# TianyiFranklinWang/MIRROR

Hardware: AMD Instinct MI355X
Metric: SSL samples/sec (slide+RNA pairs) (higher is better)
Workload: dtype bf16; 1 GPU; BASELINE c2: B=16/GPU x [4096 patch tokens x 1024-d] + [2048 genes], D=512, RNA depth 6 / 8 heads, train mode, local-batch InfoNCE; precision_policy=bf16, per_gpu_batch=16, global_batch=16, parallelism=dp1, grad_bucket_dtype=f32, step_launch=hip_graph

## Files before the change

include/mirror_hip.h:

```cpp
#ifndef MIRROR_HIP_H
#define MIRROR_HIP_H
#include <stdint.h>

#ifdef __cplusplus
extern "C" {
#endif

#define MH_OK 0
#define MH_EINVAL (-1)
#define MH_EUNSUP (-2)
#define MH_EHIP (-3)

#define MH_F32 0
#define MH_BF16 1

#define MH_ACT_NONE 0
#define MH_ACT_RELU 1
#define MH_ACT_GELU 2

typedef void* mh_stream;

const char* mh_last_error(void);
int mh_version(void);
int mh_exp_build(void);
// ... 23 lines not shown
    int32_t a_kc, b_kc;
    int32_t dtA, dtB, dtC, mma;
    int32_t batch1, batch2;
    int64_t sA1, sA2, sB1, sB2, sC1, sC2;
    float alpha, diag;
    int32_t act;
    int32_t accumulate;
    int32_t split_k;
    const void* R; float rcoef;
    float* workspace;
    int64_t workspace_floats;
    void* C2;
    int32_t r_bf16;
    int32_t k_segments;
    int64_t sA_seg, sB_seg;
    int32_t row_softmax;
    const mh_gemm_epi* epi;
    int32_t a_rows_per_batch, a_row_skip;
    int32_t shared_chip;
    int32_t c_rows_per_batch, c_row_skip;
    int32_t window_batches;
} mh_gemm_desc;
int mh_gemm(const mh_gemm_desc* d, mh_stream s);
const char* mh_gemm_variant_name(void);
int64_t mh_gemm_workspace_bytes(const mh_gemm_desc* d);

int mh_skinny_fwd(const void* x, int64_t ldx, const void* w, int64_t ldw, const float* bias, const float* addend, int64_t ldadd,
                  void* y, int64_t ldy, int M, int N, int K, int act, int dt_x, int dt_y, mh_stream s);
int mh_skinny_wgrad(const void* dy, int64_t lddy, const void* x, int64_t ldx, float* dw, int64_t lddw, float* db, int M, int N,
                    int K, int accumulate, int dt_dy, int dt_x, mh_stream s);
#define MH_SKINNY_MANY_MAX 32
typedef struct {
    const void* dy; int64_t lddy;
    const void* x; int64_t ldx;
    float* dw; int64_t lddw;
    float* db;
    int32_t M, N, K;
    int32_t dt_dy, dt_x;
} mh_skinny_wgrad_item;
int mh_skinny_wgrad_many(const mh_skinny_wgrad_item* items, int n, mh_stream s);
int mh_transpose_bf16(const void* in, void* out, int R, int C, mh_stream s);
int mh_transpose_bf16_many(const void* src, void* dst, const int64_t* table, int n, int max_r, int max_c, int vec_ok,
                           mh_stream s);

int mh_layernorm_fwd(const void* x, const float* gamma, const float* beta, void* y, float* mean, float* rstd,
                     int batches, int rows_per_batch, int D, int64_t x_bs, int64_t y_bs, float eps,
                     int dt_x, int dt_y, mh_stream s);
int mh_layernorm_fwd_dual(const float* x, const float* gamma, const float* beta, float* y, void* y_bf16, float* mean, float* rstd,
                          int batches, int rows_per_batch, int D, int64_t x_bs, int64_t y_bs, float eps, mh_stream s);
int mh_layernorm_fwd_q8(const float* x, const float* gamma, const float* beta, void* y, float* mean, float* rstd,
                        int batches, int rows_per_batch, int D, int64_t x_bs, int64_t y_bs, float eps, void* q8, unsigned* ring,
                        const float* tick, float margin, float* scale, mh_stream s);
int64_t mh_layernorm_bwd_workspace_bytes(int64_t rows, int D);
typedef struct {
    const void* dy;
    const void* x;
    const float *gamma, *mean, *rstd;
    void* dx;
    float *dgamma, *dbeta;
    int32_t batches, rows_per_batch, D;
    int64_t x_bs, y_bs;
    int32_t dt_x, dt_dy, dt_dx;
    int32_t accumulate_dx;
    float* workspace;
    int64_t ws_floats;
    const void* gadd;
    int32_t pad, l;
    const float* row_mask;
    const float* lm_scale;
    void* relu_out;
    int32_t relu_first, relu_rows;
    float* relu_db;
    const void* fan_bf16;
    float fan_alpha;
    const float* fan_cls;
    void* drop_out;
    float drop_p;
    uint64_t drop_seed, drop_offset;
    const uint64_t* drop_base;
    float* drop_db;
    int32_t drop_rows_per_batch;
} mh_ln_bwd;
int mh_layernorm_bwd(const mh_ln_bwd* d, mh_stream s);

int mh_layernorm_fwd_lm(const float* x, const float* gamma, const float* beta, void* y, float* mean, float* rstd, void* xpm,
                        void* xpm_bf16, int batches, int rows, int D, int64_t x_bs, int pad, int l, float eps, const float* row_mask,
                        const float* lm_scale, mh_stream s);

int mh_quant_fp8(const void* x, int64_t n, void* q, float* scale, unsigned* amax_scratch, int dt, mh_stream s);
int mh_quant_fp8_delayed(const void* x, int64_t n, void* q, float* scale, unsigned* ring, const float* tick, float margin,
                         int dt, mh_stream s);
int mh_gemm_fp8(const void* A, int64_t lda, int64_t a_bs, const void* B, int64_t ldb, void* C, int64_t ldc, int64_t c_bs, int batch,
                const float* scale_a, const float* scale_b, const float* bias, int act, int M, int N, int K, int dt_c, mh_stream s);

int mh_softmax_fwd(const void* x, void* y, int64_t rows, int cols, int64_t ldx, int64_t ldy,
                   int dt_x, int dt_y, mh_stream s);
int mh_softmax_bwd(const void* y, const void* dy, void* dx, int64_t rows, int cols, int64_t ldy, int64_t lddy,
                   int64_t lddx, int dt_y, int dt_dy, int dt_dx, mh_stream s);

int mh_softmax_masked_fwd(const void* x, void* y, const float* rowmask, const float* colmask, int64_t batches, int h, int R,
                          int cols, int dt_x, int dt_y, mh_stream s);
int mh_softmax_masked_bwd(const void* y, const void* dy, void* dx, const float* rowmask, const float* colmask, int64_t batches,
                          int h, int R, int cols, int dt_y, int dt_d, mh_stream s);
int mh_row_scale(const void* x, const float* scale, void* y, int64_t rows, int D, int dt, mh_stream s);
int mh_keymask_plan(const unsigned char* mask, float* mrow, float* mlm, float* lscale, int64_t B, int64_t n_src, int lead, int wrap,
                    int pad, int l, mh_stream s);

int mh_landmark_fwd(const void* qkv, void* lm, int B, int n_p, int D, int l, int dt, mh_stream s);
int mh_landmark_bwd(const void* dlm, void* dqkv, int B, int n_p, int D, int l, int dt, mh_stream s);
int mh_resconv_fwd(const void* v, int64_t ldv, int64_t v_bs, const float* w, void* out, int64_t ldo, int64_t o_bs,
                   int B, int n_p, int heads, int dh, int taps, int transpose, int accumulate,
                   int dt_v, int dt_o, mh_stream s);
int mh_resconv_wgrad(const void* v, int64_t ldv, int64_t v_bs, const void* dout, int64_t ldo, int64_t o_bs,
                     float* dw, int B, int n_p, int heads, int dh, int taps, int dt_v, int dt_o, mh_stream s);
int64_t mh_resconv_bwd_workspace_bytes(int B, int n_p, int heads, int dh, int taps);
int mh_resconv_bwd(const void* dout, int64_t ldo, int64_t o_bs, const void* v, int64_t ldv, int64_t v_bs, const float* w, void* dv,
                   int64_t lddv, int64_t dv_bs, float* dw, float* workspace, int64_t ws_floats, int B, int n_p, int heads, int dh,
                   int taps, int dt_v, int dt_o, mh_stream s);
int mh_pinv_absmax(const float* x, uint64_t* stats64, int BH, int m, mh_stream s);
int mh_pinv_z0(const float* x, const uint64_t* stats64, float* z0, int BH, int m, mh_stream s);
int mh_pinv_z0_bwd(const float* x, const float* z0, const float* dz0, const uint64_t* stats64, float* dx,
                   float* scratch1, int scratch_zeroed, int BH, int m, mh_stream s);
int mh_pinv_s2_bwd(const float* p, const float* dz0, const uint64_t* stats64, float* dx, float* scratch1, int scratch_zeroed, int BH,
                   int m, const float* mlm, int heads, mh_stream s);
int mh_pinv_chain_prep(const float* x, const uint64_t* stats64, float* z0, void* xp, void* z0p, int BH, int m, mh_stream s);
int mh_pinv_chain_pack(const float* dz, void* up, int BH, int m, mh_stream s);
int mh_pinv_chain_fwd(const void* XP, void* saved, void* zfT, int BH, int m, int iters, const float* z0f, const uint64_t* stats64,
                      int z0_rowmajor, mh_stream s);
int mh_nys_sim2(const void* lm, float* a2, void* xp, float* z0f, uint64_t* stats64, int B, int m, int D, int heads, float scale,
                int64_t lm_ld, const float* mlm, mh_stream s);
int mh_nys_dz_dav(const float* dw2, const float* av, const void* zfT, void* up, void* dav, float* delta3, int BH, int m, int dh,
                  mh_stream s);
int mh_pinv_chain_bwd(const void* XP, const void* saved, const void* dzf, void* work, float* dX, float* dz0, int BH, int m,
                      int iters, mh_stream s);
int64_t mh_pinv_chain_workspace_bytes(int BH, int m, int iters, int which);
int mh_nys_attn1_fwd(const void* qkv, const void* lm, const void* w2, void* out, float* lse1, const float* mrow, const float* mlm,
                     int B, int h, int n_p, int m, int dh, float scale, int accumulate, int64_t lm_ld, void* o1, mh_stream s);
int mh_nys_attn1_fwd_q8(const void* qkv, const void* lm, const void* w2, void* out, float* lse1, int B, int h, int n_p, int m, int dh,
                        float scale, int accumulate, void* q8, unsigned* ring, const float* tick, float margin, float* q8_scale, void* o1,
                        mh_stream s);
int64_t mh_nys_attn3_ws_floats(int B, int h, int n_p);
int64_t mh_nys_attn3_workspace_bytes(int B, int h, int n_p);
int mh_nys_attn3_fwd(const void* qkv, const void* lm, float* av, float* lse3, float* workspace, int64_t ws_floats,
                     const float* mrow, const float* mlm, int B, int h, int n_p, int m, int dh, float scale, int64_t lm_ld,
                     const float* rc_w, void* rc_out, mh_stream s);
int mh_nys_attn1_bwd(const void* qkv, const void* lm, const void* w2, const void* dout, const float* lse1, const void* o1, float* delta1,
                     void* dqkv, float* dw2, float* dlm, const float* mrow, const float* mlm, int B, int h, int n_p, int m, int dh,
                     float scale, int64_t lm_ld, mh_stream s);
int mh_nys_attn3_bwd(const void* qkv, const void* lm, const float* av, const void* dav, const float* lse3, float* delta3,
                     void* dqkv, float* dlm, const float* mrow, const float* mlm, int B, int h, int n_p, int m, int dh,
                     float scale, int64_t lm_ld, mh_stream s);
int mh_nys_cls_attn(const void* qkv, const void* lm, const void* z, const float* lse3, float* row, const float* mrow, const float* mlm,
                    int B, int h, int n_p, int m, int dh, int cls_row, float scale, int64_t lm_ld, int z_colmajor, int dt,
                    mh_stream s);
int mh_lm_merge(const float* a, const float* b, void* out, int64_t rows, int cols, int64_t out_ld, int zero_cols, mh_stream s);
int mh_eye_minus(const float* P, float* T, float d, int BH, int m, mh_stream s);

int mh_seq_finish(void* seq, const float* cls, int B, int N, int add, int D, int dt, mh_stream s);
int mh_seq_finish_bwd(void* dseq, float* dcls, int B, int N, int add, int D, int dt, mh_stream s);
int mh_ppeg_merge(const float* w7, const float* w5, const float* w3, const float* b7, const float* b5,
                  const float* b3, float* merged, float* bsum, int D, mh_stream s);
int mh_ppeg_fwd(const void* x, void* y, const float* merged, const float* bsum, int B, int S, int D,
                int flip, int dt_x, int dt_y, mh_stream s);
int mh_ppeg_wgrad(const void* x, const void* dout, float* dmerged, float* dbsum, int B, int S, int D,
                  int dt_x, int dt_o, mh_stream s);
int mh_ppeg_bwd(const float* x, const float* dy, const float* merged, float* dx, float* dmerged, float* dbsum, int B, int S,
// ... 296 lines not shown
```

mirror_amd/_lib.py:

```python
from __future__ import annotations

import ctypes as C
import os

_HERE = os.path.dirname(os.path.abspath(__file__))
LIB_PATH = os.environ.get("MIRROR_HIP_LIB") or os.path.join(_HERE, "lib", "libmirror_hip.so")

MH_F32, MH_BF16 = 0, 1
ACT_NONE, ACT_RELU, ACT_GELU = 0, 1, 2


class GemmEpi(C.Structure):
    _fields_ = [
        ("kind", C.c_int32), ("resid", C.c_void_p),
        ("p", C.c_float), ("seed", C.c_uint64), ("offset", C.c_uint64), ("dev_base", C.c_void_p),
        ("mask", C.c_void_p), ("token", C.c_void_p), ("pos", C.c_void_p),
        ("rows_per_batch", C.c_int32), ("first", C.c_int32),
        ("tgt", C.c_void_p), ("tgt_bs", C.c_int64), ("sq", C.c_void_p),
    ]


class SkinnyWgradItem(C.Structure):
    _fields_ = [("dy", C.c_void_p), ("lddy", C.c_int64), ("x", C.c_void_p), ("ldx", C.c_int64), ("dw", C.c_void_p), ("lddw", C.c_int64),
                ("db", C.c_void_p), ("M", C.c_int32), ("N", C.c_int32), ("K", C.c_int32), ("dt_dy", C.c_int32), ("dt_x", C.c_int32)]
# ... 4 lines not shown
        ("A", C.c_void_p), ("B", C.c_void_p), ("C", C.c_void_p), ("bias", C.c_void_p),
        ("M", C.c_int32), ("N", C.c_int32), ("K", C.c_int32),
        ("lda", C.c_int64), ("ldb", C.c_int64), ("ldc", C.c_int64),
        ("a_kc", C.c_int32), ("b_kc", C.c_int32),
        ("dtA", C.c_int32), ("dtB", C.c_int32), ("dtC", C.c_int32), ("mma", C.c_int32),
        ("batch1", C.c_int32), ("batch2", C.c_int32),
        ("sA1", C.c_int64), ("sA2", C.c_int64), ("sB1", C.c_int64), ("sB2", C.c_int64),
        ("sC1", C.c_int64), ("sC2", C.c_int64),
        ("alpha", C.c_float), ("diag", C.c_float),
        ("act", C.c_int32), ("accumulate", C.c_int32), ("split_k", C.c_int32),
        ("R", C.c_void_p), ("rcoef", C.c_float),
        ("workspace", C.c_void_p), ("workspace_floats", C.c_int64),
        ("C2", C.c_void_p), ("r_bf16", C.c_int32),
        ("k_segments", C.c_int32), ("sA_seg", C.c_int64), ("sB_seg", C.c_int64),
        ("row_softmax", C.c_int32),
        ("epi", C.POINTER(GemmEpi)), ("a_rows_per_batch", C.c_int32), ("a_row_skip", C.c_int32),
        ("shared_chip", C.c_int32),
        ("c_rows_per_batch", C.c_int32), ("c_row_skip", C.c_int32),
        ("window_batches", C.c_int32),
    ]


P, I, L, F, U64 = C.c_void_p, C.c_int, C.c_int64, C.c_float, C.c_uint64


class EmaCfg(C.Structure):
    _fields_ = [("decay", C.c_double), ("min_decay", C.c_double), ("warmup_gamma", C.c_double), ("warmup_power", C.c_double),
                ("update_after_step", C.c_int64), ("use_warmup", C.c_int32)]


class OptimCfg(C.Structure):
    _fields_ = [("rule", C.c_int32), ("beta1", C.c_float), ("beta2", C.c_float), ("eps", C.c_float), ("momentum", C.c_float),
                ("nesterov", C.c_int32)]


OPT_ADAM, OPT_ADAMW, OPT_SGD = 0, 1, 2
OPT_SKIP_GROUP = 255


class LossTermsDesc(C.Structure):
    _fields_ = [
        ("wsi_emb", C.c_void_p), ("rna_emb", C.c_void_p), ("logit_scale", C.c_void_p), ("align_ext", C.c_void_p),
        ("B", C.c_int32), ("D", C.c_int32), ("has_align", C.c_int32),
        ("rna_pred", C.c_void_p), ("rna_tgt", C.c_void_p), ("rna_mask", C.c_void_p), ("n_rna", C.c_int64),
        ("w_mu", C.c_void_p), ("w_logstd", C.c_void_p), ("r_mu", C.c_void_p), ("r_logstd", C.c_void_p),
        ("n_wstyle", C.c_int64), ("n_rstyle", C.c_int64), ("rows_wstyle", C.c_int32), ("rows_rstyle", C.c_int32),
        ("w_score", C.c_void_p), ("r_score", C.c_void_p), ("Bc", C.c_int32), ("P", C.c_int32),
        ("wsi_acc", C.c_void_p), ("weight", C.c_float * 6),
        ("scratch", C.c_void_p), ("save", C.c_void_p), ("out", C.c_void_p),
        ("g_total", C.c_void_p), ("g_terms", C.c_void_p),
        ("d_wsi_emb", C.c_void_p), ("d_rna_emb", C.c_void_p), ("d_logit_scale", C.c_void_p), ("d_align_ext", C.c_void_p),
        ("d_rna_pred", C.c_void_p), ("d_rna_tgt", C.c_void_p), ("d_w_mu", C.c_void_p), ("d_w_logstd", C.c_void_p), ("d_r_mu", C.c_void_p),
        ("d_r_logstd", C.c_void_p), ("d_w_score", C.c_void_p), ("d_r_score", C.c_void_p),
    ]


class RnaBlockDesc(C.Structure):
    _fields_ = (
        [("B", C.c_int32), ("D", C.c_int32), ("Hh", C.c_int32), ("H", C.c_int32), ("eps", C.c_float), ("p_drop", C.c_float),
         ("seed", C.c_uint64), ("offset", C.c_uint64), ("dev_base", C.c_void_p)]
        + [(n, C.c_void_p) for n in (
            "w_qkv", "w_proj", "w_fc1", "w_fc2", "wt_qkv", "wt_proj", "wt_fc1", "wt_fc2",
            "b_qkv", "b_proj", "b_fc1", "b_fc2", "g1", "be1", "g2", "be2",
            "x", "y", "stats", "qkv", "attn", "o", "x1", "u", "f", "dy", "dx",
            "dw_qkv", "dw_proj", "dw_fc1", "dw_fc2", "db_qkv", "db_proj", "db_fc1", "db_fc2", "dg1", "dbe1", "dg2", "dbe2",
            "scratch")])


class LnBwdDesc(C.Structure):
    _fields_ = [
        ("dy", C.c_void_p), ("x", C.c_void_p), ("gamma", C.c_void_p), ("mean", C.c_void_p), ("rstd", C.c_void_p),
        ("dx", C.c_void_p), ("dgamma", C.c_void_p), ("dbeta", C.c_void_p),
        ("batches", C.c_int32), ("rows_per_batch", C.c_int32), ("D", C.c_int32), ("x_bs", C.c_int64), ("y_bs", C.c_int64),
        ("dt_x", C.c_int32), ("dt_dy", C.c_int32), ("dt_dx", C.c_int32), ("accumulate_dx", C.c_int32),
        ("workspace", C.c_void_p), ("ws_floats", C.c_int64),
        ("gadd", C.c_void_p), ("pad", C.c_int32), ("l", C.c_int32), ("row_mask", C.c_void_p), ("lm_scale", C.c_void_p),
        ("relu_out", C.c_void_p), ("relu_first", C.c_int32), ("relu_rows", C.c_int32), ("relu_db", C.c_void_p),
        ("fan_bf16", C.c_void_p), ("fan_alpha", C.c_float), ("fan_cls", C.c_void_p),
        ("drop_out", C.c_void_p), ("drop_p", C.c_float), ("drop_seed", C.c_uint64), ("drop_offset", C.c_uint64),
        ("drop_base", C.c_void_p), ("drop_db", C.c_void_p), ("drop_rows_per_batch", C.c_int32),
    ]


_SIGS = {
    "mh_gemm": [C.POINTER(GemmDesc)],
    "mh_skinny_fwd": [P, L, P, L, P, P, L, P, L, I, I, I, I, I, I],
    "mh_skinny_wgrad": [P, L, P, L, P, L, P, I, I, I, I, I, I],
    "mh_skinny_wgrad_many": [C.POINTER(SkinnyWgradItem), I],
    "mh_transpose_bf16": [P, P, I, I],
    "mh_transpose_bf16_many": [P, P, P, I, I, I, I],
    "mh_layernorm_fwd": [P, P, P, P, P, P, I, I, I, L, L, F, I, I],
    "mh_layernorm_fwd_dual": [P, P, P, P, P, P, P, I, I, I, L, L, F],
    "mh_layernorm_fwd_q8": [P, P, P, P, P, P, I, I, I, L, L, F, P, P, P, F, P],
    "mh_layernorm_bwd": [C.POINTER(LnBwdDesc)],
    "mh_layernorm_fwd_lm": [P, P, P, P, P, P, P, P, I, I, I, L, I, I, F, P, P],
    "mh_softmax_fwd": [P, P, L, I, L, L, I, I],
    "mh_softmax_bwd": [P, P, P, L, I, L, L, L, I, I, I],
    "mh_landmark_fwd": [P, P, I, I, I, I, I],
    "mh_landmark_bwd": [P, P, I, I, I, I, I],
    "mh_resconv_fwd": [P, L, L, P, P, L, L, I, I, I, I, I, I, I, I, I],
    "mh_resconv_wgrad": [P, L, L, P, L, L, P, I, I, I, I, I, I, I],
    "mh_resconv_bwd": [P, L, L, P, L, L, P, P, L, L, P, P, L, I, I, I, I, I, I, I],
    "mh_pinv_absmax": [P, P, I, I],
    "mh_pinv_z0": [P, P, P, I, I],
    "mh_pinv_z0_bwd": [P, P, P, P, P, P, I, I, I],
    "mh_pinv_s2_bwd": [P, P, P, P, P, I, I, I, P, I],
    "mh_eye_minus": [P, P, F, I, I],
    "mh_pinv_chain_prep": [P, P, P, P, P, I, I],
    "mh_pinv_chain_pack": [P, P, I, I],
    "mh_pinv_chain_fwd": [P, P, P, I, I, I, P, P, I],
    "mh_nys_sim2": [P, P, P, P, P, I, I, I, I, F, L, P],
    "mh_nys_dz_dav": [P, P, P, P, P, P, I, I, I],
    "mh_pinv_chain_bwd": [P, P, P, P, P, P, I, I, I],
    "mh_nys_attn1_fwd": [P, P, P, P, P, P, P, I, I, I, I, I, F, I, L, P],
    "mh_nys_attn1_fwd_q8": [P, P, P, P, P, I, I, I, I, I, F, I, P, P, P, F, P, P],
    "mh_nys_attn3_fwd": [P, P, P, P, P, L, P, P, I, I, I, I, I, F, L, P, P],
    "mh_nys_attn1_bwd": [P, P, P, P, P, P, P, P, P, P, P, P, I, I, I, I, I, F, L],
    "mh_nys_attn3_bwd": [P, P, P, P, P, P, P, P, P, P, I, I, I, I, I, F, L],
    "mh_nys_cls_attn": [P, P, P, P, P, P, P, I, I, I, I, I, I, F, L, I, I],
    "mh_seq_finish": [P, P, I, I, I, I, I],
    "mh_seq_finish_bwd": [P, P, I, I, I, I, I],
    "mh_ppeg_merge": [P, P, P, P, P, P, P, P, I],
    "mh_ppeg_fwd": [P, P, P, P, I, I, I, I, I, I],
    "mh_ppeg_wgrad": [P, P, P, P, I, I, I, I, I],
    "mh_ppeg_bwd": [P, P, P, P, P, P, I, I, I, P, P, F, U64, U64, P],
    "mh_ppeg_grad_scatter": [P, P, P, P, P, P, P, P, I],
    "mh_rank_mask": [P, P, I, I, I],
    "mh_mask_apply_fwd": [P, P, P, P, P, I, I, I, I, I, I, I],
    "mh_mask_apply_bwd": [P, P, P, P, P, I, I, I, I, I, I, I, P],
    "mh_rank_mask_keep": [P, P, P, P, I, I, I],
    "mh_rows_gather": [P, P, P, I, I, I, I, I],
    "mh_mask_expand_fwd": [P, P, P, P, P, I, I, I, I, I],
    "mh_mask_apply_bwd_keep": [P, P, P, P, P, I, I, I, I, I, P],
    "mh_rows_expand_zero": [P, P, P, I, I, I, I, I],
    "mh_headattn_fwd": [P, P, P, I, I, I, I],
    "mh_headattn_bwd": [P, P, P, P, I, I, I, I],
    "mh_add": [P, P, P, L, I, I, I],
    "mh_lm_merge": [P, P, P, L, I, L, I],
    "mh_cast": [P, P, L, I, I],
    "mh_gelu_fwd": [P, P, L, I, I],
    "mh_gelu_bwd": [P, P, P, L, I, I, I],
    "mh_relu_bwd": [P, P, P, L, I, L, L, L, I, I, I],
    "mh_dropout": [P, P, L, F, U64, U64, P, I, I],
    "mh_noise_draws": [P, L, L, U64, U64, P],
    "mh_dropout_add": [P, P, P, L, F, U64, U64, P, I],
    "mh_dropout_lite": [P, P, P, L, F, U64, U64, P, I, I],
    "mh_timestamp": [P],
    "mh_dropout_lite_colsum": [P, P, L, I, F, U64, U64, P, P],
    "mh_colsum": [P, P, L, I, L, I],
    "mh_l2norm_fwd": [P, P, P, I, I, L, F, I, I],
    "mh_l2norm_bwd": [P, P, P, P, I, I, L, F, I, I, I, I],
    "mh_exp_fwd": [P, P, L],
    "mh_exp_bwd": [P, P, P, L, I],
    "mh_reparam_fwd": [P, P, P, P, L],
    "mh_reparam_bwd": [P, P, P, P, P, P, P, L],
    "mh_ce_rows_fwd": [P, L, P, F, I, I, I, F, P, P, P],
    "mh_ce_rows_bwd": [P, L, P, F, P, P, I, F, P, P, I, I, I],
    "mh_mse_masked_fwd": [P, P, P, P, L, I, L, L, I, I],
    "mh_mse_masked_fwd_ordered": [P, P, P, P, L, I, L, L, I, I, P],
    "mh_mse_masked_bwd": [P, P, P, P, P, F, P, P, L, I, L, L, I, I, I, P, I],
    "mh_fanout_bwd": [P, P, F, P, P, I, I, I, I],
    "mh_gather_rows": [P, P, P, L, L, L, I],
    "mh_sample_rows": [P, P, P, P, I, I, L, U64, U64, P, F],
    "mh_sample_weighted": [P, L, P, L, U64, U64, P],
    "mh_quant_fp8": [P, L, P, P, P, I],
    "mh_quant_fp8_delayed": [P, L, P, P, P, P, F, I],
    "mh_gemm_fp8": [P, L, L, P, L, P, L, L, I, P, P, P, I, I, I, I, I],
    "mh_weighted_sum": [P, P, P, P, P, P, F, F, F, F, F, F, I, P],
    "mh_weighted_sum_bwd": [P, F, F, F, F, F, F, I, P],
    "mh_softmax_masked_fwd": [P, P, P, P, L, I, I, I, I, I],
    "mh_softmax_masked_bwd": [P, P, P, P, P, L, I, I, I, I, I],
    "mh_row_scale": [P, P, P, L, I, I],
    "mh_keymask_plan": [P, P, P, P, L, L, I, I, I, I],
    "mh_kl_fwd": [P, P, P, L, F],
    "mh_kl_bwd": [P, P, P, P, P, L, F],
    "mh_symkl_fwd": [P, P, P, I, I, F],
    "mh_symkl_bwd": [P, P, P, P, P, I, I, F],
# ... 182 lines not shown
```

mirror_amd/csrc/norm_softmax.hip:

```cpp
#include "common.h"
#include <cstdlib>

#define LN_MAXPL 32

template <typename TX, typename TY>
__global__ __launch_bounds__(256) void layernorm_fwd_kernel(const TX* __restrict__ x, const float* __restrict__ gamma,
                                                            const float* __restrict__ beta, TY* __restrict__ y,
                                                            float* __restrict__ mean, float* __restrict__ rstd,
                                                            long rows, int rpb, int D, long x_bs, long y_bs, float eps) {
    const int lane = threadIdx.x & 63;
    const long row = (long)blockIdx.x * 4 + (threadIdx.x >> 6);
    if (row >= rows) return;
    const long b = row / rpb, i = row % rpb;
    const TX* xr = x + b * x_bs + i * D;
    TY* yr = y + b * y_bs + i * D;
    float v[LN_MAXPL];
    float s = 0.f;
#pragma unroll
    for (int k = 0; k < LN_MAXPL; k++) {
        const int c = lane + 64 * k;
        v[k] = (c < D) ? ldf(xr + c) : 0.f;
        s += v[k];
    }
    const float mu = wave_sum(s) / D;
    float q = 0.f;
#pragma unroll
    for (int k = 0; k < LN_MAXPL; k++) {
        const int c = lane + 64 * k;
        const float d = (c < D) ? v[k] - mu : 0.f;
        q += d * d;
    }
    const float rs = rsqrtf(wave_sum(q) / D + eps);
#pragma unroll
    for (int k = 0; k < LN_MAXPL; k++) {
        const int c = lane + 64 * k;
        if (c < D) stf(yr + c, (v[k] - mu) * rs * gamma[c] + beta[c]);
    }
    if (lane == 0) { mean[row] = mu; rstd[row] = rs; }
}

template <typename TX, typename TDY, typename TDX>
__global__ __launch_bounds__(256) void layernorm_bwd_kernel(const TDY* __restrict__ dy, const TX* __restrict__ x,
                                                            const float* __restrict__ gamma, const float* __restrict__ mean,
                                                            const float* __restrict__ rstd, TDX* __restrict__ dx,
                                                            float* __restrict__ dgamma, float* __restrict__ dbeta,
                                                            long rows, int rpb, int D, long x_bs, long y_bs, int acc_dx) {
    const int lane = threadIdx.x & 63, wave = threadIdx.x >> 6;
    float pg[LN_MAXPL], pb[LN_MAXPL];
#pragma unroll
    for (int k = 0; k < LN_MAXPL; k++) { pg[k] = 0.f; pb[k] = 0.f; }
    for (long row = (long)blockIdx.x * 4 + wave; row < rows; row += (long)gridDim.x * 4) {
        const long b = row / rpb, i = row % rpb;
        const TX* xr = x + b * x_bs + i * D;
        const TDY* dyr = dy + b * y_bs + i * D;
        TDX* dxr = dx + b * x_bs + i * D;
        const float mu = mean[row], rs = rstd[row];
        float xh[LN_MAXPL], gd[LN_MAXPL];
        float s1 = 0.f, s2 = 0.f;
#pragma unroll
        for (int k = 0; k < LN_MAXPL; k++) {
            const int c = lane + 64 * k;
            if (c < D) {
                const float d = ldf(dyr + c);
                xh[k] = (ldf(xr + c) - mu) * rs;
                gd[k] = d * gamma[c];
                pg[k] += d * xh[k];
                pb[k] += d;
                s1 += gd[k];
                s2 += gd[k] * xh[k];
            } else { xh[k] = 0.f; gd[k] = 0.f; }
        }
        s1 = wave_sum(s1) / D;
        s2 = wave_sum(s2) / D;
#pragma unroll
        for (int k = 0; k < LN_MAXPL; k++) {
            const int c = lane + 64 * k;
            if (c < D) {
                float r = rs * (gd[k] - s1 - xh[k] * s2);
                if (acc_dx) r += ldf(dxr + c);
                stf(dxr + c, r);
            }
        }
    }
    __shared__ float red[2][4][64];
#pragma unroll
    for (int k = 0; k < LN_MAXPL; k++) {
        if (64 * k >= D) break;
        __syncthreads();
        red[0][wave][lane] = pg[k];
        red[1][wave][lane] = pb[k];
        __syncthreads();
        if (wave == 0) {
            const int c = lane + 64 * k;
            if (c < D) {
                atomicAdd(dgamma + c, red[0][0][lane] + red[0][1][lane] + red[0][2][lane] + red[0][3][lane]);
                atomicAdd(dbeta + c, red[1][0][lane] + red[1][1][lane] + red[1][2][lane] + red[1][3][lane]);
            }
        }
    }
}

typedef f4_t f4;

template <typename TX, typename TY, int LNV_CH>
__global__ __launch_bounds__(256) void layernorm_fwd_vec_kernel(const TX* __restrict__ x, const float* __restrict__ gamma,
                                                                const float* __restrict__ beta, TY* __restrict__ y,
                                                                float* __restrict__ mean, float* __restrict__ rstd,
                                                                long rows, int rpb, int D, long x_bs, long y_bs, float eps,
                                                                bf16_t* __restrict__ y2 = nullptr) {
    const int lane = threadIdx.x & 63;
    const long row = (long)blockIdx.x * 4 + (threadIdx.x >> 6);
    if (row >= rows) return;
    const long b = row / rpb, i = row % rpb;
    const TX* xr = x + b * x_bs + i * D;
    TY* yr = y + b * y_bs + i * D;
    bf16_t* y2r = y2 ? y2 + b * y_bs + i * D : nullptr;
    f4 v[LNV_CH];
    float s = 0.f;
#pragma unroll
    for (int k = 0; k < LNV_CH; k++) {
        const int c = 256 * k + 4 * lane;
        if (c < D) { v[k] = ld4(xr + c); s += v[k][0] + v[k][1] + v[k][2] + v[k][3]; }
        else v[k] = (f4){0.f, 0.f, 0.f, 0.f};
    }
    const float mu = wave_sum(s) / D;
    float q = 0.f;
#pragma unroll
    for (int k = 0; k < LNV_CH; k++) {
        const int c = 256 * k + 4 * lane;
        if (c < D) {
#pragma unroll
            for (int e = 0; e < 4; e++) { const float d = v[k][e] - mu; q += d * d; }
        }
    }
    const float rs = rsqrtf(wave_sum(q) / D + eps);
#pragma unroll
    for (int k = 0; k < LNV_CH; k++) {
        const int c = 256 * k + 4 * lane;
        if (c < D) {
            const f4 g = ld4(gamma + c), bt = ld4(beta + c);
            f4 o;
#pragma unroll
            for (int e = 0; e < 4; e++) o[e] = (v[k][e] - mu) * rs * g[e] + bt[e];
            st4(yr + c, o);
            if (y2r) st4(y2r + c, o);
        }
    }
    if (lane == 0) { mean[row] = mu; rstd[row] = rs; }
}

#define LMU 2
template <int LNV_CH, int SPLIT>
__global__ __launch_bounds__(256) void layernorm_fwd_lm_kernel(const float* __restrict__ x, const float* __restrict__ gamma,
                                                               const float* __restrict__ beta, bf16_t* __restrict__ y,
                                                               float* __restrict__ mean, float* __restrict__ rstd,
                                                               float* __restrict__ xpm, bf16_t* __restrict__ xpm16, int groups, int m, int rows,
                                                               int D, long x_bs, int pad, int l, float eps, const float* __restrict__ rmask,
                                                               const float* __restrict__ lm_scale) {
    __shared__ f4 part[SPLIT > 1 ? 4 : 1][LNV_CH][64];
    const int lane = threadIdx.x & 63, wave = threadIdx.x >> 6, sub = wave % SPLIT;
    const int grp = blockIdx.x * (4 / SPLIT) + wave / SPLIT;
    if (SPLIT == 1 && grp >= groups) return;
    const int b = grp / m, g = grp - b * m;
    const long n_p = (long)pad + rows;
    f4 gm[LNV_CH], bt[LNV_CH], acc[LNV_CH];
#pragma unroll
    for (int k = 0; k < LNV_CH; k++) {
        const int c = 256 * k + 4 * lane;
        acc[k] = (f4){0.f, 0.f, 0.f, 0.f};
        gm[k] = c < D ? ld4(gamma + c) : acc[k];
        bt[k] = c < D ? ld4(beta + c) : acc[k];
    }
    const int per = (l + SPLIT - 1) / SPLIT;
    const int jbeg = g * l + sub * per;
    const int jend = min(jbeg + per, (g + 1) * l);
    auto load_chunk = [&](f4 (&v)[LMU][LNV_CH], float (&kp)[LMU], int j0) {
#pragma unroll
        for (int u = 0; u < LMU; u++) {
            const int j = j0 + u;
            const bool live = j < jend && j >= pad;
            const float* xr = x + b * x_bs + (long)(live ? j - pad : 0) * D;
            kp[u] = (rmask && live) ? rmask[b * n_p + j] : 1.f;
#pragma unroll
            for (int k = 0; k < LNV_CH; k++) {
                const int c = 256 * k + 4 * lane;
                v[u][k] = (live && c < D) ? ld4(xr + c) : (f4){0.f, 0.f, 0.f, 0.f};
            }
        }
    };
    auto do_chunk = [&](f4 (&v)[LMU][LNV_CH], float (&kp)[LMU], int j0) {
#pragma unroll
        for (int u = 0; u < LMU; u++) {
            const int j = j0 + u;
            if (j >= jend) break;
            bf16_t* yr = y + (b * n_p + j) * D;
            if (j < pad) {
#pragma unroll
                for (int k = 0; k < LNV_CH; k++) {
                    const int c = 256 * k + 4 * lane;
                    if (c < D) st4(yr + c, (f4){0.f, 0.f, 0.f, 0.f});
                }
                continue;
            }
            float s = 0.f;
#pragma unroll
            for (int k = 0; k < LNV_CH; k++) s += v[u][k][0] + v[u][k][1] + v[u][k][2] + v[u][k][3];
            const float mu = wave_sum(s) / D;
            float q = 0.f;
#pragma unroll
            for (int k = 0; k < LNV_CH; k++) {
                const int c = 256 * k + 4 * lane;
                if (c < D) {
#pragma unroll
                    for (int e = 0; e < 4; e++) { const float d = v[u][k][e] - mu; q += d * d; }
                }
            }
            const float rs = rsqrtf(wave_sum(q) / D + eps);
            const bool keep = kp[u] != 0.f;
#pragma unroll
            for (int k = 0; k < LNV_CH; k++) {
                const int c = 256 * k + 4 * lane;
                if (c < D) {
                    f4 o;
#pragma unroll
                    for (int e = 0; e < 4; e++) o[e] = keep ? bf2f(f2bf((v[u][k][e] - mu) * rs * gm[k][e] + bt[k][e])) : 0.f;
                    st4(yr + c, o);
                    acc[k] += o;
                }
// ... 165 lines not shown
        if (wave == 0) {
            const int c = 256 * k + 4 * lane;
            if (c < D) {
                const f4 g = red[0][0][lane] + red[0][1][lane] + red[0][2][lane] + red[0][3][lane];
                const f4 bb = red[1][0][lane] + red[1][1][lane] + red[1][2][lane] + red[1][3][lane];
#pragma unroll
                for (int e = 0; e < 4; e++) { atomicAdd(dgamma + c + e, g[e]); atomicAdd(dbeta + c + e, bb[e]); }
            }
        }
    }
}

extern "C" int mh_layernorm_fwd(const void* x, const float* gamma, const float* beta, void* y, float* mean, float* rstd,
                                int batches, int rpb, int D, int64_t x_bs, int64_t y_bs, float eps, int dt_x, int dt_y,
                                mh_stream s) {
    MH_REQUIRE(D >= 1 && D <= 64 * LN_MAXPL, "mh_layernorm_fwd: D=%d unsupported (max %d)", D, 64 * LN_MAXPL);
    const long rows = (long)batches * rpb;
    if (rows == 0) return MH_OK;
    dim3 grid(mh_cdiv(rows, 4));
    const bool vecok = D % 4 == 0 && x_bs % 4 == 0 && y_bs % 4 == 0 && ((uintptr_t)x & 15) == 0 && ((uintptr_t)y & 15) == 0 &&
                       ((uintptr_t)gamma & 15) == 0 && ((uintptr_t)beta & 15) == 0;
#define LN_FV1(TX, TY, NC) hipLaunchKernelGGL((layernorm_fwd_vec_kernel<TX, TY, NC>), grid, dim3(256), 0, (hipStream_t)s, (const TX*)x, gamma, beta, (TY*)y, mean, rstd, rows, rpb, D, (long)x_bs, (long)y_bs, eps)
#define LN_FV(TX, TY) do { if (D <= 512) LN_FV1(TX, TY, 2); else if (D <= 1024) LN_FV1(TX, TY, 4); else LN_FV1(TX, TY, 8); } while (0)
    if (vecok) {
        if (dt_x == MH_F32 && dt_y == MH_F32) LN_FV(float, float);
        else if (dt_x == MH_F32 && dt_y == MH_BF16) LN_FV(float, bf16_t);
        else if (dt_x == MH_BF16 && dt_y == MH_BF16) LN_FV(bf16_t, bf16_t);
        else LN_FV(bf16_t, float);
        MH_LAUNCH_CHECK("mh_layernorm_fwd");
        return MH_OK;
    }
#undef LN_FV
#undef LN_FV1
#define LN_F(TX, TY) hipLaunchKernelGGL((layernorm_fwd_kernel<TX, TY>), grid, dim3(256), 0, (hipStream_t)s, (const TX*)x, gamma, beta, (TY*)y, mean, rstd, rows, rpb, D, (long)x_bs, (long)y_bs, eps)
    if (dt_x == MH_F32 && dt_y == MH_F32) LN_F(float, float);
    else if (dt_x == MH_F32 && dt_y == MH_BF16) LN_F(float, bf16_t);
    else if (dt_x == MH_BF16 && dt_y == MH_BF16) LN_F(bf16_t, bf16_t);
    else LN_F(bf16_t, float);
#undef LN_F
    MH_LAUNCH_CHECK("mh_layernorm_fwd");
    return MH_OK;
}

extern "C" int mh_layernorm_fwd_lm(const float* x, const float* gamma, const float* beta, void* y, float* mean, float* rstd, void* xpm,
                                   void* xpm_bf16, int batches, int rows, int D, int64_t x_bs, int pad, int l, float eps, const float* row_mask,
                                   const float* lm_scale, mh_stream s) {
    MH_REQUIRE(l >= 1 && pad >= 0 && rows >= 1 && (pad + rows) % l == 0, "mh_layernorm_fwd_lm: pad + rows = %d must be a multiple of l = %d", pad + rows, l);
    MH_REQUIRE(D % 4 == 0 && D <= 2048 && x_bs % 4 == 0 && (((uintptr_t)x | (uintptr_t)gamma | (uintptr_t)beta) & 15) == 0 &&
                   ((uintptr_t)y & 7) == 0 && ((uintptr_t)xpm & 15) == 0 && ((uintptr_t)xpm_bf16 & 7) == 0,
               "mh_layernorm_fwd_lm: D %% 4 == 0, D <= 2048 and aligned buffers (D=%d)", D);
    if (batches == 0) return MH_OK;
    const int m = (pad + rows) / l, groups = batches * m;
    int split = 1;
    while (split < 4 && (long)groups * split < 4096 && l >= 8 * split && groups % (4 / (2 * split)) == 0) split *= 2;
#ifdef MH_EXP
    if (const char* e = getenv("MH_LN_LM_SPLIT")) split = atoi(e);
#endif
    MH_REQUIRE((split == 1 || split == 2 || split == 4) && groups % (4 / split) == 0, "mh_layernorm_fwd_lm: %d waves per group with %d groups", split, groups);
    dim3 grid(mh_cdiv(groups, 4 / split));
#define LNL_(NC, SP) hipLaunchKernelGGL((layernorm_fwd_lm_kernel<NC, SP>), grid, dim3(256), 0, (hipStream_t)s, x, gamma, beta, (bf16_t*)y, mean, rstd, (float*)xpm, (bf16_t*)xpm_bf16, groups, m, rows, D, (long)x_bs, pad, l, eps, row_mask, lm_scale)
#define LNL(NC) do { if (split == 1) LNL_(NC, 1); else if (split == 2) LNL_(NC, 2); else LNL_(NC, 4); } while (0)
    if (D <= 512) LNL(2); else if (D <= 1024) LNL(4); else LNL(8);
#undef LNL
#undef LNL_
    MH_LAUNCH_CHECK("mh_layernorm_fwd_lm");
    return MH_OK;
}

extern "C" int mh_layernorm_fwd_dual(const float* x, const float* gamma, const float* beta, float* y, void* y_bf16, float* mean, float* rstd,
                                     int batches, int rpb, int D, int64_t x_bs, int64_t y_bs, float eps, mh_stream s) {
    const long rows = (long)batches * rpb;
    if (rows == 0) return MH_OK;
    MH_REQUIRE(y_bf16 && D % 4 == 0 && D <= 2048 && x_bs % 4 == 0 && y_bs % 4 == 0 &&
                   (((uintptr_t)x | (uintptr_t)y | (uintptr_t)gamma | (uintptr_t)beta) & 15) == 0 && ((uintptr_t)y_bf16 & 7) == 0,
               "mh_layernorm_fwd_dual: D %% 4 == 0, D <= 2048 and aligned buffers (D=%d)", D);
    dim3 grid(mh_cdiv(rows, 4));
#define LND(NC) hipLaunchKernelGGL((layernorm_fwd_vec_kernel<float, float, NC>), grid, dim3(256), 0, (hipStream_t)s, x, gamma, beta, y, mean, rstd, rows, rpb, D, (long)x_bs, (long)y_bs, eps, (bf16_t*)y_bf16)
    if (D <= 512) LND(2); else if (D <= 1024) LND(4); else LND(8);
#undef LND
    MH_LAUNCH_CHECK("mh_layernorm_fwd_dual");
    return MH_OK;
}

extern "C" int mh_layernorm_fwd_q8(const float* x, const float* gamma, const float* beta, void* y, float* mean, float* rstd,
                                   int batches, int rows_per_batch, int D, int64_t x_bs, int64_t y_bs, float eps, void* q8, unsigned* ring,
                                   const float* tick, float margin, float* scale, mh_stream s) {
    const long rows = (long)batches * rows_per_batch;
    if (rows == 0) return MH_OK;
    MH_REQUIRE(D % 4 == 0 && D <= 2048 && x_bs % 4 == 0 && y_bs % 4 == 0 && (((uintptr_t)x | (uintptr_t)gamma | (uintptr_t)beta) & 15) == 0 &&
                   ((uintptr_t)y & 7) == 0 && ((uintptr_t)q8 & 3) == 0,
               "mh_layernorm_fwd_q8: D %% 4 == 0, D <= 2048 and aligned buffers (D=%d)", D);
    MH_REQUIRE(ring && tick && scale && margin >= 1.f, "mh_layernorm_fwd_q8: ring, tick, scale and margin >= 1 are required");
    dim3 grid((unsigned)min((long)mh_cdiv(rows, 4), 4096L));
#define LNQ(NC) hipLaunchKernelGGL((layernorm_fwd_q8_kernel<NC>), grid, dim3(256), 0, (hipStream_t)s, x, gamma, beta, (bf16_t*)y, mean, rstd, rows, rows_per_batch, D, (long)x_bs, (long)y_bs, eps, (unsigned char*)q8, ring, tick, margin, scale)
    if (D <= 512) LNQ(2); else if (D <= 1024) LNQ(4); else LNQ(8);
#undef LNQ
    MH_LAUNCH_CHECK("mh_layernorm_fwd_q8");
    return MH_OK;
}

template <typename TX, typename TDY, int LNV_CH, bool RELU = false, bool FAN = false, bool DROP = false>
__global__ __launch_bounds__(256, LNV_CH == 2 ? 4 : 1) void layernorm_bwd_ws_kernel(const TDY* __restrict__ dy, const TX* __restrict__ x,
                                                               const float* __restrict__ gamma, const float* __restrict__ mean,
                                                               const float* __restrict__ rstd, TX* __restrict__ dx,
                                                               float* __restrict__ ws, int rows, int rpb, int D, long x_bs,
                                                               long y_bs, int acc_dx, int rows_per_block,
                                                               const TDY* __restrict__ gadd = nullptr, int ga_pad = 0, int ga_l = 1,
                                                               int ga_m = 0, float ga_scale = 0.f, bf16_t* __restrict__ relu_out = nullptr,
                                                               int relu_first = 0, int relu_rows = 0, int relu_cs = 0,
                                                               const bf16_t* __restrict__ fan = nullptr, float fan_alpha = 0.f,
                                                               const float* __restrict__ fan_cls = nullptr,
                                                               bf16_t* __restrict__ drop_out = nullptr, float drop_p = 0.f, uint64_t drop_seed = 0,
                                                               uint64_t drop_offset = 0, const uint64_t* __restrict__ drop_base = nullptr,
                                                               int drop_rpb = 0, const float* __restrict__ rmask = nullptr,
                                                               const float* __restrict__ lm_scale = nullptr) {
    const int lane = threadIdx.x & 63, wave = threadIdx.x >> 6;
    constexpr bool THIRD = RELU || DROP;
    __shared__ f4 sgm[THIRD ? LNV_CH : 1][64];
    f4 pg[LNV_CH], pb[LNV_CH], gm[THIRD ? 1 : LNV_CH], pr[THIRD ? LNV_CH : 1];
    uint32_t dthr = 0;
    float dscale = 1.f;
    if constexpr (DROP) {
        if (drop_base) drop_offset += *drop_base & ~7ull;
        dthr = drop16_thr(drop_p);
        dscale = drop16_scale(dthr);
    }
#pragma unroll
    for (int k = 0; k < LNV_CH; k++) {
        pg[k] = (f4){0.f, 0.f, 0.f, 0.f};
        pb[k] = pg[k];
        if constexpr (THIRD) pr[k] = pg[k];
        const int c = 256 * k + 4 * lane;
        if constexpr (THIRD) {
            if (wave == 0) sgm[k][lane] = (c < D) ? ld4(gamma + c) : pg[k];
        } else gm[k] = (c < D) ? ld4(gamma + c) : pg[k];
    }
    if constexpr (THIRD) __syncthreads();
    const int r0 = blockIdx.x * rows_per_block, r1 = min(rows, r0 + rows_per_block);
    for (int row = r0 + wave; row < r1; row += 8) {
        uint32_t keepbits = 0;
        if constexpr (DROP) {
            static_assert(LNV_CH <= 4, "one byte per chunk in a 32-bit word");
            const int odd = lane & 1;
            const int rr = row + 4 * odd;
            uint32_t mine = 0;
            if (rr < r1) {
                const long orow = drop_rpb == rpb ? (long)rr : (long)(rr / rpb) * drop_rpb + (rr % rpb);
#pragma unroll
                for (int k = 0; k < LNV_CH; k++) {
                    const int c8 = 256 * k + 8 * (lane >> 1);
                    if (c8 < D) mine |= drop16_keep8((drop_offset + (uint64_t)(orow * D + c8)) >> 3, drop_seed, dthr) << (8 * k);
                }
            }
            const uint32_t other = (uint32_t)__builtin_amdgcn_mov_dpp((int)mine, 0xB1, 0xF, 0xF, true);
#pragma unroll
            for (int u = 0; u < 2; u++) {
                const uint32_t src = (odd == u) ? mine : other;
#pragma unroll
                for (int k = 0; k < LNV_CH; k++) keepbits |= (((src >> (8 * k)) >> (4 * odd)) & 15u) << (4 * (u * LNV_CH + k));
            }
            asm volatile("" : "+v"(keepbits));
        }
        f4 dv[2][LNV_CH], xv[2][LNV_CH], ov[2][LNV_CH];
        float mu[2], rs[2];
        long xo[2], ro[2];
        bool ok[2];
#pragma unroll
        for (int u = 0; u < 2; u++) {
            const int rr = row + 4 * u;
            ok[u] = rr < r1;
            const int rc = ok[u] ? rr : row;
            const int b = rc / rpb, i = rc - b * rpb;
            xo[u] = b * x_bs + (long)i * D;
            ro[u] = (RELU && i >= relu_first && i < relu_first + relu_rows) ? ((long)b * relu_rows + (i - relu_first)) * D
                    : (DROP ? ((long)b * drop_rpb + i) * D : -1);
            const TDY* dyr = dy + b * y_bs + (long)i * D;
            mu[u] = mean[rc];
            rs[u] = rstd[rc];
#pragma unroll
            for (int k = 0; k < LNV_CH; k++) {
                const int c = 256 * k + 4 * lane;
                if (c < D) {
                    dv[u][k] = ld4(dyr + c);
                    xv[u][k] = ld4(x + xo[u] + c);
                    if (acc_dx) ov[u][k] = ld4(dx + xo[u] + c);
                    if (gadd) dv[u][k] += ld4(gadd + ((long)b * ga_m + (i + ga_pad) / ga_l) * D + c) *
                                          (lm_scale ? ga_scale * lm_scale[(long)b * ga_m + (i + ga_pad) / ga_l] : ga_scale);
                    if (rmask && rmask[(long)b * (ga_pad + rpb) + ga_pad + i] == 0.f) dv[u][k] = (f4){0.f, 0.f, 0.f, 0.f};
                    if constexpr (FAN) {
                        if (i >= 1) dv[u][k] += ld4(fan + ((long)b * (rpb - 1) + (i - 1)) * D + c) * fan_alpha;
                        else if (fan_cls) dv[u][k] += ld4(fan_cls + (long)b * D + c);
                    }
                }
            }
        }
#pragma unroll
        for (int u = 0; u < 2; u++) {
            if (!ok[u]) continue;
            float s1 = 0.f, s2 = 0.f;
            unsigned pos = 0;
#pragma unroll
            for (int k = 0; k < LNV_CH; k++) {
                const int c = 256 * k + 4 * lane;
                if (c < D) {
                    f4 gq;
                    if constexpr (THIRD) gq = sgm[k][lane]; else gq = gm[k];
#pragma unroll
                    for (int e = 0; e < 4; e++) {
                        if constexpr (RELU) pos |= (xv[u][k][e] > 0.f ? 1u : 0u) << (4 * k + e);
                        const float xh = (xv[u][k][e] - mu[u]) * rs[u];
                        const float d = dv[u][k][e];
                        const float gd = d * gq[e];
                        pg[k][e] += d * xh;
                        pb[k][e] += d;
                        s1 += gd;
                        s2 += gd * xh;
                        xv[u][k][e] = xh;
                        dv[u][k][e] = gd;
                    }
                }
            }
            s1 = wave_sum(s1) / D;
            s2 = wave_sum(s2) / D;
#pragma unroll
            for (int k = 0; k < LNV_CH; k++) {
                const int c = 256 * k + 4 * lane;
                if (c < D) {
                    f4 r;
#pragma unroll
                    for (int e = 0; e < 4; e++) r[e] = rs[u] * (dv[u][k][e] - s1 - xv[u][k][e] * s2);
                    if (acc_dx) r += ov[u][k];
                    if (RELU && !DROP && ro[u] >= 0) {
                        typedef unsigned ln_u32x2 __attribute__((ext_vector_type(2)));
                        const ln_u32x2 w = {pack_bf2((pos >> (4 * k)) & 1u ? r[0] : 0.f, (pos >> (4 * k + 1)) & 1u ? r[1] : 0.f),
                                         pack_bf2((pos >> (4 * k + 2)) & 1u ? r[2] : 0.f, (pos >> (4 * k + 3)) & 1u ? r[3] : 0.f)};
                        *reinterpret_cast<ln_u32x2*>(relu_out + ro[u] + c) = w;
                        pr[k] += (f4){__uint_as_float(w[0] << 16), __uint_as_float(w[0] & 0xffff0000u),
                                      __uint_as_float(w[1] << 16), __uint_as_float(w[1] & 0xffff0000u)};
                    } else {
                        st4(dx + xo[u] + c, r);
                        if constexpr (DROP) {
                            typedef unsigned ln_u32x2d __attribute__((ext_vector_type(2)));
                            const long e0 = ro[u] + c;
                            const uint32_t keep = keepbits >> (4 * (u * LNV_CH + k));
                            const ln_u32x2d w = {pack_bf2((keep & 1u) ? __fmul_rn(r[0], dscale) : 0.f, (keep & 2u) ? __fmul_rn(r[1], dscale) : 0.f),
                                                 pack_bf2((keep & 4u) ? __fmul_rn(r[2], dscale) : 0.f, (keep & 8u) ? __fmul_rn(r[3], dscale) : 0.f)};
                            *reinterpret_cast<ln_u32x2d*>(drop_out + e0) = w;
                            pr[k] += (f4){__uint_as_float(w[0] << 16), __uint_as_float(w[0] & 0xffff0000u),
                                          __uint_as_float(w[1] << 16), __uint_as_float(w[1] & 0xffff0000u)};
                        }
                    }
                }
            }
        }
    }
    __shared__ f4 red[THIRD ? 3 : 2][4][64];
    const int segs = ((RELU && relu_cs) || DROP) ? 3 : 2;
    float* wsb = ws + (long)blockIdx.x * segs * D;
#pragma unroll
    for (int k = 0; k < LNV_CH; k++) {
        if (256 * k >= D) break;
        __syncthreads();
        red[0][wave][lane] = pg[k];
        red[1][wave][lane] = pb[k];
        if constexpr (THIRD) red[2][wave][lane] = pr[k];
        __syncthreads();
        if (wave == 0) {
            const int c = 256 * k + 4 * lane;
            if (c < D) {
                *reinterpret_cast<f4*>(wsb + c) = red[0][0][lane] + red[0][1][lane] + red[0][2][lane] + red[0][3][lane];
                *reinterpret_cast<f4*>(wsb + D + c) = red[1][0][lane] + red[1][1][lane] + red[1][2][lane] + red[1][3][lane];
                if constexpr (THIRD)
                    if (DROP || relu_cs) *reinterpret_cast<f4*>(wsb + 2 * D + c) = red[2][0][lane] + red[2][1][lane] + red[2][2][lane] + red[2][3][lane];
            }
        }
    }
}

__global__ __launch_bounds__(256) void layernorm_bwd_fold_kernel(const float* __restrict__ ws, int nb, int D, float* __restrict__ dgamma,
                                                                 float* __restrict__ dbeta) {
    const int t = blockIdx.x * 256 + threadIdx.x;
    if (t >= 2 * D) return;
    const int per = (nb + gridDim.y - 1) / gridDim.y;
    const int b0 = blockIdx.y * per, b1 = min(nb, b0 + per);
    float s = 0.f;
    for (int b = b0; b < b1; b++) s += ws[(long)b * 2 * D + t];
    atomicAdd(t < D ? dgamma + t : dbeta + (t - D), s);
}

__global__ __launch_bounds__(256) void layernorm_bwd_fold4_kernel(const float* __restrict__ ws, int nb, int D, float* __restrict__ dgamma,
                                                                  float* __restrict__ dbeta, int segs = 2, float* __restrict__ dthird = nullptr) {
    typedef float lf4 __attribute__((ext_vector_type(4)));
    __shared__ lf4 red[4][64];
    const int lane = threadIdx.x & 63, wave = threadIdx.x >> 6;
    const int t = (blockIdx.x * 64 + lane) * 4;
    const bool live = t < segs * D;
    const int chunks = gridDim.y * 4, per = (nb + chunks - 1) / chunks;
    const int b0 = (blockIdx.y * 4 + wave) * per, b1 = min(nb, b0 + per);
    lf4 s = {0.f, 0.f, 0.f, 0.f};
    if (live) {
        int b = b0;
        for (; b + 8 <= b1; b += 8) {
            lf4 v[8];
#pragma unroll
            for (int u = 0; u < 8; u++) v[u] = *reinterpret_cast<const lf4*>(ws + (long)(b + u) * segs * D + t);
#pragma unroll
            for (int u = 0; u < 8; u++) s += v[u];
        }
        for (; b < b1; b++) s += *reinterpret_cast<const lf4*>(ws + (long)b * segs * D + t);
    }
    red[wave][lane] = s;
    __syncthreads();
    if (wave == 0 && live) {
        s = red[0][lane] + red[1][lane] + red[2][lane] + red[3][lane];
        float* dst = t < D ? dgamma + t : (t < 2 * D ? dbeta + (t - D) : dthird + (t - 2 * D));
#pragma unroll
        for (int e = 0; e < 4; e++) atomicAdd(dst + e, s[e]);
    }
}

static int ln_bwd_blocks() { return 512; }

extern "C" int64_t mh_layernorm_bwd_workspace_bytes(int64_t rows, int D) {
    if (rows < 64 || D <= 0) return 0;
    const int64_t nb = rows / 16 < 1024 ? (rows / 16 < 1 ? 1 : rows / 16) : 1024;
    return 3 * (int64_t)D * nb * 4;
}

static int ln_bwd_impl(const mh_ln_bwd& d, mh_stream s) {
    const int D = d.D, rpb = d.rows_per_batch, dt_x = d.dt_x, dt_dy = d.dt_dy;
    const int l = d.gadd ? d.l : 1;
    const long rows = (long)d.batches * rpb;
    const bool vecok = D % 4 == 0 && d.x_bs % 4 == 0 && d.y_bs % 4 == 0 && ((uintptr_t)d.x & 15) == 0 && ((uintptr_t)d.dy & 15) == 0 &&
                       ((uintptr_t)d.dx & 15) == 0 && ((uintptr_t)d.gamma & 15) == 0;
    const bool ws_form = vecok && d.workspace && d.ws_floats >= 2L * D && rows >= 64;
    const bool f32_x = dt_x == MH_F32 && d.dt_dx == MH_F32;
    const bool ws3 = ((uintptr_t)d.workspace & 15) == 0 && d.ws_floats >= 3L * D;
    const bool fan_ok = rpb >= 2 && ((uintptr_t)d.fan_bf16 & 7) == 0 && (!d.fan_cls || ((uintptr_t)d.fan_cls & 15) == 0) && D % 4 == 0;
    MH_REQUIRE(D >= 1 && D <= 64 * LN_MAXPL, "mh_layernorm_bwd: D=%d unsupported", D);
    MH_REQUIRE(d.dt_dx == dt_x, "mh_layernorm_bwd: dx dtype must equal x dtype");
    MH_REQUIRE(rows < (1L << 31), "mh_layernorm_bwd: too many rows");
    MH_REQUIRE(!d.gadd || (l >= 1 && d.pad >= 0 && (d.pad + rpb) % l == 0 && ((uintptr_t)d.gadd & 15) == 0),
               "mh_layernorm_bwd: landmark rider: l >= 1, pad >= 0, (pad + rows) %% l == 0, gadd on 16 bytes");
    MH_REQUIRE(d.gadd || (!d.relu_out && !d.row_mask && !d.lm_scale), "mh_layernorm_bwd: landmark rider: relu_out, row_mask and lm_scale need gadd");
    MH_REQUIRE(!d.gadd || (!d.fan_bf16 && !d.drop_out), "mh_layernorm_bwd: landmark rider: gadd excludes fan_bf16 and drop_out");
    MH_REQUIRE(!d.relu_out || (dt_x == MH_F32 && dt_dy == MH_BF16 && d.relu_first >= 0 && d.relu_rows >= 0 && d.relu_first + d.relu_rows <= rpb &&
                               ((uintptr_t)d.relu_out & 7) == 0 && D % 4 == 0),
               "mh_layernorm_bwd: ReLU rider: relu_out needs f32 x, bf16 dy and a row range inside the batch");
    MH_REQUIRE(!d.relu_db || (d.relu_out && ws3), "mh_layernorm_bwd: ReLU rider: relu_db rides on relu_out (workspace of >= 3 D floats)");
    MH_REQUIRE(!d.fan_bf16 || (f32_x && fan_ok), "mh_layernorm_bwd: fan rider: f32 x / dx, fan [batches, rows - 1, D] bf16 on quads, rows >= 2");
    MH_REQUIRE(!d.drop_out || d.drop_rows_per_batch >= rpb, "mh_layernorm_bwd: drop rider: the Dropout's tensor has %d rows per batch, the norm reads %d",
               d.drop_rows_per_batch, rpb);
    MH_REQUIRE(!d.drop_out || (f32_x && d.drop_db && d.drop_p >= 0.f && d.drop_p < 1.f && (d.drop_offset & 7) == 0 && ((uintptr_t)d.drop_out & 7) == 0 &&
                               D % 8 == 0 && D <= 1024 && ws3),
               "mh_layernorm_bwd: drop rider: f32 x / dx, drop_out / drop_db, p in [0, 1), offset %% 8 == 0, D %% 8 == 0, D <= 1024, a workspace of >= 3 D floats");
    MH_REQUIRE(rows == 0 || ws_form || !(d.gadd || d.fan_bf16 || d.drop_out),
               "mh_layernorm_bwd: the %s rider needs the workspace form (D %% 4 == 0, 16-byte aligned buffers, a workspace of >= %d D floats, >= 64 rows)",
               d.gadd ? "landmark" : (d.drop_out ? "drop" : "fan"), d.drop_out ? 3 : 2);
    if (rows == 0) return MH_OK;
    dim3 grid((unsigned)min((long)mh_cdiv(rows, 4), (long)ln_bwd_blocks()));
    if (ws_form) {
        float* third = d.drop_out ? d.drop_db : d.relu_db;
        const int segs = third ? 3 : 2;
        const long cap = d.ws_floats / ((long)segs * D);
        long nb = min(cap, min((long)mh_cdiv(rows, 16), 1024L));
        const int rows_per_block = (int)(mh_cdiv(mh_cdiv(rows, nb), 8) * 8);
        nb = mh_cdiv(rows, rows_per_block);
        dim3 g2((unsigned)nb);
#define LN_WS(TX, TDY, NC, RL, FN, DR) hipLaunchKernelGGL((layernorm_bwd_ws_kernel<TX, TDY, NC, RL, FN, DR>), g2, dim3(256), 0, (hipStream_t)s, (const TDY*)d.dy, (const TX*)d.x, d.gamma, d.mean, d.rstd, (TX*)d.dx, d.workspace, (int)rows, rpb, D, (long)d.x_bs, (long)d.y_bs, d.accumulate_dx, rows_per_block, (const TDY*)d.gadd, d.pad, l, (d.pad + rpb) / l, 1.f / (float)l, (bf16_t*)d.relu_out, d.relu_first, d.relu_rows, d.relu_db ? 1 : 0, (const bf16_t*)d.fan_bf16, d.fan_alpha, d.fan_cls, (bf16_t*)d.drop_out, d.drop_p, d.drop_seed, d.drop_offset, d.drop_base, d.drop_rows_per_batch, d.row_mask, d.lm_scale)
#define LN_BW(TX, TDY, RL) do { if (D <= 512) LN_WS(TX, TDY, 2, RL, false, false); else if (D <= 1024) LN_WS(TX, TDY, 4, RL, false, false); else LN_WS(TX, TDY, 8, RL, false, false); } while (0)
#define LN_BWF(NC) do { if (dt_dy == MH_F32) LN_WS(float, float, NC, false, true, false); else LN_WS(float, bf16_t, NC, false, true, false); } while (0)
#define LN_BWD(TDY, FN) do { if (D <= 512) LN_WS(float, TDY, 2, false, FN, true); else LN_WS(float, TDY, 4, false, FN, true); } while (0)
        if (d.drop_out) {
            if (d.fan_bf16 && dt_dy == MH_F32) LN_BWD(float, true);
            else if (d.fan_bf16) LN_BWD(bf16_t, true);
            else if (dt_dy == MH_F32) LN_BWD(float, false);
            else LN_BWD(bf16_t, false);
        } else if (d.fan_bf16) {
            if (D <= 512) LN_BWF(2); else if (D <= 1024) LN_BWF(4); else LN_BWF(8);
        } else if (d.relu_out) LN_BW(float, bf16_t, true);
        else if (dt_x == MH_F32 && dt_dy == MH_F32) LN_BW(float, float, false);
        else if (dt_x == MH_F32 && dt_dy == MH_BF16) LN_BW(float, bf16_t, false);
        else if (dt_x == MH_BF16 && dt_dy == MH_BF16) LN_BW(bf16_t, bf16_t, false);
        else LN_BW(bf16_t, float, false);
#undef LN_BWD
#undef LN_BWF
#undef LN_BW
#undef LN_WS
        if (D % 4 == 0 && ((uintptr_t)d.workspace & 15) == 0)
            hipLaunchKernelGGL(layernorm_bwd_fold4_kernel, dim3(mh_cdiv(segs * D / 4, 64), (unsigned)min(mh_cdiv(nb, 32), 16)), dim3(256), 0,
                               (hipStream_t)s, (const float*)d.workspace, (int)nb, D, d.dgamma, d.dbeta, segs, third);
        else
            hipLaunchKernelGGL(layernorm_bwd_fold_kernel, dim3(mh_cdiv(2 * D, 256), (unsigned)min(nb, 32L)), dim3(256), 0, (hipStream_t)s,
                               (const float*)d.workspace, (int)nb, D, d.dgamma, d.dbeta);
        MH_LAUNCH_CHECK("mh_layernorm_bwd");
        return MH_OK;
    }
    if (vecok) {
#define LN_BV1(TX, TDY, NC) hipLaunchKernelGGL((layernorm_bwd_vec_kernel<TX, TDY, NC>), grid, dim3(256), 0, (hipStream_t)s, (const TDY*)d.dy, (const TX*)d.x, d.gamma, d.mean, d.rstd, (TX*)d.dx, d.dgamma, d.dbeta, rows, rpb, D, (long)d.x_bs, (long)d.y_bs, d.accumulate_dx)
#define LN_BV(TX, TDY) do { if (D <= 512) LN_BV1(TX, TDY, 2); else if (D <= 1024) LN_BV1(TX, TDY, 4); else LN_BV1(TX, TDY, 8); } while (0)
        if (dt_x == MH_F32 && dt_dy == MH_F32) LN_BV(float, float);
        else if (dt_x == MH_F32 && dt_dy == MH_BF16) LN_BV(float, bf16_t);
        else if (dt_x == MH_BF16 && dt_dy == MH_BF16) LN_BV(bf16_t, bf16_t);
        else LN_BV(bf16_t, float);
#undef LN_BV
#undef LN_BV1
        MH_LAUNCH_CHECK("mh_layernorm_bwd");
        return MH_OK;
    }
#define LN_B(TX, TDY) hipLaunchKernelGGL((layernorm_bwd_kernel<TX, TDY, TX>), grid, dim3(256), 0, (hipStream_t)s, (const TDY*)d.dy, (const TX*)d.x, d.gamma, d.mean, d.rstd, (TX*)d.dx, d.dgamma, d.dbeta, rows, rpb, D, (long)d.x_bs, (long)d.y_bs, d.accumulate_dx)
    if (dt_x == MH_F32 && dt_dy == MH_F32) LN_B(float, float);
    else if (dt_x == MH_F32 && dt_dy == MH_BF16) LN_B(float, bf16_t);
    else if (dt_x == MH_BF16 && dt_dy == MH_BF16) LN_B(bf16_t, bf16_t);
    else LN_B(bf16_t, float);
#undef LN_B
    MH_LAUNCH_CHECK("mh_layernorm_bwd");
    return MH_OK;
}

extern "C" int mh_layernorm_bwd(const mh_ln_bwd* d, mh_stream s) {
    MH_REQUIRE(d, "mh_layernorm_bwd: NULL descriptor");
    return ln_bwd_impl(*d, s);
}

template <typename TX, typename TY, bool WAVE>
__global__ __launch_bounds__(256) void softmax_fwd_kernel(const TX* x, TY* y, long rows,
                                                          int cols, long ldx, long ldy) {
    __shared__ float red[4];
    const int lane = threadIdx.x & 63;
    const long row = WAVE ? (long)blockIdx.x * 4 + (threadIdx.x >> 6) : (long)blockIdx.x;
    if (WAVE && row >= rows) return;
    const int t0 = WAVE ? lane : threadIdx.x, step = WAVE ? 64 : 256;
    const TX* xr = x + row * ldx;
    TY* yr = y + row * ldy;
    float m = -INFINITY;
    for (int c = t0; c < cols; c += step) m = fmaxf(m, ldf(xr + c));
    m = WAVE ? wave_max(m) : block_max256(m, red);
    float sum = 0.f;
    for (int c = t0; c < cols; c += step) sum += __expf(ldf(xr + c) - m);
    sum = WAVE ? wave_sum(sum) : block_sum256(sum, red);
    const float inv = 1.f / sum;
    for (int c = t0; c < cols; c += step) stf(yr + c, __expf(ldf(xr + c) - m) * inv);
}

template <typename TY, typename TDY, typename TDX, bool WAVE>
__global__ __launch_bounds__(256) void softmax_bwd_kernel(const TY* y, const TDY* dy,
                                                          TDX* dx, long rows, int cols, long ldy, long lddy,
                                                          long lddx) {
    __shared__ float red[4];
    const int lane = threadIdx.x & 63;
    const long row = WAVE ? (long)blockIdx.x * 4 + (threadIdx.x >> 6) : (long)blockIdx.x;
    if (WAVE && row >= rows) return;
    const int t0 = WAVE ? lane : threadIdx.x, step = WAVE ? 64 : 256;
    const TY* yr = y + row * ldy;
    const TDY* dyr = dy + row * lddy;
    TDX* dxr = dx + row * lddx;
    float dot = 0.f;
    for (int c = t0; c < cols; c += step) dot += ldf(yr + c) * ldf(dyr + c);
    dot = WAVE ? wave_sum(dot) : block_sum256(dot, red);
    for (int c = t0; c < cols; c += step) stf(dxr + c, ldf(yr + c) * (ldf(dyr + c) - dot));
}

template <typename TX, typename TY, bool WAVE, int NV>
__global__ __launch_bounds__(256) void softmax_fwd_vec_kernel(const TX* x, TY* y, long rows, int cols, long ldx, long ldy) {
    __shared__ float red[4];
    const int lane = threadIdx.x & 63;
    const long row = WAVE ? (long)blockIdx.x * 4 + (threadIdx.x >> 6) : (long)blockIdx.x;
    if (WAVE && row >= rows) return;
    const int t0 = (WAVE ? lane : threadIdx.x) * 4, step = (WAVE ? 64 : 256) * 4;
    const TX* xr = x + row * ldx;
    TY* yr = y + row * ldy;
    f4 v[NV];
    float m = -INFINITY;
#pragma unroll
    for (int k = 0; k < NV; k++) {
        const int c = t0 + k * step;
        if (c < cols) { v[k] = ld4(xr + c); m = fmaxf(fmaxf(fmaxf(m, v[k][0]), fmaxf(v[k][1], v[k][2])), v[k][3]); }
    }
    m = WAVE ? wave_max(m) : block_max256(m, red);
    float sum = 0.f;
#pragma unroll
    for (int k = 0; k < NV; k++) {
        const int c = t0 + k * step;
        if (c < cols) {
#pragma unroll
            for (int e = 0; e < 4; e++) { v[k][e] = __expf(v[k][e] - m); sum += v[k][e]; }
        }
    }
    sum = WAVE ? wave_sum(sum) : block_sum256(sum, red);
    const float inv = 1.f / sum;
#pragma unroll
    for (int k = 0; k < NV; k++) {
        const int c = t0 + k * step;
        if (c < cols) st4(yr + c, v[k] * inv);
    }
}

template <typename TY, typename TD, bool WAVE, int NV>
__global__ __launch_bounds__(256) void softmax_bwd_vec_kernel(const TY* y, const TD* dy, TD* dx, long rows, int cols, long ldy,
                                                              long lddy, long lddx) {
    __shared__ float red[4];
    const int lane = threadIdx.x & 63;
    const long row = WAVE ? (long)blockIdx.x * 4 + (threadIdx.x >> 6) : (long)blockIdx.x;
    if (WAVE && row >= rows) return;
    const int t0 = (WAVE ? lane : threadIdx.x) * 4, step = (WAVE ? 64 : 256) * 4;
// ... 221 lines not shown
```

mirror_amd/functional.py:

```python
from __future__ import annotations

from dataclasses import dataclass
from typing import List, Optional, Tuple

import os

import torch
from torch.autograd import Function

from . import kernels as K
from ._lib import ACT_NONE, ACT_RELU, MH_BF16, MH_F32

f32, bf16 = torch.float32, torch.bfloat16


@dataclass(frozen=True)
class Precision:
    name: str
    mma: int
    act: torch.dtype
    pinv_mma: int
    fp8_fwd: bool = False


# ... 778 lines not shown
def to_out_dropout_add(resid, core, w, b, r0: int, R: int, p: float, training: bool, prec: Precision, res=None, link=None):
    if (training and p > 0.0 and prec.act == bf16 and not prec.fp8_fwd and resid.dtype == f32 and resid.is_contiguous()
            and core.dtype == bf16 and tuple(resid.shape) == (core.shape[0], R, w.shape[0]) and (core.shape[0] * R * w.shape[0]) % 8 == 0
            and K.linear_fused_ok(core, shadow(w, prec), (r0, R))):
        site = _DropSite() if (_DROP_IN_LN_BWD and b is not None) else None
        out = ToOutDropAddFn.apply(resid, core, w, b, r0, R, p, prec, site, res, link)
        if site is not None:
            out._drop_site = site
        return out
    y = LinearRowsFn.apply(core, w, b, r0, R, prec, prec.act)
    return dropout_add(resid, y, p, training, lite=True, res=res)


class HeadSqErrFn(Function):

    @staticmethod
    def forward(ctx, x, w, b, r0, R, prec, tgt, mask, acc, cs_tok=None):
        wa = shadow(w, prec)
        Bn, T, Kd = x.shape
        N = wa.shape[0]
        y = torch.empty((Bn, R, N), device=x.device, dtype=bf16)
        K.linear_fused(x, wa, None if b is None else b.detach(), y,
                       K.epi_sqerr(mask, tgt, tgt.stride(0), acc, R), window=(r0, R))
        ctx.save_for_backward(x, wa, w, b)
        ctx.r0, ctx.R, ctx.prec, ctx.cs_tok = r0, R, prec, cs_tok
        return y

    @staticmethod
    def backward(ctx, dy):
        x, wa, w, b = ctx.saved_tensors
        prec = ctx.prec
        if not dy.is_contiguous():
            dy = dy.contiguous()
        if dy.dtype != prec.act:
            dy = K.cast(dy, prec.act)
        got = None if ctx.cs_tok is None else ctx.cs_tok.claim(dy)
        db_table = None if got is None else got[0]
        dx, dw, db = _linear_rows_bwd(ctx.needs_input_grad[0:3], x, wa, w, b, ctx.r0, ctx.R, prec, dy, db_table=db_table)
        return dx, dw, db, None, None, None, None, None, None, None


def head_sqerr(x, w, b, r0: int, R: int, prec: Precision, tgt, mask):
    N = w.shape[0]
    if (tgt is not None and mask is not None and prec.act == bf16 and not prec.fp8_fwd and x.dtype == bf16 and tgt.dtype == f32
            and tgt.dim() == 3 and tuple(tgt.shape) == (x.shape[0], R, N) and tgt.stride(2) == 1 and tgt.stride(1) == N
            and mask.dtype == f32 and mask.is_contiguous() and tuple(mask.shape) == (x.shape[0], R) and R % 256 == 0
            and torch.is_grad_enabled() and K.linear_fused_ok(x, shadow(w, prec), (r0, R))):
        acc = zeros((2,), x.device)
        tok = _Handover("colsum") if (b is not None and _BIAS_IN_PRODUCER) else None
        y = HeadSqErrFn.apply(x, w, b, r0, R, prec, tgt, mask, acc, tok)
        y._sq = (acc, tgt, mask, tgt._version, mask._version)
        y._sq_cs = tok
        return y
    return LinearRowsFn.apply(x, w, b, r0, R, prec, prec.act)


def _cs_of(pred, acc):
    sq, tok = getattr(pred, "_sq", None), getattr(pred, "_sq_cs", None)
    return tok if (sq is not None and tok is not None and acc is not None and sq[0] is acc) else None


def _mse_bwd_cs(tok, pred, tgt, dp, D):
    if tok is None or not K.mse_masked_bwd_colsum_ok(pred, tgt, dp, D):
        return None
    ws = torch.empty((K.MSE_CS_BLOCKS, D), device=dp.device, dtype=f32)
    tok.offer(dp, ws)
    return ws


def _sq_of(pred, tgt, mask):
    sq = getattr(pred, "_sq", None)
    if sq is None:
        return None
    acc, t0, m0, tv, mv = sq
    if (t0.data_ptr() == tgt.data_ptr() and tuple(t0.shape) == tuple(tgt.shape) and t0.stride() == tgt.stride() and t0._version == tv
            and m0.data_ptr() == mask.data_ptr() and tuple(m0.shape) == tuple(mask.shape) and m0._version == mv):
        return acc
    return None


class EmbedMaskPosFn(Function):

    @staticmethod
    def forward(ctx, h32, h, w, b, mask, token, pos, first, prec, keepmap=None):
        wa = shadow(w, prec)
        Bn, T, Kd = h.shape
        N = wa.shape[0]
        out = torch.empty((Bn, T, N), device=h.device, dtype=f32)
        M = Bn * T
        bd = None if b is None else b.detach()
        tok, ps = token.detach().reshape(-1).contiguous(), pos.detach().reshape(T, N).contiguous()
        ctx.geom = (Bn, T, N, first, token.shape, pos.shape, prec)
        ctx.params = (token, pos)
        ctx.keep = None if keepmap is None else keepmap[2]
        if keepmap is not None:
            keep_idx, slot, keep = keepmap
            hc = K.rows_gather(h, keep_idx, first, keep)
            rc = _gemm_rows(hc, wa.t(), bias=bd, mma=prec.mma, out_dtype=bf16)
            K.mask_expand_fwd(rc, slot, tok, ps, T, first, keep, out)
            ctx.save_for_backward(hc, wa, w, b, slot)
            return out
        tail = K.linear_fused_tail(M)
        fork = _tail_fork() if tail else None
        K.linear_fused(h, wa, bd, out, K.epi_maskpos(mask, tok, ps, T, first), m_rows=M - tail)
        if tail and T - tail >= first:
            with _tail_branch(fork, h.device):
                rt = _tail_rows(h[Bn - 1, T - tail:], wa.t(), torch.empty((tail, N), device=h.device, dtype=bf16), bias=bd, mma=prec.mma)
                K.mask_apply_fwd(rt.view(1, tail, N), mask[Bn - 1, T - tail - first:].contiguous(), tok, ps[T - tail:].reshape(-1), 1, tail, N, 0,
                                 False, out=out[Bn - 1:, T - tail:])
        elif tail:
            raise K.MirrorHipError("EmbedMaskPosFn: the tail rows cross the unmasked prefix")
        ctx.save_for_backward(h, wa, w, b, mask)
        return out

    @staticmethod
    def backward(ctx, dy):
        h, wa, w, b, mask = ctx.saved_tensors
        Bn, T, N, first, tshape, pshape, prec = ctx.geom
        keep = ctx.keep
        Tc = T if keep is None else first + keep
        dy = dy.contiguous()
        dr = torch.empty((Bn, Tc, N), device=dy.device, dtype=prec.act)
        token, pos = ctx.params
        dtok, s_tok = _gbuf_n(token, (N,))
        dpos, s_pos = _gbuf_n(pos, (T * N,))
        db_in = None
        quad = K.mask_apply_bwd_dbias_ok(dy, dr, dpos, N)
        if b is not None and ctx.needs_input_grad[3] and _BIAS_IN_PRODUCER and (quad or keep is not None):
            db_in = _gbuf(b, (N,))
        dbias = None if db_in is None else db_in[0]
        if keep is None:
            K.mask_apply_bwd(dy, mask, dtok, dpos, Bn, T, N, first, False, out=dr, dbias=dbias)
        elif quad:
            K.mask_apply_bwd_keep(dy, mask, dtok, dpos, Bn, T, N, first, keep, out=dr, dbias=dbias)
        else:
            dp = zeros((T * N,), dy.device)
            K.mask_apply_bwd_keep(dy, mask, dtok, dp, Bn, T, N, first, keep, out=dr, dbias=dbias)
            dpos.add_(dp)
        dtok, dpos = _gret(token, dtok, s_tok), _gret(pos, dpos, s_pos)
        needs = (ctx.needs_input_grad[0], ctx.needs_input_grad[2], ctx.needs_input_grad[3])
        dh, dw, db = _linear_rows_bwd(needs, h, wa, w, b, 0, Tc, prec, dr, dx_dtype=f32, db_have=db_in)
        if keep is not None and dh is not None:
            dh = K.rows_expand_zero(dh, mask, T, first, keep)
        return (dh, None, dw, db, None, None if dtok is None else dtok.reshape(tshape), None if dpos is None else dpos.reshape(pshape),
                None, None, None)


def embed_mask_pos(h, w, b, mask, token, pos, first: int, prec: Precision):
    hb = h if h.dtype == bf16 else getattr(h, "_bf16", None)
    if (hb is not None and prec.act == bf16 and not prec.fp8_fwd and hb.is_contiguous() and tuple(hb.shape) == tuple(h.shape)
            and mask.dtype == f32 and mask.is_contiguous() and hb.shape[1] >= 256 and K.linear_fused_ok(hb, shadow(w, prec))
            and token.numel() == w.shape[0] and pos.numel() == h.shape[1] * w.shape[0]):
        keepmap = _keep_of(mask, hb.shape[0], hb.shape[1] - first)
        if keepmap is not None and -(-hb.shape[0] * hb.shape[1] // 256) * (w.shape[0] // 256) <= _EMBED_KEEP_TILES:
            keepmap = None
        return EmbedMaskPosFn.apply(h, hb, w, b, mask, token, pos, first, prec, keepmap)
    r = linear(h, w, b, prec=prec)
    return MaskApplyFn.apply(r, mask, token, pos, first, False)


_EMBED_KEEP_TILES = _CUS


def _keep_of(mask, Bn: int, n_tok: int):
    km = getattr(mask, "_keep", None)
    if km is None or mask._version != 0 or tuple(mask.shape) != (Bn, n_tok):
        return None
    keep_idx, slot, keep = km
    if tuple(slot.shape) != (Bn, n_tok) or tuple(keep_idx.shape) != (Bn, keep) or slot.device != mask.device:
        return None
    return km


class LayerNormFn(Function):

    @staticmethod
    def forward(ctx, x, gamma, beta, eps, rows, pad, out_dtype, q8_key=None, dual=None, fan_slot=None, res=None, q8_out=None):
        x = x.contiguous()
        Bn, T, D = x.shape
        y = torch.empty((Bn, pad + rows, D), device=x.device, dtype=out_dtype)
        ctx.fan_slot, ctx.res = fan_slot, res
        ctx.drop_site = getattr(x, "_drop_site", None) if (_DROP_IN_LN_BWD and pad == 0 and x.dtype == f32) else None
        if ctx.drop_site is not None and ctx.drop_site.shape != (Bn, T, D):
            ctx.drop_site = None
        if dual is not None:
            mean = torch.empty((Bn * rows,), device=x.device, dtype=f32)
            rstd = torch.empty_like(mean)
            y16 = torch.empty((Bn, rows, D), device=x.device, dtype=bf16)
            K.layernorm_fwd_dual(x, gamma.detach(), beta.detach(), y, y16, mean, rstd, Bn, rows, D, T * D, rows * D, eps)
            dual.append(y16)
            ctx.save_for_backward(x, gamma, mean, rstd, beta)
            ctx.rows, ctx.pad = rows, pad
            return y
        if pad:
            y[:, :pad].zero_()
        mean = torch.empty((Bn * rows,), device=x.device, dtype=f32)
        rstd = torch.empty_like(mean)
        st = _fp8_state
        site = st["sites"].get(q8_key) if (q8_key is not None and st["tick"] is not None) else None
        if site is not None and st["host_step"] - site[1] >= 2 and x.dtype == f32 and out_dtype == bf16 and D % 4 == 0 and D <= 2048:
            q = torch.empty((Bn, pad + rows, D), device=x.device, dtype=torch.uint8)
            if pad:
                q[:, :pad].zero_()
            sc = K.layernorm_fwd_q8(x, gamma.detach(), beta.detach(), y[:, pad:], mean, rstd, Bn, rows, D, T * D, (pad + rows) * D, eps,
                                    q[:, pad:], site[0], st["tick"])
            q8_out.append((q, sc))
        else:
            K.layernorm_fwd(x, gamma.detach(), beta.detach(), y[:, pad:], mean, rstd, Bn, rows, D, T * D, (pad + rows) * D, eps)
        ctx.save_for_backward(x, gamma, mean, rstd, beta)
        ctx.rows, ctx.pad = rows, pad
        return y

    @staticmethod
    def backward(ctx, dy):
        x, gamma, mean, rstd, beta = ctx.saved_tensors
        Bn, T, D = x.shape
        rows, pad = ctx.rows, ctx.pad
        if not dy.is_contiguous():
            dy = dy.contiguous()
        dg, sunk_g = _gbuf(gamma, (D,))
        db, sunk_b = _gbuf(beta, (D,))
        fan = None
        if ctx.fan_slot is not None and ctx.fan_slot.extra is not None:
            fan, ctx.fan_slot.extra = ctx.fan_slot.extra, None
            if pad or not K.layernorm_bwd_fan_ok(dy, x, x, fan[0], fan[2], Bn, rows, D):
                dy, fan = K.fanout_bwd(dy.float(), fan[0], fan[1], fan[2], Bn, rows, D), None
        G = None if ctx.res is None else ctx.res.take("grad")
        if G is not None and G.numel() == x.numel() and G.dtype == x.dtype and G.is_contiguous():
            G = G.view(x.shape)
            K.layernorm_bwd(dy[:, pad:], x, gamma.detach(), mean, rstd, G, dg, db, Bn, rows, D, T * D, (pad + rows) * D,
                            accumulate_dx=True, fan=fan)
            return None, _gret(gamma, dg, sunk_g), _gret(beta, db, sunk_b), None, None, None, None, None, None, None, None, None
        dx = torch.empty_like(x)
        if rows < T:
            dx[:, rows:].zero_()
        site, drop = ctx.drop_site, None
        if site is not None:
            gbd = torch.empty((Bn, T, D), device=x.device, dtype=bf16)
            cs = zeros((D,), x.device)
            if K.layernorm_bwd_drop_ok(dy, x, dx, gbd, cs, Bn, rows, D, site.offset) and (fan is None or dy.dtype == f32):
                if rows < T:
                    gbd[:, rows:].zero_()
                drop = (gbd, site.p, site.seed, site.offset, site.base, cs)
                site.offer(dx, gbd, cs)
        K.layernorm_bwd(dy[:, pad:], x, gamma.detach(), mean, rstd, dx, dg, db, Bn, rows, D, T * D, (pad + rows) * D, fan=fan, drop=drop)
        return dx, _gret(gamma, dg, sunk_g), _gret(beta, db, sunk_b), None, None, None, None, None, None, None, None, None


def _alias(base: torch.Tensor, offset: int, size, stride) -> torch.Tensor:
    t = torch.empty(0, device=base.device, dtype=base.dtype)
    t.set_(base.untyped_storage(), base.storage_offset() + int(offset), tuple(size), tuple(stride))
    return t


class NormQkvLmFn(Function):

    @staticmethod
    def forward(ctx, x, gamma, beta, eps, rows, pad, l, w, prec, link, rmask=None, lscale=None, res=None):
        ctx.relu_slot = getattr(x, "_relu_slot", None)
        ctx.link, ctx.res = link, res
        x = x.contiguous()
        Bn, T, D = x.shape
        n_p = pad + rows
        m = n_p // l
        P, E = Bn * n_p, Bn * m
        wa = shadow(w, prec)
        N3, c0 = wa.shape[0], 2 * wa.shape[1]
        xe = torch.empty((P + E, D), device=x.device, dtype=bf16)
        mean = torch.empty((Bn * rows,), device=x.device, dtype=f32)
        rstd = torch.empty_like(mean)
        xs = xe[:P].view(Bn, n_p, D)
        K.layernorm_fwd_lm(x, gamma.detach(), beta.detach(), xs, mean, rstd, None, Bn, rows, D, T * D, pad, l, eps, xpm_bf16=xe[P:],
                           row_mask=rmask, lm_scale=lscale)
        ctx.rmask, ctx.lscale = rmask, lscale
        qe = torch.empty((P + E, N3), device=x.device, dtype=bf16)
        qkv = _alias(qe, 0, (Bn, n_p, N3), (n_p * N3, N3, 1))
        fast = (pad > 0 and prec.mma == MH_BF16 and c0 % 256 == 0 and (N3 - c0) % 256 == 0
                and K.gemm_rows_ext_ok(Bn, n_p, pad, rows, E, D, c0, xe, qe[:, :c0]) and _rows_window_ok(xs, qkv[..., c0:], pad, rows, N3 - c0, prec))
        if fast:
            fork = _tail_fork()
            tail = K.gemm_rows_ext(xe, wa[:c0].t(), qe[:, :c0], Bn, n_p, pad, rows, E)
            if tail:
                with _tail_branch(fork, x.device):
                    _tail_rows(xe[P + E - tail:], wa[:c0].t(), qe[P + E - tail:, :c0], mma=prec.mma)

            def later():
                fork = _tail_fork()
                _rows_window(xs, wa[c0:].t(), qkv[..., c0:], pad, rows, mma=prec.mma)
                with _tail_branch(fork, x.device):
                    qkv[:, :pad].zero_()
        else:
            K.gemm(xe, wa[:c0].t(), out=qe[:, :c0], mma=prec.mma)

            def later():
                K.gemm(xe[:P], wa[c0:].t(), out=qe[:P, c0:], mma=prec.mma)
        link.v_cols = later
        ctx.save_for_backward(x, gamma, mean, rstd, beta, xe, wa, w)
        ctx.geo = (rows, pad, l, fast, prec)
        return qkv, _alias(qe, P * N3, (Bn, m, c0), (m * N3, N3, 1))

    @staticmethod
    def backward(ctx, dqkv, dlm):
        x, gamma, mean, rstd, beta, xe, wa, w = ctx.saved_tensors
        rows, pad, l, fast, prec = ctx.geo
        Bn, T, D = x.shape
        n_p = pad + rows
        m = n_p // l
        P, E = Bn * n_p, Bn * m
        N3, c0 = wa.shape[0], 2 * wa.shape[1]
        pend = ctx.link.take("lm_merge")
        merge = None if pend is None else pend[1]
        de = ext_rows_of(dqkv, dlm, P, E, N3, c0, copy_lm=merge is None)
        if pend is not None and de.data_ptr() != pend[0].data_ptr():
            raise K.MirrorHipError("NormQkvLmFn.backward: the pending landmark merge belongs to another gradient buffer")
        dxe = torch.empty((P + E, D), device=x.device, dtype=bf16)
        if fast:
            fork = _tail_fork()
            _rows_window(de[:P].view(Bn, n_p, N3), wa, dxe[:P].view(Bn, n_p, D), pad, rows, mma=prec.mma, wt=shadow_t(w, prec))
            with _tail_branch(fork, x.device):
                if merge is not None:
                    merge()
                K.gemm(de[P:, :c0], wa[:c0], out=dxe[P:], mma=prec.mma)
        else:
            if merge is not None:
                merge()
            K.gemm(de, wa, out=dxe, mma=prec.mma)
        dw = None
        if ctx.needs_input_grad[7]:
            dwb, sunk = _gbuf(w, (N3, D))
# ... 40 lines not shown
        return dx, _gret(gamma, dg, sunk_g), _gret(beta, db, sunk_b), None, None, None, None, dw, None, None, None, None, None


def ext_rows_alloc(Bn: int, n_p: int, m: int, N3: int, c0: int, device):
    P, E = Bn * n_p, Bn * m
    de = torch.empty((P + E, N3), device=device, dtype=bf16)
    return de, _alias(de, 0, (Bn, n_p, N3), (n_p * N3, N3, 1)), _alias(de, P * N3, (Bn, m, c0), (m * N3, N3, 1))


def ext_rows_of(dqkv, dlm, P: int, E: int, N3: int, c0: int, copy_lm: bool = True):
    if (dqkv.dtype == bf16 and dlm.dtype == bf16 and dqkv.is_contiguous() and dqkv.numel() == P * N3
            and dlm.data_ptr() == dqkv.data_ptr() + P * N3 * 2 and dlm.dim() == 3 and tuple(dlm.stride()) == (dlm.shape[1] * N3, N3, 1)
            and dlm.shape[0] * dlm.shape[1] == E and dlm.shape[2] == c0
            and dqkv.untyped_storage().nbytes() - dqkv.storage_offset() * 2 >= (P + E) * N3 * 2):
        return torch.as_strided(dqkv, (P + E, N3), (N3, 1))
    if not copy_lm:
        raise K.MirrorHipError("NormQkvLmFn.backward: a pending landmark merge needs the gradient views of ext_rows_alloc")
    de = torch.empty((P + E, N3), device=dqkv.device, dtype=bf16)
    de[:P].copy_(dqkv.reshape(P, N3))
    de[P:, :c0].copy_(dlm.reshape(E, c0))
    de[P:, c0:].zero_()
    return de


_KEYMASK_PLAN = True
class KeyMask:

    def __init__(self, src: torch.Tensor, lead: int = 0, wrap: int = 0):
        self.src = src if src.dtype == torch.bool else src.to(torch.bool)
        self.src = self.src.contiguous()
        self.lead, self.wrap = int(lead), int(wrap)
        self.shape = (src.shape[0], self.lead + src.shape[1] + self.wrap)
        self._plans = {}

    def dense(self) -> torch.Tensor:
        parts = ([torch.ones_like(self.src[:, :1]).expand(-1, self.lead)] if self.lead else []) + [self.src] + (
            [self.src[:, :self.wrap]] if self.wrap else [])
        return torch.cat(parts, dim=1) if len(parts) > 1 else self.src

    def plan(self, pad: int, l: int):
        key = (pad, l)
        if key not in self._plans:
            if _KEYMASK_PLAN:
                self._plans[key] = K.keymask_plan(self.src, self.lead, self.wrap, pad, l)
            else:
                n = self.shape[1]
                mrow = torch.nn.functional.pad(self.dense().to(torch.float32), (pad, 0), value=0.0).contiguous()
                cnt = mrow.reshape(mrow.shape[0], (n + pad) // l, l).sum(-1)
                self._plans[key] = (mrow, (cnt > 0).float().contiguous(), (float(l) / (cnt + 1e-8)).contiguous())
        return self._plans[key]


_LM_ROWS = True
_RELU_SQUARE_PAD = True
_RELU_IN_LN_BWD = True
class _ReluSlot(_Handover):
    __slots__ = ("n", "bias", "redo")

    def __init__(self):
        super().__init__("relu")
        self.n = self.bias = self.redo = None


def layer_norm_landmarks_ok(x, rows: int, pad: int, l: int, prec: Precision) -> bool:
    return (_LM_ROWS and prec.act == bf16 and not prec.fp8_fwd and x.dim() == 3 and x.dtype == f32 and x.shape[-1] % 4 == 0
            and x.shape[-1] <= 2048 and (pad + rows) % l == 0 and x.shape[0] * rows >= 64)


def fp8_site_key(w: torch.Tensor, prec: "Precision"):
    return (shadow(w, prec).data_ptr(), "x")


_FAN_IN_LN_BWD = True


class _FanSlot:
    __slots__ = ("extra",)

    def __init__(self):
        self.extra = None



def layer_norm(x, gamma, beta, eps, *, rows=None, pad=0, out_dtype=f32, q8_key=None, bf16_copy=False, res=None):
    squeeze = x.dim() == 2
    if squeeze:
        x = x.unsqueeze(0)
    r = x.shape[1] if rows is None else rows
    dual = None
    if (bf16_copy and not squeeze and x.dtype == f32 and out_dtype == f32 and pad == 0 and x.shape[-1] % 4 == 0
            and x.shape[-1] <= 2048 and q8_key is None):
        dual = []
    slot = _FanSlot() if (_FAN_IN_LN_BWD and not squeeze and pad == 0 and out_dtype == f32 and x.dtype == f32) else None
    q8 = [] if q8_key is not None else None
    y = LayerNormFn.apply(x, gamma, beta, eps, r, pad, out_dtype, q8_key, dual, slot, res, q8)
    if dual:
        y._bf16 = dual[0]
    if q8:
        y._q8 = q8[0]
    if slot is not None:
        y._fan_slot = slot
    return y.squeeze(0) if squeeze else y


class AddFn(Function):

    @staticmethod
    def forward(ctx, a, b, out_dtype, residual):
        ctx.da, ctx.db = a.dtype, b.dtype
        ctx.res = residual if a.is_contiguous() else None
        return K.add(a.contiguous(), b.contiguous(), out_dtype=out_dtype)

    @staticmethod
    def backward(ctx, dy):
        dy = dy.contiguous()
        ga = K.cast(dy, ctx.da)
        if ctx.res is not None and ga.dtype == f32:
            ctx.res.grad = ga
        return ga, K.cast(dy, ctx.db), None, None


def add(a, b, out_dtype=f32, residual=None):
    return AddFn.apply(a, b, out_dtype, residual)


class GeluFn(Function):
    @staticmethod
    def forward(ctx, x):
        x = x.contiguous()
        ctx.save_for_backward(x)
        return K.gelu_fwd(x)

    @staticmethod
    def backward(ctx, dy):
        (x,) = ctx.saved_tensors
        dy = dy.contiguous()
        return K.gelu_bwd(x, dy if dy.dtype == x.dtype else K.cast(dy, x.dtype))


gelu = GeluFn.apply

_dropout_state = {"seed": 0x5EED, "offset": 0, "base": None, "noise": 0}


def manual_seed(seed: int) -> None:
    _dropout_state["seed"], _dropout_state["offset"], _dropout_state["noise"] = int(seed) & ((1 << 63) - 1), 0, 0
    if _dropout_state["base"] is not None:
        _dropout_state["base"].zero_()


def dropout_step_begin(device) -> None:
    if _dropout_state["base"] is None or _dropout_state["base"].device != torch.device(device):
        _dropout_state["base"] = torch.zeros(1, device=device, dtype=torch.int64)
    _dropout_state["offset"] = 0


def _step_used() -> int:
    used, _dropout_state["offset"] = (_dropout_state["offset"] + 7) // 8 * 8, 0
    return used


def dropout_step_end() -> None:
    base, used = _dropout_state["base"], _step_used()
    if base is not None and used:
        base.add_(used)


def dropout_step_take():
    base, used = _dropout_state["base"], _step_used()
    return (base, used) if (base is not None and used) else (None, 0)


def dropout_device_base_off() -> None:
    _dropout_state["base"] = None


_NOISE_OFFSET = 1 << 44


# ... 591 lines not shown
        elif side is not None:
            torch.cuda.current_stream().wait_stream(side)
            K.shared_chip = False
            del work
        else:
            dS2 = pinv_backward_tile(a2, saved, st, dZ, getattr(ctx, "a2b", None)) if ctx.tile else pinv_backward(a2, saved, st, dZ, pm, sd)
            sm_bwd(a2, dS2, mlm if kmask else None, mlm if kmask else None)
        if dlm2 is None:
            K.gemm(tr(dS2), ql, out=dkl, alpha=scale, accumulate=True, mma=pio)
            K.gemm(dS2, kl, out=dql, alpha=scale, accumulate=True, mma=pio)
        dres = _gret(res_w, dres, dres_sunk)
        dres = None if dres is None else dres.view_as(res_w)
        if de is not None and ctx.link is not None and (kmask is None or (lscale is None and dlm2 is not None)):
            merge = lambda: K.lm_merge(dlm, dlm2, de[Bn * n_p:], D3 - 2 * D)
            ctx.link.lm_merge = (de, merge)
            return dqkv, dres, None, None, None, None, None, None, dlm_out, None, None
        if dlm2 is not None:
            dlm = K.add(dlm, dlm2, out_dtype=A)
        if kmask is not None and lscale is not None:
            dlm = K.row_scale(dlm, lscale)
        if ctx.lm_ext:
            if de is not None:
                dlm_out.copy_(dlm)
                de[Bn * n_p:, 2 * D:].zero_()
                return dqkv, dres, None, None, None, None, None, None, dlm_out, None, None
            return dqkv, dres, None, None, None, None, None, None, dlm, None, None
        K.landmark_bwd(K.cast(dlm, A), dqkv, l)
        return dqkv, dres, None, None, None, None, None, None, None, None, None


class RowScaleFn(Function):

    @staticmethod
    def forward(ctx, x, s):
        ctx.save_for_backward(s)
        return K.row_scale(x.contiguous(), s)

    @staticmethod
    def backward(ctx, dy):
        (s,) = ctx.saved_tensors
        return K.row_scale(dy.contiguous(), s), None


_PROBE = os.environ.get("MIRROR_PROBE", "0") != "0"
_probe_names: List[str] = []
_probe_buf: Optional[torch.Tensor] = None


def probe(name: str) -> None:
    global _probe_buf
    if not _PROBE:
        return
    if _probe_buf is None:
        _probe_buf = torch.zeros(256, dtype=torch.int64, device="cuda")
    if name not in _probe_names:
        _probe_names.append(name)
    K.timestamp(_probe_buf[_probe_names.index(name):_probe_names.index(name) + 1])


def probe_read() -> dict:
    torch.cuda.synchronize()
    v = _probe_buf[:len(_probe_names)].tolist()
    return dict(zip(_probe_names, v))


class ProbeFn(Function):

    @staticmethod
    def forward(ctx, x, name):
        ctx.name = name
        probe(name + ".fwd")
        return x.view_as(x)

    @staticmethod
    def backward(ctx, g):
        probe(ctx.name + ".bwd")
        return g, None


def probe_point(x: torch.Tensor, name: str) -> torch.Tensor:
    if not (_PROBE and x.requires_grad):
        return x
    y = ProbeFn.apply(x, name)
    for attr in ("_bf16", "_relu_slot", "_drop_site", "_fan_slot"):
        if getattr(x, attr, None) is not None:
            setattr(y, attr, getattr(x, attr))
    return y


def rank_mask(noise: torch.Tensor, len_keep: int) -> torch.Tensor:
    return K.rank_mask(noise, len_keep)


class MaskApplyFn(Function):

    @staticmethod
    def forward(ctx, x, mask, token, pos, first, token_scalar):
        x = x.contiguous()
        if x.dim() == 2:
            Bn, T, D = x.shape[0], x.shape[1], 1
        else:
            Bn, T, D = x.shape
        y = torch.empty(x.shape, device=x.device, dtype=f32)
        K.mask_apply_fwd(x, mask, token.detach().reshape(-1).contiguous(), pos.detach().reshape(-1).contiguous(),
                         Bn, T, D, first, token_scalar, out=y)
        ctx.save_for_backward(mask)
        ctx.geom = (Bn, T, D, first, token_scalar, token.shape, pos.shape, x.dtype)
        ctx.params = (token, pos)
        return y

    @staticmethod
    def backward(ctx, dy):
        (mask,) = ctx.saved_tensors
        Bn, T, D, first, token_scalar, tshape, pshape, xdt = ctx.geom
        dy = dy.contiguous()
        dx = torch.empty(dy.shape, device=dy.device, dtype=xdt)
        token, pos = ctx.params
        dtok, s_tok = _gbuf_n(token, (1 if token_scalar else D,))
        dpos, s_pos = _gbuf_n(pos, (T * D,))
        K.mask_apply_bwd(dy, mask, dtok, dpos, Bn, T, D, first, token_scalar, out=dx)
        dtok, dpos = _gret(token, dtok, s_tok), _gret(pos, dpos, s_pos)
        return dx, None, None if dtok is None else dtok.reshape(tshape), None if dpos is None else dpos.reshape(pshape), None, None


class _FanToken:
    __slots__ = ("grad",)

    def __init__(self):
        self.grad = None


class EncFanoutFn(Function):

    @staticmethod
    def forward(ctx, E, tok, slot=None):
        ctx.set_materialize_grads(False)
        ctx.tok, ctx.shape, ctx.slot = tok, tuple(E.shape), slot
        return E.view_as(E), E[:, 1:], E[:, 0]

    @staticmethod
    def backward(ctx, g_full, g_tgt, g_cls):
        Bn, T, D = ctx.shape
        x, alpha = (None, 0.0) if ctx.tok.grad is None else ctx.tok.grad
        ctx.tok.grad = None
        late = None
        if g_tgt is not None:
            if x is None:
                x, alpha = g_tgt.contiguous(), 1.0
            else:
                late = g_tgt
        gf = None if g_full is None else g_full.contiguous().float()
        c = None if g_cls is None else g_cls.contiguous().float()
        if (ctx.slot is not None and _FAN_IN_LN_BWD and late is None and gf is not None and x is not None and x.dtype == bf16
                and x.is_contiguous() and ctx.slot.extra is None):
            ctx.slot.extra = (x, alpha, c)
            return gf, None, None
        dE = K.fanout_bwd(gf, x, alpha, c, Bn, T, D)
        if late is not None:
            dE[:, 1:] += late
        return dE, None, None


def enc_fanout(E: torch.Tensor):
    if not (torch.is_grad_enabled() and E.requires_grad and E.dim() == 3 and E.is_contiguous() and E.dtype == f32):
        return E, E[:, 1:], E[:, 0]
    tok = _FanToken()
    full, tgt, cls = EncFanoutFn.apply(E, tok, getattr(E, "_fan_slot", None))
    tgt._fan_token = tok
    if getattr(E, "_bf16", None) is not None:
        full._bf16 = E._bf16
    return full, tgt, cls


class L2NormRowFn(Function):

    @staticmethod
    def forward(ctx, x, eps, out_dtype):
        if x.dim() == 2 and x.stride(1) == 1 and x.stride(0) >= x.shape[1]:
            (Bn, D), rs = x.shape, x.stride(0)
        else:
            x = x.contiguous()
            if x.dim() == 3:
                Bn, T, D = x.shape
                rs = T * D
            else:
                (Bn, D), rs = x.shape, x.shape[1]
        y, nrm = K.l2norm_fwd(x, Bn, D, rs, eps, out_dtype)
        ctx.save_for_backward(y, nrm)
        ctx.geom = (tuple(x.shape), x.dtype)
        return y

    @staticmethod
    def backward(ctx, dy):
        y, nrm = ctx.saved_tensors
        shape, xdt = ctx.geom
        dy = dy.contiguous()
        if dy.dtype != y.dtype:
            dy = K.cast(dy, y.dtype)
        if len(shape) == 2:
            dx, rs = torch.empty(shape, device=dy.device, dtype=xdt), shape[1]
        else:
            dx = zeros(shape, dy.device) if xdt == f32 else torch.zeros(shape, device=dy.device, dtype=xdt)
            rs = shape[1] * shape[2]
        K.l2norm_bwd(y, nrm, dy, dx, shape[0], shape[-1], rs, accumulate=False)
        return dx, None, None


class HeadAttnFn(Function):

    @staticmethod
    def forward(ctx, qkv, H):
        qkv = qkv.contiguous()
        out, attn = K.headattn_fwd(qkv, H)
        ctx.save_for_backward(qkv, attn)
        ctx.H = H
        return out

    @staticmethod
    def backward(ctx, dout):
        qkv, attn = ctx.saved_tensors
        dout = dout.contiguous()
        if dout.dtype != qkv.dtype:
            dout = K.cast(dout, qkv.dtype)
        return K.headattn_bwd(qkv, attn, dout, ctx.H), None


_RNA_FUSED = True


class RnaBlockFn(Function):

    NAMES = ("g1", "be1", "w_qkv", "b_qkv", "w_proj", "b_proj", "g2", "be2", "w_fc1", "b_fc1", "w_fc2", "b_fc2")

    @staticmethod
    def forward(ctx, x, g1, be1, wqkv, bqkv, wproj, bproj, g2, be2, w1, b1, w2, b2, H, eps, p, prec):
        masters = dict(zip(RnaBlockFn.NAMES, (g1, be1, wqkv, bqkv, wproj, bproj, g2, be2, w1, b1, w2, b2)))
        params = {}
        for k, v in masters.items():
            if v is None:
                params[k] = None
            elif k.startswith("w_"):
                params[k] = shadow(v, prec).contiguous()
            else:
                params[k] = v.detach().reshape(-1)
        B, D = x.shape
        Hh = w1.shape[0]
        st = _dropout_state
        ctx.drop = (float(p), st["seed"], st["offset"], st["base"]) if p > 0.0 else (0.0, 0, 0, None)
        if p > 0.0:
            q4 = lambda n: (n + 3) // 4 * 4
            o0 = st["offset"]
            st["offset"] += 2 * q4(B * D) + q4(B * Hh)
            _tap((B, D), p, st["seed"], o0, False)
            _tap((B, Hh), p, st["seed"], o0 + q4(B * D), False)
# ... 494 lines not shown
```

mirror_amd/kernels.py:

```python
from __future__ import annotations

import ctypes as C
import functools
import os
from typing import Optional


import torch

from . import _lib
from ._lib import ACT_GELU, ACT_NONE, ACT_RELU, MH_BF16, MH_F32, GemmDesc, MirrorHipError

_DT = {torch.float32: MH_F32, torch.bfloat16: MH_BF16}


def dt(t: torch.Tensor) -> int:
    try:
        return _DT[t.dtype]
    except KeyError:
        raise MirrorHipError(f"unsupported dtype {t.dtype} (f32 / bf16 only)") from None


_raw_stream = getattr(torch._C, "_cuda_getCurrentRawStream", None)

# ... 406 lines not shown
    M, Kd = x2d.shape
    N = w.shape[0]
    y = torch.empty((M, N), device=x2d.device, dtype=out_dtype) if out is None else out
    if tuple(y.shape) != (M, N) or y.stride(1) != 1 or x2d.stride(1) != 1 or w.stride(1) != 1:
        raise MirrorHipError("skinny_fwd: bad operands")
    _lib.call("mh_skinny_fwd", _p(x2d), x2d.stride(0), _p(w), w.stride(0), _p(bias), _p(addend), 0 if addend is None else addend.stride(0),
              _p(y), y.stride(0), M, N, Kd, act, dt(x2d), dt(y), stream=_stream())
    return y


def skinny_rows_ok(x2d: torch.Tensor, w: torch.Tensor, y2d: torch.Tensor) -> bool:
    ok_dt = (torch.bfloat16, torch.float32)
    return (x2d.dim() == 2 and w.dim() == 2 and y2d.dim() == 2 and 1 <= x2d.shape[0] <= 32 and x2d.shape[1] % 32 == 0
            and x2d.shape[1] == w.shape[1] and tuple(y2d.shape) == (x2d.shape[0], w.shape[0])
            and x2d.stride(1) == 1 and w.stride(1) == 1 and y2d.stride(1) == 1
            and x2d.stride(0) % 8 == 0 and w.stride(0) % 8 == 0 and y2d.stride(0) % 8 == 0
            and x2d.data_ptr() % 16 == 0 and w.data_ptr() % 16 == 0 and y2d.data_ptr() % 16 == 0
            and x2d.dtype in ok_dt and y2d.dtype in ok_dt and w.dtype == torch.bfloat16)


def skinny_wgrad(dy2d: torch.Tensor, x2d: torch.Tensor, dw: torch.Tensor, accumulate: bool, db: Optional[torch.Tensor] = None) -> None:
    _chk(dy2d, x2d, dw, db)
    assert db is None or (db.dtype == torch.float32 and db.numel() == dy2d.shape[1] and db.is_contiguous())
    M, N = dy2d.shape
    Kd = x2d.shape[1]
    ok_dt = (torch.bfloat16, torch.float32)
    if (dy2d.dtype not in ok_dt or x2d.dtype not in ok_dt or dw.dtype != torch.float32 or x2d.shape[0] != M
            or tuple(dw.shape) != (N, Kd) or dy2d.stride(1) != 1 or x2d.stride(1) != 1 or dw.stride(1) != 1):
        raise MirrorHipError("skinny_wgrad: bad operands")
    _lib.call("mh_skinny_wgrad", _p(dy2d), dy2d.stride(0), _p(x2d), x2d.stride(0), _p(dw), dw.stride(0), _p(db), M, N, Kd,
              int(accumulate), dt(dy2d), dt(x2d), stream=_stream())


SKINNY_MANY_MAX = 32


def skinny_wgrad_many(items) -> None:
    for i0 in range(0, len(items), SKINNY_MANY_MAX):
        chunk = items[i0:i0 + SKINNY_MANY_MAX]
        arr = (_lib.SkinnyWgradItem * len(chunk))()
        for e, (dy2d, x2d, dw, db) in zip(arr, chunk):
            _chk(dy2d, x2d, dw, db)
            M, N = dy2d.shape
            Kd = x2d.shape[1]
            if (dy2d.dtype not in (torch.bfloat16, torch.float32) or x2d.dtype not in (torch.bfloat16, torch.float32) or dw.dtype != torch.float32 or x2d.shape[0] != M
                    or tuple(dw.shape) != (N, Kd) or dy2d.stride(1) != 1 or x2d.stride(1) != 1 or dw.stride(1) != 1
                    or (db is not None and (db.dtype != torch.float32 or db.numel() != N or not db.is_contiguous()))):
                raise MirrorHipError("skinny_wgrad_many: bad operands")
            e.dy, e.lddy, e.x, e.ldx, e.dw, e.lddw, e.db = dy2d.data_ptr(), dy2d.stride(0), x2d.data_ptr(), x2d.stride(0), dw.data_ptr(), dw.stride(0), _p(db)
            e.M, e.N, e.K, e.dt_dy, e.dt_x = M, N, Kd, dt(dy2d), dt(x2d)
        _lib.call("mh_skinny_wgrad_many", arr, len(chunk), stream=_stream())


def transpose_bf16(x: torch.Tensor, out: Optional[torch.Tensor] = None) -> torch.Tensor:
    _chk(x, out)
    _contig(x, "transpose input")
    R, Cc = x.shape
    y = out if out is not None else torch.empty((Cc, R), device=x.device, dtype=torch.bfloat16)
    _lib.call("mh_transpose_bf16", _p(x), _p(y), R, Cc, stream=_stream())
    return y


def transpose_bf16_many(src: torch.Tensor, dst: torch.Tensor, table: torch.Tensor, n: int, max_r: int, max_c: int,
                        vec_ok: bool = False) -> None:
    _chk(src, dst, table)
    assert table.dtype == torch.int64 and table.is_contiguous() and table.numel() == 4 * n
    _lib.call("mh_transpose_bf16_many", _p(src), _p(dst), _p(table), n, max_r, max_c, int(vec_ok), stream=_stream())


def layernorm_fwd(x, gamma, beta, y, mean, rstd, batches, rpb, D, x_bs, y_bs, eps):
    _chk(x, gamma, beta, y, mean, rstd)
    _lib.call("mh_layernorm_fwd", _p(x), _p(gamma), _p(beta), _p(y), _p(mean), _p(rstd), batches, rpb, D, x_bs, y_bs,
              eps, dt(x), dt(y), stream=_stream())


def layernorm_fwd_dual(x, gamma, beta, y, y16, mean, rstd, batches, rpb, D, x_bs, y_bs, eps):
    _chk(x, gamma, beta, y, y16, mean, rstd)
    if not (x.dtype == torch.float32 and y.dtype == torch.float32 and y16.dtype == torch.bfloat16):
        raise MirrorHipError("layernorm_fwd_dual: f32 input, f32 + bf16 outputs")
    _lib.call("mh_layernorm_fwd_dual", _p(x), _p(gamma), _p(beta), _p(y), _p(y16), _p(mean), _p(rstd), batches, rpb, D, x_bs, y_bs,
              eps, stream=_stream())


def layernorm_fwd_q8(x, gamma, beta, y, mean, rstd, batches, rpb, D, x_bs, y_bs, eps, q8, ring, tick, margin: float = 1.25):
    _chk(x, gamma, beta, y, mean, rstd, q8, ring, tick)
    if not (x.dtype == torch.float32 and y.dtype == torch.bfloat16 and q8.dtype == torch.uint8 and ring.numel() == 3
            and ring.dtype == torch.int32 and tick.dtype == torch.float32):
        raise MirrorHipError("layernorm_fwd_q8: f32 input, bf16 + uint8 outputs, int32[3] ring, f32 tick")
    scale = torch.empty((1,), device=x.device, dtype=torch.float32)
    _lib.call("mh_layernorm_fwd_q8", _p(x), _p(gamma), _p(beta), _p(y), _p(mean), _p(rstd), batches, rpb, D, x_bs, y_bs, eps,
              _p(q8), _p(ring), _p(tick), float(margin), _p(scale), stream=_stream())
    return scale


def layernorm_bwd(dy, x, gamma, mean, rstd, dx, dgamma, dbeta, batches, rpb, D, x_bs, y_bs, accumulate_dx=False, gadd=None,
                  pad: int = 0, l: int = 1, relu_out=None, relu_first: int = 0, relu_db=None, fan=None, drop=None, row_mask=None, lm_scale=None):
    _chk(dy, x, gamma, mean, rstd, dx, dgamma, dbeta, gadd, relu_out, relu_db, row_mask, lm_scale)
    d = _lib.LnBwdDesc()
    d.dy, d.x, d.gamma, d.mean, d.rstd, d.dx, d.dgamma, d.dbeta = _p(dy), _p(x), _p(gamma), _p(mean), _p(rstd), _p(dx), _p(dgamma), _p(dbeta)
    d.batches, d.rows_per_batch, d.D, d.x_bs, d.y_bs = batches, rpb, D, x_bs, y_bs
    d.dt_x, d.dt_dy, d.dt_dx, d.accumulate_dx = dt(x), dt(dy), dt(dx), int(accumulate_dx)
    ws = None
    nbytes = int(_lib.load().mh_layernorm_bwd_workspace_bytes(batches * rpb, D))
    if nbytes:
        ws = torch.empty((nbytes // 4,), device=x.device, dtype=torch.float32)
        d.workspace, d.ws_floats = ws.data_ptr(), ws.numel()
    if gadd is not None:
        if gadd.dtype != dy.dtype or not gadd.is_contiguous() or gadd.numel() != batches * ((pad + rpb) // l) * D:
            raise MirrorHipError("layernorm_bwd: gadd must be contiguous [batches, (pad + rows) / l, D] in dy's dtype")
        d.gadd, d.pad, d.l = _p(gadd), int(pad), int(l)
    if lm_scale is not None:
        if lm_scale.dtype != torch.float32 or not lm_scale.is_contiguous() or lm_scale.numel() != batches * ((pad + rpb) // l):
            raise MirrorHipError("layernorm_bwd: lm_scale is a contiguous f32 [batches, (pad + rows) / l]")
        d.lm_scale = _p(lm_scale)
    if row_mask is not None:
        if row_mask.dtype != torch.float32 or not row_mask.is_contiguous() or row_mask.numel() != batches * (pad + rpb):
            raise MirrorHipError("layernorm_bwd: row_mask is a contiguous f32 [batches, pad + rows]")
        d.row_mask = _p(row_mask)
    if relu_out is not None:
        if (relu_out.dtype != torch.bfloat16 or not relu_out.is_contiguous() or relu_out.dim() != 3
                or relu_out.shape[0] != batches or relu_out.shape[2] != D or relu_first + relu_out.shape[1] > rpb):
            raise MirrorHipError("layernorm_bwd: relu_out must be contiguous bf16 [batches, R, D] with relu_first + R <= rows")
        d.relu_out, d.relu_first, d.relu_rows = _p(relu_out), int(relu_first), int(relu_out.shape[1])
    if relu_db is not None:
        if relu_db.dtype != torch.float32 or relu_db.numel() != D or not relu_db.is_contiguous():
            raise MirrorHipError("layernorm_bwd: relu_db is a contiguous f32 [D]")
        d.relu_db = _p(relu_db)
    if fan is not None:
        src, alpha, cls = fan
        _chk(src, cls)
        if not layernorm_bwd_fan_ok(dy, x, dx, src, cls, batches, rpb, D) or ws is None:
            raise MirrorHipError("layernorm_bwd: fan needs f32 x / dx, a contiguous bf16 [batches, rows - 1, D] source and >= 64 rows")
        d.fan_bf16, d.fan_alpha, d.fan_cls = _p(src), float(alpha), _p(cls)
    if drop is not None:
        dout, p_, seed_, off_, base_, ddb = drop
        _chk(dout, base_, ddb)
        if ws is None or not layernorm_bwd_drop_ok(dy, x, dx, dout, ddb, batches, rpb, D, off_):
            raise MirrorHipError("layernorm_bwd: drop needs f32 x / dx, a contiguous bf16 [batches, rows, D] output, D % 8 == 0, D <= 1024, offset % 8 == 0, >= 64 rows")
        d.drop_out, d.drop_p, d.drop_seed, d.drop_offset, d.drop_base, d.drop_db = _p(dout), float(p_), int(seed_), int(off_), _p(base_), _p(ddb)
        d.drop_rows_per_batch = int(dout.shape[1])
    _lib.call("mh_layernorm_bwd", C.byref(d), stream=_stream())


def layernorm_bwd_drop_ok(dy, x, dx, dout, ddb, batches: int, rpb: int, D: int, offset: int) -> bool:
    f = torch.float32
    return (x.dtype == f and dx.dtype == f and dy.dtype in (f, torch.bfloat16) and dout.dtype == torch.bfloat16 and dout.is_contiguous()
            and dout.dim() == 3 and dout.shape[0] == batches and dout.shape[1] >= rpb and dout.shape[2] == D and ddb.dtype == f and ddb.is_contiguous() and ddb.numel() == D and D % 8 == 0 and D <= 1024
            and offset % 8 == 0 and batches * rpb >= 64 and all(t.data_ptr() % 16 == 0 for t in (dy, x, dx, dout)))


def layernorm_bwd_fan_ok(dy, x, dx, src, cls, batches: int, rpb: int, D: int) -> bool:
    f = torch.float32
    return (dy.dtype in (f, torch.bfloat16) and x.dtype == f and dx.dtype == f and src.dtype == torch.bfloat16 and src.is_contiguous()
            and src.numel() == batches * (rpb - 1) * D and rpb >= 2 and batches * rpb >= 64 and D % 4 == 0
            and (cls is None or (cls.dtype == f and cls.is_contiguous() and cls.numel() == batches * D and cls.data_ptr() % 16 == 0))
            and all(t.data_ptr() % 16 == 0 for t in (dy, x, dx)) and src.data_ptr() % 8 == 0)


def layernorm_fwd_lm(x, gamma, beta, y, mean, rstd, xpm, batches, rows, D, x_bs, pad, l, eps, xpm_bf16=None, row_mask=None, lm_scale=None):
    _chk(x, gamma, beta, y, mean, rstd, xpm, xpm_bf16, row_mask, lm_scale)
    if lm_scale is not None and not (lm_scale.dtype == torch.float32 and lm_scale.is_contiguous() and lm_scale.numel() == batches * ((pad + rows) // l)):
        raise MirrorHipError("layernorm_fwd_lm: lm_scale is a contiguous f32 [batches, (pad + rows) / l]")
    if row_mask is not None and not (row_mask.dtype == torch.float32 and row_mask.is_contiguous() and row_mask.numel() == batches * (pad + rows)):
        raise MirrorHipError("layernorm_fwd_lm: row_mask is a contiguous f32 [batches, pad + rows]")
    if not (x.dtype == torch.float32 and y.dtype == torch.bfloat16 and y.is_contiguous() and (xpm is not None or xpm_bf16 is not None)
            and (xpm is None or (xpm.dtype == torch.float32 and xpm.is_contiguous()))):
        raise MirrorHipError("layernorm_fwd_lm: f32 input, contiguous bf16 rows and f32 (and / or bf16) landmark means")
    n_lm = batches * ((pad + rows) // l) * D
    if xpm_bf16 is not None and not (xpm_bf16.dtype == torch.bfloat16 and xpm_bf16.is_contiguous() and xpm_bf16.numel() == n_lm):
        raise MirrorHipError("layernorm_fwd_lm: xpm_bf16 must be a contiguous bf16 tensor of batches * (pad + rows) / l * D elements")
    _lib.call("mh_layernorm_fwd_lm", _p(x), _p(gamma), _p(beta), _p(y), _p(mean), _p(rstd), _p(xpm), _p(xpm_bf16), batches, rows, D, x_bs, int(pad),
              int(l), eps, _p(row_mask), _p(lm_scale), stream=_stream())


def softmax_fwd(x: torch.Tensor, y: Optional[torch.Tensor] = None, out_dtype=None) -> torch.Tensor:
    _chk(x, y)
    _contig(x, "softmax input")
    cols = x.shape[-1]
    if y is None:
        y = torch.empty_like(x, dtype=out_dtype or x.dtype)
    _contig(y, "softmax output")
    _lib.call("mh_softmax_fwd", _p(x), _p(y), x.numel() // max(cols, 1), cols, cols, cols, dt(x), dt(y), stream=_stream())
    return y


def softmax_bwd(y: torch.Tensor, dy: torch.Tensor, dx: Optional[torch.Tensor] = None) -> torch.Tensor:
    _chk(y, dy, dx)
    _contig(y, "softmax y"), _contig(dy, "softmax dy")
    cols = y.shape[-1]
    if dx is None:
        dx = dy
    _lib.call("mh_softmax_bwd", _p(y), _p(dy), _p(dx), y.numel() // max(cols, 1), cols, cols, cols, cols, dt(y), dt(dy),
              dt(dx), stream=_stream())
    return dx


def softmax_masked_fwd(x: torch.Tensor, rowmask: torch.Tensor, colmask: torch.Tensor, y: Optional[torch.Tensor] = None,
                       out_dtype=None) -> torch.Tensor:
    _chk(x, y, rowmask, colmask)
    _contig(x, "softmax input")
    Bn, h, R, Cc = x.shape
    assert rowmask.shape == (Bn, R) and colmask.shape == (Bn, Cc) and rowmask.dtype == colmask.dtype == torch.float32
    if y is None:
        y = torch.empty_like(x, dtype=out_dtype or x.dtype)
    _contig(y, "softmax output")
    _lib.call("mh_softmax_masked_fwd", _p(x), _p(y), _p(rowmask.contiguous()), _p(colmask.contiguous()), Bn, h, R, Cc, dt(x), dt(y),
              stream=_stream())
    return y


def softmax_masked_bwd(y: torch.Tensor, dy: torch.Tensor, rowmask: torch.Tensor, colmask: torch.Tensor) -> torch.Tensor:
    _chk(y, dy, rowmask, colmask)
    _contig(y, "softmax y"), _contig(dy, "softmax dy")
    Bn, h, R, Cc = y.shape
    _lib.call("mh_softmax_masked_bwd", _p(y), _p(dy), _p(dy), _p(rowmask.contiguous()), _p(colmask.contiguous()), Bn, h, R, Cc, dt(y),
              dt(dy), stream=_stream())
    return dy


def row_scale(x: torch.Tensor, scale: torch.Tensor, out: Optional[torch.Tensor] = None) -> torch.Tensor:
    _chk(x, scale, out)
    _contig(x, "row_scale input")
    D = x.shape[-1]
    rows = x.numel() // max(D, 1)
    assert scale.numel() == rows and scale.dtype == torch.float32
    if out is None:
        out = torch.empty_like(x)
    _lib.call("mh_row_scale", _p(x), _p(scale.contiguous()), _p(out), rows, D, dt(x), stream=_stream())
    return out


def keymask_plan(mask: torch.Tensor, lead: int, wrap: int, pad: int, l: int):
    _chk(mask)
    _contig(mask, "key-padding mask")
    assert mask.dtype == torch.bool and mask.dim() == 2
    B, n_src = mask.shape
    n_tot = pad + lead + n_src + wrap
    assert l > 0 and n_tot % l == 0 and 0 <= wrap <= n_src, "the padded sequence must be m groups of l rows"
    m = n_tot // l
# ... 1948 lines not shown
```

mirror_amd/models/mirror.py:

```python
from __future__ import annotations

import logging
import math
import os
from typing import Dict, Optional, Tuple

import numpy as np
import torch
from torch import nn

from .. import functional as Fn
from ..functional import FP32, BF16, POLICIES, Precision
from .._lib import ACT_NONE, MirrorHipError

_logger = logging.getLogger(__name__)
f32 = torch.float32

_DEFAULT_PRECISION: Optional[str] = None

_LM_MASKED = True


def set_precision(name: Optional[str]) -> None:
    global _DEFAULT_PRECISION
# ... 117 lines not shown
        assert residual, "the reference always enables the residual conv (models/mirror.py:306)"
        inner = heads * dim_head
        self.heads, self.num_landmarks, self.pinv_iterations = heads, num_landmarks, pinv_iterations
        self.eps, self.drop = eps, dropout
        self.to_qkv = nn.Linear(dim, inner * 3, bias=False)
        self.to_out = nn.Sequential(nn.Linear(inner, dim), nn.Dropout(dropout))
        ks = residual_conv_kernel
        self.res_conv = nn.Conv2d(heads, heads, (ks, 1), padding=(ks // 2, 0), groups=heads, bias=False)


class TransLayer(nn.Module):

    def __init__(self, dim: int = 512):
        super().__init__()
        self.norm = nn.LayerNorm(dim)
        self.attn = NystromAttention(dim=dim, dim_head=dim // 8, heads=8, num_landmarks=dim // 2,
                                     pinv_iterations=6, residual=True, dropout=0.1)

    def forward(self, x, prec: Precision, mask=None, capture: Optional[list] = None):
        a = self.attn
        if capture is not None and (self.training or torch.is_grad_enabled()):
            raise RuntimeError("TransLayer.forward(capture=): attention maps are read in eval mode under torch.no_grad()")
        n, m = x.shape[1], a.num_landmarks
        pad = (m - n % m) % m
        l = math.ceil(n / m)
        lm = kmask = mrow = None
        link, res = Fn.NystromLink(), Fn.ResidualLink()
        if capture is not None:
            link.capture = {"pad": pad, "n": n}
            capture.append(link.capture)
        if mask is not None:
            km = mask if isinstance(mask, Fn.KeyMask) else Fn.KeyMask(mask.to(x.device))
            if tuple(km.shape) != tuple(x.shape[:2]):
                raise ValueError(f"key-padding mask must be {tuple(x.shape[:2])}, got {tuple(km.shape)}")
            kmask = km.plan(pad, l)
            mrow = kmask[0]
        if (mask is None or _LM_MASKED) and Fn.layer_norm_landmarks_ok(x, n, pad, l, prec):
            lsc = None if kmask is None else kmask[2]
            qkv, lm = Fn.NormQkvLmFn.apply(x, self.norm.weight, self.norm.bias, self.norm.eps, n, pad, l, a.to_qkv.weight, prec, link,
                                           mrow, lsc, res)
            if kmask is not None:
                kmask = (kmask[0], kmask[1], None)
        else:
            xp = Fn.layer_norm(x, self.norm.weight, self.norm.bias, self.norm.eps, pad=pad, out_dtype=prec.act,
                               q8_key=Fn.fp8_site_key(a.to_qkv.weight, prec) if prec.fp8_fwd else None, res=res)
            if mask is not None:
                xp = Fn.RowScaleFn.apply(xp, mrow)
            qkv = Fn.linear(xp, a.to_qkv.weight, None, prec=prec, defer_from=2 * a.to_qkv.weight.shape[1], link=link)
        q8 = [] if prec.fp8_fwd else None
        core = Fn.NystromCoreFn.apply(qkv, a.res_conv.weight, a.heads, l, a.pinv_iterations, prec, kmask,
                                      Fn.fp8_site_key(a.to_out[0].weight, prec) if prec.fp8_fwd else None, lm, link, q8)
        if q8:
            core._q8 = q8[0]
        return Fn.to_out_dropout_add(x, core, a.to_out[0].weight, a.to_out[0].bias, pad, n, a.drop, self.training, prec, res, link)


class PPEG(nn.Module):

    def __init__(self, dim: int = 512):
        super().__init__()
        self.proj = nn.Conv2d(dim, dim, 7, 1, 7 // 2, groups=dim)
        self.proj1 = nn.Conv2d(dim, dim, 5, 1, 5 // 2, groups=dim)
        self.proj2 = nn.Conv2d(dim, dim, 3, 1, 3 // 2, groups=dim)

    def forward(self, x, H, W):
        assert H == W and x.shape[1] == 1 + H * W
        return Fn.PPEGFn.apply(x, self.proj.weight, self.proj.bias, self.proj1.weight, self.proj1.bias,
                               self.proj2.weight, self.proj2.bias, H)


class FeatureTransMIL(nn.Module):

    def __init__(self, input_dim: int = 1024, embed_dim: int = 512):
        super().__init__()
        self.input_dim, self.embed_dim = input_dim, embed_dim
        self.pos_layer = PPEG(dim=embed_dim)
        self._fc1 = nn.Sequential(nn.Linear(input_dim, embed_dim), nn.ReLU())
        self.cls_token = nn.Parameter(torch.randn(1, 1, embed_dim))
        self.layer1 = TransLayer(dim=embed_dim)
        self.layer2 = TransLayer(dim=embed_dim)
        self.norm = nn.LayerNorm(embed_dim)
        self.precision: Optional[str] = None

    def _encode(self, h, keep_rows: Optional[int], mask: Optional[torch.Tensor] = None, capture: Optional[list] = None):
        prec = resolve_precision(self.precision)
        if not h.is_cuda:
            raise MirrorHipError("mirror_amd models run on MI355X only (no CPU fallback): move the inputs to the GPU")
        n_tok = h.shape[1]
        side = int(np.ceil(np.sqrt(n_tok)))
        add = side * side - n_tok
        seq = Fn.probe_point(Fn.fc1_seq(h, self._fc1[0].weight, self._fc1[0].bias, self.cls_token, add, prec), "wsi_fc1_out")
        smask = None
        if mask is not None:
            smask = Fn.KeyMask(mask.to(h.device, torch.bool), lead=1, wrap=add)
        seq = self.layer1(seq, prec, smask, capture)
        seq = self.pos_layer(seq, side, side)
        seq = self.layer2(seq, prec, smask, capture)
        rows = seq.shape[1] - add if keep_rows is None else keep_rows
        return Fn.layer_norm(seq, self.norm.weight, self.norm.bias, self.norm.eps, rows=rows, out_dtype=f32,
                             bf16_copy=(keep_rows is None and prec.act == torch.bfloat16 and torch.is_grad_enabled()))

    def forward(self, h):
        return self._encode(h, keep_rows=1)[:, 0]

    def forward_with_attention(self, h, mask: Optional[torch.Tensor] = None):
        if self.training or torch.is_grad_enabled():
            raise RuntimeError("forward_with_attention: call it in eval mode under torch.no_grad() (the map is an inference output)")
        ops: list = []
        emb = self._encode(h, keep_rows=1, mask=mask, capture=ops)[:, 0]
        n_tok = h.shape[1]
        maps = []
        for o in ops:
            km = o["kmask"]
            row = Fn.K.nys_cls_attn(o["qkv"], o["lm"], o["z"], o["heads"], o["scale"], o["pad"], lse3=o["lse3"],
                                    mrow=None if km is None else km[0], mlm=None if km is None else km[1],
                                    z_colmajor=o["z_colmajor"])
            first = o["pad"] + 1
            m = row[:, :, first:first + n_tok].clone()
            add = o["n"] - 1 - n_tok
            if add:
                m[:, :, :add] += row[:, :, first + n_tok:first + n_tok + add]
            maps.append(m)
        return emb, torch.stack(maps, dim=1)


class TransFormerHybrid(TransFormer):

    def __init__(self, input_dim: int, embed_dim: int = 768, depth: int = 2, num_heads: int = 12,
                 mlp_ratio: float = 4.0, qkv_bias: bool = True, gene_embed: str = "learn",
                 embed_drop_rate: float = 0.0, pos_drop_rate: float = 0.0, proj_drop_rate: float = 0.0,
                 norm_eps: float = 1e-6, retention_decoder_depth: int = 1, **unused):
        super().__init__(input_dim, embed_dim, depth, num_heads, mlp_ratio, qkv_bias, gene_embed,
                         embed_drop_rate, pos_drop_rate, proj_drop_rate, norm_eps)
        self.alignment_head = nn.Linear(embed_dim, embed_dim)
        self.retention_embed = nn.Linear(embed_dim, embed_dim)
        self.mask_token = nn.Parameter(torch.zeros(1, 1))
        self.retention_gene_embed = nn.Parameter(torch.randn(1, embed_dim) * 0.02)
        self.retention_blocks = nn.ModuleList([
            Block(embed_dim, num_heads, mlp_ratio, qkv_bias, proj_drop_rate, norm_eps)
            for _ in range(retention_decoder_depth)])
        self.retention_norm = nn.LayerNorm(embed_dim, eps=norm_eps)
        self.retention_head = nn.Linear(embed_dim, embed_dim)
        nn.init.normal_(self.mask_token, std=0.02)
        _trunc_normal_(self.retention_gene_embed, std=0.02)
        with torch.no_grad():
            for layer_id, layer in enumerate(self.retention_blocks):
                layer.attn.proj.weight.div_(math.sqrt(2.0 * (layer_id + 1)))
                layer.mlp.fc2.weight.div_(math.sqrt(2.0 * (layer_id + 1)))

    def forward_encoder(self, x):
        if not x.is_cuda:
            raise MirrorHipError("mirror_amd models run on MI355X only (no CPU fallback): move the inputs to the GPU")
        return TransFormer.forward(self, x)

    def forward_alignment_head(self, x):
        prec = resolve_precision(self.precision)
        y = Fn.L2NormRowFn.apply(x, 1e-12, f32)
        return Fn.linear(y, self.alignment_head.weight, self.alignment_head.bias, prec=prec, out_dtype=f32)

    def _draw_mask(self, x, mask_ratio: float, noise: Optional[torch.Tensor] = None):
        B, N = x.shape
        len_keep = int(N * (1 - mask_ratio))
        if noise is None:
            noise = torch.rand(B, N, device=x.device)
        return Fn.rank_mask(noise, len_keep)

    def random_masking(self, x, mask_ratio: float, noise: Optional[torch.Tensor] = None) -> Tuple[torch.Tensor, torch.Tensor]:
        mask = self._draw_mask(x, mask_ratio, noise)
        zero_pos = torch.zeros(x.shape[1], device=x.device, dtype=f32)
        return Fn.MaskApplyFn.apply(x, mask, self.mask_token, zero_pos, 0, True), mask

    def forward_retention_head(self, x, mask_ratio: float, noise: Optional[torch.Tensor] = None):
        prec = resolve_precision(self.precision)
        r = Fn.linear(x, self.retention_embed.weight, self.retention_embed.bias, prec=prec, out_dtype=f32)
        mask = self._draw_mask(r, mask_ratio, noise)
        r = Fn.MaskApplyFn.apply(r, mask, self.mask_token, self.retention_gene_embed, 0, True)
        for blk in self.retention_blocks:
            r = blk(r, prec)
        r = Fn.layer_norm(r, self.retention_norm.weight, self.retention_norm.bias, self.retention_norm.eps,
                          out_dtype=prec.act)
        r = Fn.linear(r, self.retention_head.weight, self.retention_head.bias, prec=prec, out_dtype=f32)
        return r, mask

    def forward_decoders(self, x, mask_ratio: float, noise: Optional[torch.Tensor] = None):
        alignment_x = self.forward_alignment_head(x)
        retention_x, mask = self.forward_retention_head(x, mask_ratio, noise)
        return alignment_x, retention_x, mask

    def forward(self, x, mask_ratio: float = 0.75):
        x = self.forward_encoder(x)
        alignment_x, retention_x, mask = self.forward_decoders(x, mask_ratio)
        return alignment_x, retention_x, x, mask


class FeatureTransMILHybrid(FeatureTransMIL):

    def __init__(self, input_dim: int = 1024, embed_dim: int = 512, num_tokens: int = 2048,
                 retention_decoder_depth: int = 1):
        super().__init__(input_dim, embed_dim)
        self.num_tokens = num_tokens
        self.alignment_head = nn.Linear(embed_dim, embed_dim)
        self.retention_embed = nn.Linear(embed_dim, embed_dim)
        self.mask_token = nn.Parameter(torch.zeros(1, 1, embed_dim))
        self.retention_gene_embed = nn.Parameter(torch.randn(1, num_tokens + 1, embed_dim) * 0.02)
        self.retention_blocks = nn.ModuleList([TransLayer(dim=embed_dim) for _ in range(retention_decoder_depth)])
        self.retention_norm = nn.LayerNorm(embed_dim)
        self.retention_head = nn.Linear(embed_dim, embed_dim)
        self.init_weights()

    def init_weights(self) -> None:
        nn.init.normal_(self.mask_token, std=0.02)
        nn.init.normal_(self.cls_token, std=0.02)
        _trunc_normal_(self.retention_gene_embed, std=0.02)
        for m in self.modules():
            if isinstance(m, nn.Linear):
                nn.init.xavier_uniform_(m.weight)
                if m.bias is not None:
                    nn.init.constant_(m.bias, 0)
            elif isinstance(m, nn.LayerNorm):
                nn.init.constant_(m.bias, 0)
                nn.init.constant_(m.weight, 1.0)

    def forward_encoder(self, h, mask: Optional[torch.Tensor] = None):
        return self._encode(h, keep_rows=None, mask=mask)

    def forward_alignment_head(self, h):
        prec = resolve_precision(self.precision)
        y = Fn.L2NormRowFn.apply(h, 1e-12, f32)
        return Fn.linear(y, self.alignment_head.weight, self.alignment_head.bias, prec=prec, out_dtype=f32)

    def _draw_mask(self, h, mask_ratio: float, noise: Optional[torch.Tensor] = None):
        B, N = h.shape[0], h.shape[1]
        len_keep = int(N * (1 - mask_ratio))
        if noise is None:
            noise = torch.rand(B, N, device=h.device)
        return Fn.rank_mask(noise, len_keep)

    def random_masking(self, h, mask_ratio: float, noise: Optional[torch.Tensor] = None) -> Tuple[torch.Tensor, torch.Tensor]:
        mask = self._draw_mask(h, mask_ratio, noise)
        zero_pos = torch.zeros(h.shape[1] * h.shape[2], device=h.device, dtype=f32)
        return Fn.MaskApplyFn.apply(h, mask, self.mask_token, zero_pos, 0, False), mask

    def forward_retention_head(self, h, mask_ratio: float, noise: Optional[torch.Tensor] = None,
                               mask: Optional[torch.Tensor] = None, key_padding_mask: Optional[torch.Tensor] = None,
                               target: Optional[torch.Tensor] = None):
        prec = resolve_precision(self.precision)
        if h.shape[1] != self.num_tokens + 1:
            raise ValueError(f"wsi_num_tokens={self.num_tokens} but the batch has {h.shape[1] - 1} tokens")
        if mask is None:
            mask = self._draw_mask(h[:, 1:], mask_ratio, noise)
        r = Fn.embed_mask_pos(h, self.retention_embed.weight, self.retention_embed.bias, mask, self.mask_token,
                              self.retention_gene_embed, 1, prec)
        kp = None
        if key_padding_mask is not None:
            kp = Fn.KeyMask(key_padding_mask.to(h.device, torch.bool), lead=1)
        for blk in self.retention_blocks:
            r = blk(r, prec, kp)
        r = Fn.layer_norm(r, self.retention_norm.weight, self.retention_norm.bias, self.retention_norm.eps,
                          out_dtype=prec.act)
        r = Fn.head_sqerr(r, self.retention_head.weight, self.retention_head.bias, 1, r.shape[1] - 1, prec, target, mask)
        return r, mask

    def forward_decoders(self, h, mask_ratio: float, noise: Optional[torch.Tensor] = None):
        alignment_h = self.forward_alignment_head(h)
        retention_h, mask = self.forward_retention_head(h, mask_ratio, noise)
        return alignment_h, retention_h, mask

    def forward(self, h, mask_ratio: float = 0.75):
        h = self.forward_encoder(h)
        alignment_h, retention_h, mask = self.forward_decoders(h, mask_ratio)
        return alignment_h, retention_h, h[:, 1:, :], mask


class MIRROR(nn.Module):

    def __init__(self, wsi_embed_dim: int, rna_embed_dim: int, embed_dim: int, wsi_num_tokens: int = 2048,
                 wsi_retention_decoder_depth: int = 1, rna_encoder_depth: int = 2, rna_gene_embed: str = "learn",
                 rna_mlp_ratio: float = 2.572, rna_pos_drop_rate: float = 0.0, rna_proj_drop_rate: float = 0.1,
                 rna_attn_drop_rate: float = 0.0, rna_drop_path_rate: float = 0.0, rna_norm_layer=None,
                 rna_act_layer=None, rna_retention_decoder_depth: int = 1,
                 init_logit_scale: float = float(np.log(1 / 0.07)), style_mlp_hidden_dim: int = 512,
                 style_mlp_out_dim: int = 256, style_norm_layer=None, style_act_layer=None,
                 style_latent_dim: int = 128, num_prototypes: int = 3000, rna_num_heads: int = 12):
        super().__init__()
        for nm, v, ok in (("rna_norm_layer", rna_norm_layer, (None, "layernorm")), ("rna_act_layer", rna_act_layer, (None, "gelu")),
                          ("style_norm_layer", style_norm_layer, (None,)), ("style_act_layer", style_act_layer, (None, "gelu"))):
            if v not in ok:
                raise NotImplementedError(f"{nm}={v!r}: only {ok} have HIP kernels")
        if rna_attn_drop_rate or rna_drop_path_rate:
            raise NotImplementedError("attention dropout / drop-path are 0 in every reference config")
        self.wsi_embed_dim, self.rna_embed_dim, self.embed_dim = wsi_embed_dim, rna_embed_dim, embed_dim
        self.wsi_num_tokens = wsi_num_tokens
        self.style_latent_dim = style_latent_dim
        self.logit_scale = nn.Parameter(torch.ones([]) * init_logit_scale)
        self.wsi_encoder = FeatureTransMILHybrid(wsi_embed_dim, embed_dim, wsi_num_tokens, wsi_retention_decoder_depth)
        self.rna_encoder = TransFormerHybrid(
            input_dim=rna_embed_dim, embed_dim=embed_dim, depth=rna_encoder_depth, num_heads=rna_num_heads,
            mlp_ratio=rna_mlp_ratio, gene_embed=rna_gene_embed, pos_drop_rate=rna_pos_drop_rate,
            proj_drop_rate=rna_proj_drop_rate, retention_decoder_depth=rna_retention_decoder_depth)
        self.style_encoder_mlp = _Mlp(embed_dim, style_mlp_hidden_dim, style_mlp_out_dim, None, 0.0)
        self.style_mu = nn.Linear(style_mlp_out_dim, style_latent_dim)
        self.style_logstd = nn.Linear(style_mlp_out_dim, style_latent_dim)
        self.style_decoder = nn.Linear(style_latent_dim, embed_dim)
        self.prototypes = nn.Linear(embed_dim, num_prototypes, bias=False)
        nn.init.orthogonal_(self.prototypes.weight)
        self._precision: Optional[str] = None
        self._rna_drop_n: Dict[tuple, int] = {}

    @property
    def precision(self) -> Optional[str]:
        return self._precision

    @precision.setter
    def precision(self, name: Optional[str]) -> None:
        if name is not None and name not in POLICIES:
            raise ValueError(f"unknown precision {name!r}")
        self._precision = name
        self.wsi_encoder.precision = name
        self.rna_encoder.precision = name

    def reparameterize(self, mu, logstd, eps: Optional[torch.Tensor] = None):
        if eps is None:
            eps = torch.randn_like(mu)
        return Fn.ReparamFn.apply(mu, logstd, eps)[0]

    def _style_branch(self, emb, eps, prec):
        h = self.style_encoder_mlp(emb, prec)
        mu, logstd = Fn.linear_pair(h, self.style_mu.weight, self.style_mu.bias, self.style_logstd.weight, self.style_logstd.bias,
                                    prec=prec, out_dtype=f32)
        if eps is None:
            eps = torch.randn_like(mu)
        z, mu, logstd = Fn.ReparamFn.apply(mu, logstd, eps)
        z = Fn.linear(z, self.style_decoder.weight, self.style_decoder.bias, prec=prec)
        score = Fn.linear(z, self.prototypes.weight, None, prec=prec, out_dtype=f32)
        return score, mu, logstd

    def forward_style_clustering(self, wsi_emb, rna_emb, wsi_eps=None, rna_eps=None):
        prec = resolve_precision(self._precision)
        wsi_score, wsi_mu, wsi_logstd = self._style_branch(wsi_emb, wsi_eps, prec)
        rna_score, rna_mu, rna_logstd = self._style_branch(rna_emb, rna_eps, prec)
        return wsi_score, wsi_mu, wsi_logstd, rna_score, rna_mu, rna_logstd

    def rna_branch(self, rna_emb, rna_noise, rna_mask_ratio: float):
        Fn.probe("rna_enc_start")
        rna_emb = Fn.probe_point(self.rna_encoder.forward_encoder(rna_emb), "rna_enc_out")
        a, r, mask = self.rna_encoder.forward_decoders(rna_emb, mask_ratio=rna_mask_ratio, noise=rna_noise)
        Fn.probe("rna_branch_end")
        return rna_emb, a, r, mask

    def forward(self, wsi_emb, rna_emb, wsi_mask_ratio: float = 0.75, rna_mask_ratio: float = 0.75,
                noise: Optional[Dict[str, torch.Tensor]] = None, wsi_key_padding_mask: Optional[torch.Tensor] = None):
        noise = dict(noise or {})
        if not wsi_emb.is_cuda:
            raise MirrorHipError("mirror_amd models run on MI355X only (no CPU fallback): move the inputs to the GPU")
        Fn.K.shared_chip = False
        B, dev = wsi_emb.shape[0], wsi_emb.device
        main = torch.cuda.current_stream()
        side = Fn._side_stream(dev, 1)
        wsi_in, rna_in = wsi_emb, rna_emb
        own_draws = self.training and not any(k in noise for k in ("wsi_mask", "rna_mask", "wsi_eps", "rna_eps"))
        if not own_draws:
            if "wsi_mask" not in noise:
                noise["wsi_mask"] = torch.rand(B, wsi_emb.shape[1], device=dev)
            if "rna_mask" not in noise:
                noise["rna_mask"] = torch.rand(B, self.embed_dim, device=dev)
            if "wsi_eps" not in noise:
                noise["wsi_eps"] = torch.randn(B, self.style_latent_dim, device=dev)
            if "rna_eps" not in noise:
                noise["rna_eps"] = torch.randn(B, self.style_latent_dim, device=dev)
        fork = main.record_event()

        def run_side():
            side.wait_event(fork)
            with torch.cuda.stream(side):
                if own_draws:
                    noise["wsi_mask"], noise["rna_mask"], noise["wsi_eps"], noise["rna_eps"] = Fn.noise_draws(
                        B, wsi_in.shape[1], self.embed_dim, self.style_latent_dim, dev)
                n_tok = wsi_in.shape[1]
                mask_ = Fn.rank_mask(noise["wsi_mask"], int(n_tok * (1 - wsi_mask_ratio)))
                ready_ = side.record_event()
                g = getattr(self, "_rna_graph", None)
                if (g is not None and g[1] == rna_mask_ratio and self.training and torch.is_grad_enabled()
                        and not torch.cuda.is_current_stream_capturing() and Fn._dropout_state["offset"] == 0
                        and g[0].matches((rna_in, noise["rna_mask"]))):
                    outs_ = g[0](rna_in, noise["rna_mask"])
                else:
                    outs_ = self.rna_branch(rna_in, noise["rna_mask"], rna_mask_ratio)
            return mask_, ready_, outs_

        st = Fn._dropout_state
        key = (tuple(rna_emb.shape), self.training, torch.is_grad_enabled(), rna_mask_ratio)
        n_rna = self._rna_drop_n.get(key)
        if n_rna is not None:
            off0 = st["offset"]
            st["offset"] = off0 + n_rna
            Fn.probe("wsi_enc_start")
            wsi_emb = Fn.probe_point(self.wsi_encoder.forward_encoder(wsi_in, wsi_key_padding_mask), "wsi_enc_out")
            off_w, st["offset"] = st["offset"], off0
            wsi_mask, mask_ready, (rna_emb, rna_alignment_emb, rna_retention_emb, rna_mask) = run_side()
            if st["offset"] != off0 + n_rna:
                raise MirrorHipError("the RNA branch consumed a different number of dropout offsets than on its first run")
            st["offset"] = off_w
        else:
            off0 = st["offset"]
            wsi_mask, mask_ready, (rna_emb, rna_alignment_emb, rna_retention_emb, rna_mask) = run_side()
            self._rna_drop_n[key] = st["offset"] - off0
            wsi_emb = self.wsi_encoder.forward_encoder(wsi_in, wsi_key_padding_mask)
        wsi_full, wsi_retention_target, wsi_cls = Fn.enc_fanout(wsi_emb)
        heads = side
        heads.wait_event(main.record_event())
        wsi_cls.record_stream(heads)
        with torch.cuda.stream(heads):
            Fn.probe("heads_start")
            wsi_alignment_emb = self.wsi_encoder.forward_alignment_head(wsi_cls)
            wsi_score, wsi_mu, wsi_logstd, rna_score, rna_mu, rna_logstd = self.forward_style_clustering(
                wsi_cls, rna_emb, noise.get("wsi_eps"), noise.get("rna_eps"))
            logit_scale = Fn.exp(self.logit_scale)
            Fn.probe("heads_end")
        ag = getattr(self, "_align_gather", None)
        if ag is not None:
            from ..losses.mirror_loss import prefetch_alignment_gather
            with torch.cuda.stream(heads):
                prefetch_alignment_gather(wsi_alignment_emb, rna_alignment_emb, ag[0])
        main.wait_event(mask_ready)
        wsi_mask.record_stream(main)
        for t in getattr(wsi_mask, "_keep", ())[:2]:
            t.record_stream(main)
        Fn.probe("decoder_start")
        wsi_retention_emb, wsi_mask = self.wsi_encoder.forward_retention_head(
            wsi_full, mask_ratio=wsi_mask_ratio, mask=wsi_mask, key_padding_mask=wsi_key_padding_mask,
            target=wsi_retention_target if self.training else None)
        Fn.probe("decoder_end")
        main.wait_stream(side)
        Fn.probe("fwd_joined")
        for t in (rna_emb, rna_alignment_emb, rna_retention_emb, rna_mask, wsi_alignment_emb, wsi_score, wsi_mu, wsi_logstd,
                  rna_score, rna_mu, rna_logstd, logit_scale):
            t.record_stream(main)
        rna_retention_target = rna_emb
        if own_draws:
            Fn.noise_draws_advance()
        return (wsi_alignment_emb, wsi_retention_emb, wsi_retention_target, wsi_mask, wsi_score, wsi_mu, wsi_logstd,
                rna_alignment_emb, rna_retention_emb, rna_retention_target, rna_mask, rna_score, rna_mu, rna_logstd,
                logit_scale)


_ACCEPTED = {
    "wsi_embed_dim", "rna_embed_dim", "embed_dim", "wsi_num_tokens", "wsi_retention_decoder_depth",
    "rna_encoder_depth", "rna_gene_embed", "rna_mlp_ratio", "rna_pos_drop_rate", "rna_proj_drop_rate",
    "rna_attn_drop_rate", "rna_drop_path_rate", "rna_norm_layer", "rna_act_layer", "rna_retention_decoder_depth",
    "init_logit_scale", "style_mlp_hidden_dim", "style_mlp_out_dim", "style_norm_layer", "style_act_layer",
    "style_latent_dim", "num_prototypes",
    "rna_num_heads",
}


class MIRRORClassifier(nn.Module):

    def __init__(self, wsi_embed_dim: int, rna_embed_dim: int, embed_dim: int, num_classes: int, rna_encoder_depth: int = 2,
                 rna_gene_embed: str = "learn", rna_mlp_ratio: float = 2.572, rna_pos_drop_rate: float = 0.0,
                 rna_proj_drop_rate: float = 0.1, rna_attn_drop_rate: float = 0.0, rna_drop_path_rate: float = 0.0,
                 rna_norm_layer=None, rna_act_layer=None, fusion: str = "concat", rna_num_heads: int = 12):
        super().__init__()
        assert fusion in ["add", "concat"], "Fusion must be either add or concat"
        if rna_attn_drop_rate or rna_drop_path_rate:
            raise NotImplementedError("attention dropout / stochastic depth are 0 in every reference config")
        self.embed_dim, self.num_classes, self.fusion = embed_dim, num_classes, fusion
        self.wsi_encoder = FeatureTransMIL(input_dim=wsi_embed_dim, embed_dim=embed_dim)
        self.rna_encoder = TransFormer(input_dim=rna_embed_dim, embed_dim=embed_dim, depth=rna_encoder_depth,
                                       num_heads=rna_num_heads, mlp_ratio=rna_mlp_ratio, gene_embed=rna_gene_embed,
                                       pos_drop_rate=rna_pos_drop_rate, proj_drop_rate=rna_proj_drop_rate)
        self.head = nn.Linear(embed_dim if fusion == "add" else embed_dim * 2, num_classes)
        self.precision: Optional[str] = None

    def forward(self, wsi_emb: torch.Tensor, rna_emb: Optional[torch.Tensor] = None) -> torch.Tensor:
        prec = resolve_precision(self.precision)
        self.wsi_encoder.precision = self.rna_encoder.precision = self.precision
        return self._head(self.wsi_encoder(wsi_emb), rna_emb, prec)

    def _head(self, w: torch.Tensor, rna_emb: Optional[torch.Tensor], prec: Precision) -> torch.Tensor:
        if rna_emb is None:
            fused = w
        else:
            r = self.rna_encoder(rna_emb)
            fused = Fn.add(w, r, f32) if self.fusion == "add" else torch.cat((w, r), dim=1)
        return Fn.linear(fused.contiguous(), self.head.weight, self.head.bias, prec=prec, out_dtype=f32)

    def forward_with_attention(self, wsi_emb: torch.Tensor, rna_emb: Optional[torch.Tensor] = None):
        if self.training or torch.is_grad_enabled():
            raise RuntimeError("forward_with_attention: call it in eval mode under torch.no_grad() (the map is an inference output)")
        prec = resolve_precision(self.precision)
        self.wsi_encoder.precision = self.rna_encoder.precision = self.precision
        w, attn = self.wsi_encoder.forward_with_attention(wsi_emb)
        return self._head(w, rna_emb, prec), attn


def mirror_classifier(**kwargs) -> MIRRORClassifier:
    accepted = {"wsi_embed_dim", "rna_embed_dim", "embed_dim", "rna_encoder_depth", "rna_gene_embed", "rna_mlp_ratio",
                "rna_pos_drop_rate", "rna_proj_drop_rate", "rna_attn_drop_rate", "rna_drop_path_rate", "rna_norm_layer",
                "rna_act_layer", "num_classes", "fusion", "rna_num_heads"}
    dropped = [k for k in kwargs if k not in accepted]
    if dropped:
        _logger.warning("Filtered model kwargs: %s", ", ".join(dropped))
    return MIRRORClassifier(**{k: v for k, v in kwargs.items() if k in accepted})


def mirror(**kwargs) -> MIRROR:
    kept = {k: v for k, v in kwargs.items() if k in _ACCEPTED}
    dropped = [k for k in kwargs if k not in _ACCEPTED]
    if dropped:
        _logger.warning("Filtered model kwargs: %s", ", ".join(dropped))
    return MIRROR(**kept)
```

Before: 2171 samples/s.

## Fuse kept-row gather into encoder final LayerNorm and its backward

The encoder's final LayerNorm now also writes a compact bf16/f32 copy of only the kept (unmasked) rows, using the random-mask slot map. This lets the retention embedding skip a separate rows_gather and its rows_expand_zero backward. The LayerNorm backward reads the compact gradient and adds it in place. The mask draw is split out of the side-stream work so the keep plan exists before the encoder norm, and a join is inserted just before the norm. This adds cross-stream sync earlier and more kernel template variants.

```diff
diff --git a/include/mirror_hip.h b/include/mirror_hip.h
--- a/include/mirror_hip.h
+++ b/include/mirror_hip.h
@@ -129,6 +129,15 @@
     int32_t drop_rows_per_batch;
 } mh_ln_bwd;
 int mh_layernorm_bwd(const mh_ln_bwd* d, mh_stream s);
+int mh_layernorm_fwd_keep(const float* x, const float* gamma, const float* beta, float* y, void* yc_bf16, float* yc_f32, float* mean,
+                          float* rstd, const int* slot, int batches, int rows_per_batch, int D, int64_t x_bs, int64_t y_bs, float eps,
+                          int first, int keep, mh_stream s);
+typedef struct {
+    const float* dhc;
+    const int32_t* slot;
+    int32_t first, keep;
+} mh_ln_bwd_keep;
+int mh_layernorm_bwd_keep(const mh_ln_bwd* d, const mh_ln_bwd_keep* k, mh_stream s);
 
 int mh_layernorm_fwd_lm(const float* x, const float* gamma, const float* beta, void* y, float* mean, float* rstd, void* xpm,
                         void* xpm_bf16, int batches, int rows, int D, int64_t x_bs, int pad, int l, float eps, const float* row_mask,
diff --git a/mirror_amd/_lib.py b/mirror_amd/_lib.py
--- a/mirror_amd/_lib.py
+++ b/mirror_amd/_lib.py
@@ -110,6 +110,10 @@
     ]
 
 
+class LnBwdKeep(C.Structure):
+    _fields_ = [("dhc", C.c_void_p), ("slot", C.c_void_p), ("first", C.c_int32), ("keep", C.c_int32)]
+
+
 _SIGS = {
     "mh_gemm": [C.POINTER(GemmDesc)],
     "mh_skinny_fwd": [P, L, P, L, P, P, L, P, L, I, I, I, I, I, I],
@@ -121,6 +125,8 @@
     "mh_layernorm_fwd_dual": [P, P, P, P, P, P, P, I, I, I, L, L, F],
     "mh_layernorm_fwd_q8": [P, P, P, P, P, P, I, I, I, L, L, F, P, P, P, F, P],
     "mh_layernorm_bwd": [C.POINTER(LnBwdDesc)],
+    "mh_layernorm_fwd_keep": [P, P, P, P, P, P, P, P, P, I, I, I, L, L, F, I, I],
+    "mh_layernorm_bwd_keep": [C.POINTER(LnBwdDesc), P],
     "mh_layernorm_fwd_lm": [P, P, P, P, P, P, P, P, I, I, I, L, I, I, F, P, P],
     "mh_softmax_fwd": [P, P, L, I, L, L, I, I],
     "mh_softmax_bwd": [P, P, P, L, I, L, L, L, I, I, I],
diff --git a/mirror_amd/csrc/norm_softmax.hip b/mirror_amd/csrc/norm_softmax.hip
--- a/mirror_amd/csrc/norm_softmax.hip
+++ b/mirror_amd/csrc/norm_softmax.hip
@@ -102,12 +102,13 @@
 
 typedef f4_t f4;
 
-template <typename TX, typename TY, int LNV_CH>
+template <typename TX, typename TY, int LNV_CH, bool KEEP = false>
 __global__ __launch_bounds__(256) void layernorm_fwd_vec_kernel(const TX* __restrict__ x, const float* __restrict__ gamma,
                                                                 const float* __restrict__ beta, TY* __restrict__ y,
                                                                 float* __restrict__ mean, float* __restrict__ rstd,
                                                                 long rows, int rpb, int D, long x_bs, long y_bs, float eps,
-                                                                bf16_t* __restrict__ y2 = nullptr) {
+                                                                bf16_t* __restrict__ y2 = nullptr, const int* __restrict__ slot = nullptr,
+                                                                int kfirst = 0, int kkeep = 0, float* __restrict__ y3 = nullptr) {
     const int lane = threadIdx.x & 63;
     const long row = (long)blockIdx.x * 4 + (threadIdx.x >> 6);
     if (row >= rows) return;
@@ -115,6 +116,16 @@
     const TX* xr = x + b * x_bs + i * D;
     TY* yr = y + b * y_bs + i * D;
     bf16_t* y2r = y2 ? y2 + b * y_bs + i * D : nullptr;
+    float* y3r = nullptr;
+    if constexpr (KEEP) {
+        long cr = i;
+        if (i >= kfirst) {
+            const int sl = slot[b * (rpb - kfirst) + (i - kfirst)];
+            cr = (sl >= 0 && sl < kkeep) ? kfirst + sl : -1;
+        }
+        y2r = cr >= 0 ? y2 + (b * (kfirst + kkeep) + cr) * D : nullptr;
+        y3r = (y3 && cr >= 0) ? y3 + (b * (kfirst + kkeep) + cr) * D : nullptr;
+    }
     f4 v[LNV_CH];
     float s = 0.f;
 #pragma unroll
@@ -144,6 +155,7 @@
             for (int e = 0; e < 4; e++) o[e] = (v[k][e] - mu) * rs * g[e] + bt[e];
             st4(yr + c, o);
             if (y2r) st4(y2r + c, o);
+            if constexpr (KEEP) { if (y3r) st4(y3r + c, o); }
         }
     }
     if (lane == 0) { mean[row] = mu; rstd[row] = rs; }
@@ -475,6 +487,24 @@
     return MH_OK;
 }
 
+extern "C" int mh_layernorm_fwd_keep(const float* x, const float* gamma, const float* beta, float* y, void* yc_bf16, float* yc_f32, float* mean,
+                                     float* rstd, const int* slot, int batches, int rpb, int D, int64_t x_bs, int64_t y_bs, float eps, int first, int keep,
+                                     mh_stream s) {
+    const long rows = (long)batches * rpb;
+    MH_REQUIRE(yc_bf16 && D % 4 == 0 && D <= 2048 && x_bs % 4 == 0 && y_bs % 4 == 0 &&
+                   (((uintptr_t)x | (uintptr_t)y | (uintptr_t)gamma | (uintptr_t)beta | (uintptr_t)yc_f32) & 15) == 0 && ((uintptr_t)yc_bf16 & 7) == 0,
+               "mh_layernorm_fwd_keep: D %% 4 == 0, D <= 2048 and aligned buffers (D=%d)", D);
+    MH_REQUIRE(first >= 0 && keep >= 0 && first + keep <= rpb && (slot || rpb == first), "mh_layernorm_fwd_keep: first=%d keep=%d of %d rows, or a null map",
+               first, keep, rpb);
+    if (rows == 0) return MH_OK;
+    dim3 grid(mh_cdiv(rows, 4));
+#define LNK(NC) hipLaunchKernelGGL((layernorm_fwd_vec_kernel<float, float, NC, true>), grid, dim3(256), 0, (hipStream_t)s, x, gamma, beta, y, mean, rstd, rows, rpb, D, (long)x_bs, (long)y_bs, eps, (bf16_t*)yc_bf16, slot, first, keep, yc_f32)
+    if (D <= 512) LNK(2); else if (D <= 1024) LNK(4); else LNK(8);
+#undef LNK
+    MH_LAUNCH_CHECK("mh_layernorm_fwd_keep");
+    return MH_OK;
+}
+
 extern "C" int mh_layernorm_fwd_q8(const float* x, const float* gamma, const float* beta, void* y, float* mean, float* rstd,
                                    int batches, int rows_per_batch, int D, int64_t x_bs, int64_t y_bs, float eps, void* q8, unsigned* ring,
                                    const float* tick, float margin, float* scale, mh_stream s) {
@@ -492,7 +522,7 @@
     return MH_OK;
 }
 
-template <typename TX, typename TDY, int LNV_CH, bool RELU = false, bool FAN = false, bool DROP = false>
+template <typename TX, typename TDY, int LNV_CH, bool RELU = false, bool FAN = false, bool DROP = false, bool KEEP = false>
 __global__ __launch_bounds__(256, LNV_CH == 2 ? 4 : 1) void layernorm_bwd_ws_kernel(const TDY* __restrict__ dy, const TX* __restrict__ x,
                                                                const float* __restrict__ gamma, const float* __restrict__ mean,
                                                                const float* __restrict__ rstd, TX* __restrict__ dx,
@@ -506,8 +536,10 @@
                                                                bf16_t* __restrict__ drop_out = nullptr, float drop_p = 0.f, uint64_t drop_seed = 0,
                                                                uint64_t drop_offset = 0, const uint64_t* __restrict__ drop_base = nullptr,
                                                                int drop_rpb = 0, const float* __restrict__ rmask = nullptr,
-                                                               const float* __restrict__ lm_scale = nullptr) {
-    const int lane = threadIdx.x & 63, wave = threadIdx.x >> 6;
+                                                               const float* __restrict__ lm_scale = nullptr,
+                                                               const float* __restrict__ dhc = nullptr, const int* __restrict__ kslot = nullptr,
+                                                               int kfirst = 0, int kkeep = 0) {
+    const int lane = threadIdx.x & 63, wave = KEEP ? __builtin_amdgcn_readfirstlane(threadIdx.x >> 6) : threadIdx.x >> 6;
     constexpr bool THIRD = RELU || DROP;
     __shared__ f4 sgm[THIRD ? LNV_CH : 1][64];
     f4 pg[LNV_CH], pb[LNV_CH], gm[THIRD ? 1 : LNV_CH], pr[THIRD ? LNV_CH : 1];
@@ -567,14 +599,28 @@
             xo[u] = b * x_bs + (long)i * D;
             ro[u] = (RELU && i >= relu_first && i < relu_first + relu_rows) ? ((long)b * relu_rows + (i - relu_first)) * D
                     : (DROP ? ((long)b * drop_rpb + i) * D : -1);
-            const TDY* dyr = dy + b * y_bs + (long)i * D;
+            const TDY* dyr = (!KEEP || dy) ? dy + b * y_bs + (long)i * D : nullptr;
+            const float* hcr = nullptr;
+            if constexpr (KEEP) {
+                int cr = i;
+                if (i >= kfirst) {
+                    const int sl = kslot[(long)b * (rpb - kfirst) + (i - kfirst)];
+                    cr = (sl >= 0 && sl < kkeep) ? kfirst + sl : -1;
+                }
+                if (cr >= 0) hcr = dhc + ((long)b * (kfirst + kkeep) + cr) * D;
+            }
             mu[u] = mean[rc];
             rs[u] = rstd[rc];
 #pragma unroll
             for (int k = 0; k < LNV_CH; k++) {
                 const int c = 256 * k + 4 * lane;
                 if (c < D) {
-                    dv[u][k] = ld4(dyr + c);
+                    if constexpr (KEEP) {
+                        if (dyr) {
+                            dv[u][k] = ld4(dyr + c);
+                            dv[u][k] += hcr ? ld4(hcr + c) : (f4){0.f, 0.f, 0.f, 0.f};
+                        } else dv[u][k] = hcr ? ld4(hcr + c) : (f4){0.f, 0.f, 0.f, 0.f};
+                    } else dv[u][k] = ld4(dyr + c);
                     xv[u][k] = ld4(x + xo[u] + c);
                     if (acc_dx) ov[u][k] = ld4(dx + xo[u] + c);
                     if (gadd) dv[u][k] += ld4(gadd + ((long)b * ga_m + (i + ga_pad) / ga_l) * D + c) *
@@ -720,7 +766,7 @@
     return 3 * (int64_t)D * nb * 4;
 }
 
-static int ln_bwd_impl(const mh_ln_bwd& d, mh_stream s) {
+static int ln_bwd_impl(const mh_ln_bwd& d, mh_stream s, const mh_ln_bwd_keep* kp = nullptr) {
     const int D = d.D, rpb = d.rows_per_batch, dt_x = d.dt_x, dt_dy = d.dt_dy;
     const int l = d.gadd ? d.l : 1;
     const long rows = (long)d.batches * rpb;
@@ -747,6 +793,11 @@
     MH_REQUIRE(!d.drop_out || (f32_x && d.drop_db && d.drop_p >= 0.f && d.drop_p < 1.f && (d.drop_offset & 7) == 0 && ((uintptr_t)d.drop_out & 7) == 0 &&
                                D % 8 == 0 && D <= 1024 && ws3),
                "mh_layernorm_bwd: drop rider: f32 x / dx, drop_out / drop_db, p in [0, 1), offset %% 8 == 0, D %% 8 == 0, D <= 1024, a workspace of >= 3 D floats");
+    MH_REQUIRE(kp || d.dy, "mh_layernorm_bwd: dy is NULL");
+    MH_REQUIRE(!kp || (kp->dhc && d.fan_bf16 && dt_dy == MH_F32 && kp->first >= 0 && kp->keep >= 0 && kp->first + kp->keep <= rpb &&
+                       (kp->slot || rpb == kp->first) && ((uintptr_t)kp->dhc & 15) == 0),
+               "mh_layernorm_bwd_keep: dhc [batches, first + keep, D] f32 on 16 bytes, slot, first + keep <= rows, the fan rider and dt_dy == MH_F32 (dy may be NULL)");
+    MH_REQUIRE(rows == 0 || ws_form || !kp, "mh_layernorm_bwd_keep: the compact source needs the workspace form");
     MH_REQUIRE(rows == 0 || ws_form || !(d.gadd || d.fan_bf16 || d.drop_out),
                "mh_layernorm_bwd: the %s rider needs the workspace form (D %% 4 == 0, 16-byte aligned buffers, a workspace of >= %d D floats, >= 64 rows)",
                d.gadd ? "landmark" : (d.drop_out ? "drop" : "fan"), d.drop_out ? 3 : 2);
@@ -760,11 +811,18 @@
         const int rows_per_block = (int)(mh_cdiv(mh_cdiv(rows, nb), 8) * 8);
         nb = mh_cdiv(rows, rows_per_block);
         dim3 g2((unsigned)nb);
-#define LN_WS(TX, TDY, NC, RL, FN, DR) hipLaunchKernelGGL((layernorm_bwd_ws_kernel<TX, TDY, NC, RL, FN, DR>), g2, dim3(256), 0, (hipStream_t)s, (const TDY*)d.dy, (const TX*)d.x, d.gamma, d.mean, d.rstd, (TX*)d.dx, d.workspace, (int)rows, rpb, D, (long)d.x_bs, (long)d.y_bs, d.accumulate_dx, rows_per_block, (const TDY*)d.gadd, d.pad, l, (d.pad + rpb) / l, 1.f / (float)l, (bf16_t*)d.relu_out, d.relu_first, d.relu_rows, d.relu_db ? 1 : 0, (const bf16_t*)d.fan_bf16, d.fan_alpha, d.fan_cls, (bf16_t*)d.drop_out, d.drop_p, d.drop_seed, d.drop_offset, d.drop_base, d.drop_rows_per_batch, d.row_mask, d.lm_scale)
+#define LN_WSK(TX, TDY, NC, RL, FN, DR, KP, ...) hipLaunchKernelGGL((layernorm_bwd_ws_kernel<TX, TDY, NC, RL, FN, DR, KP>), g2, dim3(256), 0, (hipStream_t)s, (const TDY*)d.dy, (const TX*)d.x, d.gamma, d.mean, d.rstd, (TX*)d.dx, d.workspace, (int)rows, rpb, D, (long)d.x_bs, (long)d.y_bs, d.accumulate_dx, rows_per_block, (const TDY*)d.gadd, d.pad, l, (d.pad + rpb) / l, 1.f / (float)l, (bf16_t*)d.relu_out, d.relu_first, d.relu_rows, d.relu_db ? 1 : 0, (const bf16_t*)d.fan_bf16, d.fan_alpha, d.fan_cls, (bf16_t*)d.drop_out, d.drop_p, d.drop_seed, d.drop_offset, d.drop_base, d.drop_rows_per_batch, d.row_mask, d.lm_scale, ##__VA_ARGS__)
+#define LN_WS(TX, TDY, NC, RL, FN, DR) LN_WSK(TX, TDY, NC, RL, FN, DR, false)
+#define LN_KP(NC, DR) LN_WSK(float, float, NC, false, true, DR, true, kp->dhc, kp->slot, kp->first, kp->keep)
 #define LN_BW(TX, TDY, RL) do { if (D <= 512) LN_WS(TX, TDY, 2, RL, false, false); else if (D <= 1024) LN_WS(TX, TDY, 4, RL, false, false); else LN_WS(TX, TDY, 8, RL, false, false); } while (0)
 #define LN_BWF(NC) do { if (dt_dy == MH_F32) LN_WS(float, float, NC, false, true, false); else LN_WS(float, bf16_t, NC, false, true, false); } while (0)
 #define LN_BWD(TDY, FN) do { if (D <= 512) LN_WS(float, TDY, 2, false, FN, true); else LN_WS(float, TDY, 4, false, FN, true); } while (0)
-        if (d.drop_out) {
+        if (kp) {
+            if (d.drop_out) { if (D <= 512) LN_KP(2, true); else LN_KP(4, true); }
+            else if (D <= 512) LN_KP(2, false);
+            else if (D <= 1024) LN_KP(4, false);
+            else LN_KP(8, false);
+        } else if (d.drop_out) {
             if (d.fan_bf16 && dt_dy == MH_F32) LN_BWD(float, true);
             else if (d.fan_bf16) LN_BWD(bf16_t, true);
             else if (dt_dy == MH_F32) LN_BWD(float, false);
@@ -779,7 +837,9 @@
 #undef LN_BWD
 #undef LN_BWF
 #undef LN_BW
+#undef LN_KP
 #undef LN_WS
+#undef LN_WSK
         if (D % 4 == 0 && ((uintptr_t)d.workspace & 15) == 0)
             hipLaunchKernelGGL(layernorm_bwd_fold4_kernel, dim3(mh_cdiv(segs * D / 4, 64), (unsigned)min(mh_cdiv(nb, 32), 16)), dim3(256), 0,
                                (hipStream_t)s, (const float*)d.workspace, (int)nb, D, d.dgamma, d.dbeta, segs, third);
@@ -814,6 +874,11 @@
 extern "C" int mh_layernorm_bwd(const mh_ln_bwd* d, mh_stream s) {
     MH_REQUIRE(d, "mh_layernorm_bwd: NULL descriptor");
     return ln_bwd_impl(*d, s);
+}
+
+extern "C" int mh_layernorm_bwd_keep(const mh_ln_bwd* d, const mh_ln_bwd_keep* k, mh_stream s) {
+    MH_REQUIRE(d && k, "mh_layernorm_bwd_keep: NULL descriptor");
+    return ln_bwd_impl(*d, s, k);
 }
 
 template <typename TX, typename TY, bool WAVE>
diff --git a/mirror_amd/functional.py b/mirror_amd/functional.py
--- a/mirror_amd/functional.py
+++ b/mirror_amd/functional.py
@@ -884,9 +884,12 @@
 class EmbedMaskPosFn(Function):
 
     @staticmethod
-    def forward(ctx, h32, h, w, b, mask, token, pos, first, prec, keepmap=None):
+    def forward(ctx, h32, h, w, b, mask, token, pos, first, prec, keepmap=None, rows_T=None):
         wa = shadow(w, prec)
         Bn, T, Kd = h.shape
+        ctx.compact_in = rows_T is not None
+        if rows_T is not None:
+            T = rows_T
         N = wa.shape[0]
         out = torch.empty((Bn, T, N), device=h.device, dtype=f32)
         M = Bn * T
@@ -897,7 +900,7 @@
         ctx.keep = None if keepmap is None else keepmap[2]
         if keepmap is not None:
             keep_idx, slot, keep = keepmap
-            hc = K.rows_gather(h, keep_idx, first, keep)
+            hc = h if ctx.compact_in else K.rows_gather(h, keep_idx, first, keep)
             rc = _gemm_rows(hc, wa.t(), bias=bd, mma=prec.mma, out_dtype=bf16)
             K.mask_expand_fwd(rc, slot, tok, ps, T, first, keep, out)
             ctx.save_for_backward(hc, wa, w, b, slot)
@@ -942,13 +945,33 @@
         dtok, dpos = _gret(token, dtok, s_tok), _gret(pos, dpos, s_pos)
         needs = (ctx.needs_input_grad[0], ctx.needs_input_grad[2], ctx.needs_input_grad[3])
         dh, dw, db = _linear_rows_bwd(needs, h, wa, w, b, 0, Tc, prec, dr, dx_dtype=f32, db_have=db_in)
-        if keep is not None and dh is not None:
+        if keep is not None and dh is not None and not ctx.compact_in:
             dh = K.rows_expand_zero(dh, mask, T, first, keep)
         return (dh, None, dw, db, None, None if dtok is None else dtok.reshape(tshape), None if dpos is None else dpos.reshape(pshape),
-                None, None, None)
-
-
-def embed_mask_pos(h, w, b, mask, token, pos, first: int, prec: Precision):
+                None, None, None, None)
+
+
+def embed_keep_plan(Bn: int, T: int, Kd: int, w, mask, first: int, prec: Precision):
+    if mask is None or not (prec.act == bf16 and not prec.fp8_fwd and mask.dtype == f32 and mask.is_contiguous() and T >= 256):
+        return None
+    wa = shadow(w, prec)
+    if not (K._EPI_ON and wa.dtype == bf16 and wa.dim() == 2 and wa.is_contiguous() and wa.is_cuda and wa.shape[1] == Kd and Kd % 64 == 0
+            and wa.shape[0] % 256 == 0 and Bn * T > 256 and wa.data_ptr() % 16 == 0):
+        return None
+    keepmap = _keep_of(mask, Bn, T - first)
+    if keepmap is None or -(-Bn * T // 256) * (w.shape[0] // 256) <= _EMBED_KEEP_TILES:
+        return None
+    return keepmap
+
+
+def embed_mask_pos(h, w, b, mask, token, pos, first: int, prec: Precision, h_keep=None):
+    if h_keep is not None:
+        hc, km = getattr(h_keep, "_bf16", None), getattr(h_keep, "_keepmap", None)
+        if (km is not None and hc is not None and _keep_of(mask, h.shape[0], h.shape[1] - first) is km and h_keep._first == first
+                and prec.act == bf16 and not prec.fp8_fwd and mask.dtype == f32 and mask.is_contiguous()
+                and tuple(hc.shape) == (h.shape[0], first + km[2], h.shape[2]) and tuple(h_keep.shape) == tuple(hc.shape)
+                and token.numel() == w.shape[0] and pos.numel() == h.shape[1] * w.shape[0]):
+            return EmbedMaskPosFn.apply(h_keep, hc, w, b, mask, token, pos, first, prec, km, h.shape[1])
     hb = h if h.dtype == bf16 else getattr(h, "_bf16", None)
     if (hb is not None and prec.act == bf16 and not prec.fp8_fwd and hb.is_contiguous() and tuple(hb.shape) == tuple(h.shape)
             and mask.dtype == f32 and mask.is_contiguous() and hb.shape[1] >= 256 and K.linear_fused_ok(hb, shadow(w, prec))
@@ -977,7 +1000,7 @@
 class LayerNormFn(Function):
 
     @staticmethod
-    def forward(ctx, x, gamma, beta, eps, rows, pad, out_dtype, q8_key=None, dual=None, fan_slot=None, res=None, q8_out=None):
+    def forward(ctx, x, gamma, beta, eps, rows, pad, out_dtype, q8_key=None, dual=None, fan_slot=None, res=None, q8_out=None, keep=None):
         x = x.contiguous()
         Bn, T, D = x.shape
         y = torch.empty((Bn, pad + rows, D), device=x.device, dtype=out_dtype)
@@ -988,9 +1011,17 @@
         if dual is not None:
             mean = torch.empty((Bn * rows,), device=x.device, dtype=f32)
             rstd = torch.empty_like(mean)
-            y16 = torch.empty((Bn, rows, D), device=x.device, dtype=bf16)
-            K.layernorm_fwd_dual(x, gamma.detach(), beta.detach(), y, y16, mean, rstd, Bn, rows, D, T * D, rows * D, eps)
-            dual.append(y16)
+            if keep is not None:
+                ctx.set_materialize_grads(False)
+                kslot, first, nkeep = keep
+                yc16 = torch.empty((Bn, first + nkeep, D), device=x.device, dtype=bf16)
+                yc32 = torch.empty((Bn, first + nkeep, D), device=x.device, dtype=f32)
+                K.layernorm_fwd_keep(x, gamma.detach(), beta.detach(), y, yc16, yc32, mean, rstd, kslot, Bn, rows, D, T * D, rows * D, eps, first, nkeep)
+                dual.append((yc16, yc32))
+            else:
+                y16 = torch.empty((Bn, rows, D), device=x.device, dtype=bf16)
+                K.layernorm_fwd_dual(x, gamma.detach(), beta.detach(), y, y16, mean, rstd, Bn, rows, D, T * D, rows * D, eps)
+                dual.append(y16)
             ctx.save_for_backward(x, gamma, mean, rstd, beta)
             ctx.rows, ctx.pad = rows, pad
             return y
@@ -1018,21 +1049,31 @@
         x, gamma, mean, rstd, beta = ctx.saved_tensors
         Bn, T, D = x.shape
         rows, pad = ctx.rows, ctx.pad
-        if not dy.is_contiguous():
+        if dy is not None and not dy.is_contiguous():
             dy = dy.contiguous()
         dg, sunk_g = _gbuf(gamma, (D,))
         db, sunk_b = _gbuf(beta, (D,))
-        fan = None
+        fan = keepsrc = None
         if ctx.fan_slot is not None and ctx.fan_slot.extra is not None:
             fan, ctx.fan_slot.extra = ctx.fan_slot.extra, None
+            fan, keepsrc = fan[:3], fan[3]
+            if keepsrc is not None and (pad or not K.layernorm_bwd_keep_ok(dy, keepsrc[0], keepsrc[1], Bn, rows, D, keepsrc[2], keepsrc[3])):
+                dh = K.rows_expand_zero(keepsrc[0], keepsrc[1], rows, keepsrc[2], keepsrc[3])
+                dy, keepsrc = dh if dy is None else dy.float() + dh, None
             if pad or not K.layernorm_bwd_fan_ok(dy, x, x, fan[0], fan[2], Bn, rows, D):
+                if keepsrc is not None:
+                    dh = K.rows_expand_zero(keepsrc[0], keepsrc[1], rows, keepsrc[2], keepsrc[3])
+                    dy, keepsrc = dh if dy is None else dy + dh, None
                 dy, fan = K.fanout_bwd(dy.float(), fan[0], fan[1], fan[2], Bn, rows, D), None
+        if dy is None and keepsrc is None:
+            dy = zeros((Bn, pad + rows, D), x.device)
+        dy_rows = None if dy is None else dy[:, pad:]
         G = None if ctx.res is None else ctx.res.take("grad")
         if G is not None and G.numel() == x.numel() and G.dtype == x.dtype and G.is_contiguous():
             G = G.view(x.shape)
-            K.layernorm_bwd(dy[:, pad:], x, gamma.detach(), mean, rstd, G, dg, db, Bn, rows, D, T * D, (pad + rows) * D,
-                            accumulate_dx=True, fan=fan)
-            return None, _gret(gamma, dg, sunk_g), _gret(beta, db, sunk_b), None, None, None, None, None, None, None, None, None
+            K.layernorm_bwd(dy_rows, x, gamma.detach(), mean, rstd, G, dg, db, Bn, rows, D, T * D, (pad + rows) * D,
+                            accumulate_dx=True, fan=fan, keepsrc=keepsrc)
+            return None, _gret(gamma, dg, sunk_g), _gret(beta, db, sunk_b), None, None, None, None, None, None, None, None, None, None
         dx = torch.empty_like(x)
         if rows < T:
             dx[:, rows:].zero_()
@@ -1040,13 +1081,14 @@
         if site is not None:
             gbd = torch.empty((Bn, T, D), device=x.device, dtype=bf16)
             cs = zeros((D,), x.device)
-            if K.layernorm_bwd_drop_ok(dy, x, dx, gbd, cs, Bn, rows, D, site.offset) and (fan is None or dy.dtype == f32):
+            if K.layernorm_bwd_drop_ok(dy, x, dx, gbd, cs, Bn, rows, D, site.offset) and (fan is None or dy is None or dy.dtype == f32):
                 if rows < T:
                     gbd[:, rows:].zero_()
                 drop = (gbd, site.p, site.seed, site.offset, site.base, cs)
                 site.offer(dx, gbd, cs)
-        K.layernorm_bwd(dy[:, pad:], x, gamma.detach(), mean, rstd, dx, dg, db, Bn, rows, D, T * D, (pad + rows) * D, fan=fan, drop=drop)
-        return dx, _gret(gamma, dg, sunk_g), _gret(beta, db, sunk_b), None, None, None, None, None, None, None, None, None
+        K.layernorm_bwd(dy_rows, x, gamma.detach(), mean, rstd, dx, dg, db, Bn, rows, D, T * D, (pad + rows) * D, fan=fan, drop=drop,
+                        keepsrc=keepsrc)
+        return dx, _gret(gamma, dg, sunk_g), _gret(beta, db, sunk_b), None, None, None, None, None, None, None, None, None, None
 
 
 def _alias(base: torch.Tensor, offset: int, size, stride) -> torch.Tensor:
@@ -1253,7 +1295,7 @@
 
 
 
-def layer_norm(x, gamma, beta, eps, *, rows=None, pad=0, out_dtype=f32, q8_key=None, bf16_copy=False, res=None):
+def layer_norm(x, gamma, beta, eps, *, rows=None, pad=0, out_dtype=f32, q8_key=None, bf16_copy=False, res=None, keepmap=None, first=0):
     squeeze = x.dim() == 2
     if squeeze:
         x = x.unsqueeze(0)
@@ -1264,8 +1306,16 @@
         dual = []
     slot = _FanSlot() if (_FAN_IN_LN_BWD and not squeeze and pad == 0 and out_dtype == f32 and x.dtype == f32) else None
     q8 = [] if q8_key is not None else None
-    y = LayerNormFn.apply(x, gamma, beta, eps, r, pad, out_dtype, q8_key, dual, slot, res, q8)
-    if dual:
+    keep = None
+    if dual is not None and keepmap is not None:
+        kslot = keepmap[1]
+        if (first >= 0 and kslot.dtype == torch.int32 and kslot.is_contiguous() and tuple(kslot.shape) == (x.shape[0], r - first)
+                and 0 <= keepmap[2] <= r - first and kslot.device == x.device):
+            keep = (kslot, int(first), int(keepmap[2]))
+    y = LayerNormFn.apply(x, gamma, beta, eps, r, pad, out_dtype, q8_key, dual, slot, res, q8, keep)
+    if dual and keep is not None:
+        y._keep_rows = (dual[0][0], dual[0][1], keepmap, int(first))
+    elif dual:
         y._bf16 = dual[0]
     if q8:
         y._q8 = q8[0]
@@ -2023,7 +2073,7 @@
     if not (_PROBE and x.requires_grad):
         return x
     y = ProbeFn.apply(x, name)
-    for attr in ("_bf16", "_relu_slot", "_drop_site", "_fan_slot"):
+    for attr in ("_bf16", "_relu_slot", "_drop_site", "_fan_slot", "_keep_rows"):
         if getattr(x, attr, None) is not None:
             setattr(y, attr, getattr(x, attr))
     return y
@@ -2074,14 +2124,18 @@
 class EncFanoutFn(Function):
 
     @staticmethod
-    def forward(ctx, E, tok, slot=None):
+    def forward(ctx, E, tok, slot=None, keep=None):
         ctx.set_materialize_grads(False)
         ctx.tok, ctx.shape, ctx.slot = tok, tuple(E.shape), slot
+        ctx.keep = None if keep is None else keep[1:]
+        if keep is not None:
+            return E.view_as(E), E[:, 1:], E[:, 0], keep[0]
         return E.view_as(E), E[:, 1:], E[:, 0]
 
     @staticmethod
-    def backward(ctx, g_full, g_tgt, g_cls):
+    def backward(ctx, g_full, g_tgt, g_cls, g_keep=None):
         Bn, T, D = ctx.shape
+        nret = 4
         x, alpha = (None, 0.0) if ctx.tok.grad is None else ctx.tok.grad
         ctx.tok.grad = None
         late = None
@@ -2092,25 +2146,39 @@
                 late = g_tgt
         gf = None if g_full is None else g_full.contiguous().float()
         c = None if g_cls is None else g_cls.contiguous().float()
-        if (ctx.slot is not None and _FAN_IN_LN_BWD and late is None and gf is not None and x is not None and x.dtype == bf16
-                and x.is_contiguous() and ctx.slot.extra is None):
-            ctx.slot.extra = (x, alpha, c)
-            return gf, None, None
+        ks = None
+        if g_keep is not None:
+            kslot, first, nkeep = ctx.keep
+            ks = (g_keep.contiguous(), kslot, first, nkeep)
+        if (ctx.slot is not None and _FAN_IN_LN_BWD and late is None and (gf is not None or ks is not None) and x is not None and x.dtype == bf16
+                and x.is_contiguous() and ctx.slot.extra is None and (ks is None or ks[0].dtype == f32)):
+            ctx.slot.extra = (x, alpha, c, ks)
+            return (gf,) + (None,) * (nret - 1)
+        if ks is not None:
+            dh = K.rows_expand_zero(ks[0].float(), kslot, T, first, nkeep)
+            gf = dh if gf is None else gf + dh
         dE = K.fanout_bwd(gf, x, alpha, c, Bn, T, D)
         if late is not None:
             dE[:, 1:] += late
-        return dE, None, None
-
-
-def enc_fanout(E: torch.Tensor):
+        return (dE,) + (None,) * (nret - 1)
+
+
+def enc_fanout(E: torch.Tensor, keepmap=None):
+    four = keepmap is not None
     if not (torch.is_grad_enabled() and E.requires_grad and E.dim() == 3 and E.is_contiguous() and E.dtype == f32):
-        return E, E[:, 1:], E[:, 0]
+        return (E, E[:, 1:], E[:, 0], None) if four else (E, E[:, 1:], E[:, 0])
     tok = _FanToken()
-    full, tgt, cls = EncFanoutFn.apply(E, tok, getattr(E, "_fan_slot", None))
+    kr = getattr(E, "_keep_rows", None)
+    hk = None
+    if four and kr is not None and kr[2] is keepmap:
+        full, tgt, cls, hk = EncFanoutFn.apply(E, tok, getattr(E, "_fan_slot", None), (kr[1], keepmap[1], kr[3], keepmap[2]))
+        hk._bf16, hk._keepmap, hk._first = kr[0], keepmap, kr[3]
+    else:
+        full, tgt, cls = EncFanoutFn.apply(E, tok, getattr(E, "_fan_slot", None))
     tgt._fan_token = tok
     if getattr(E, "_bf16", None) is not None:
         full._bf16 = E._bf16
-    return full, tgt, cls
+    return (full, tgt, cls, hk) if four else (full, tgt, cls)
 
 
 class L2NormRowFn(Function):
diff --git a/mirror_amd/kernels.py b/mirror_amd/kernels.py
--- a/mirror_amd/kernels.py
+++ b/mirror_amd/kernels.py
@@ -512,6 +512,19 @@
               eps, stream=_stream())
 
 
+def layernorm_fwd_keep(x, gamma, beta, y, yc16, yc32, mean, rstd, slot, batches, rpb, D, x_bs, y_bs, eps, first: int, keep: int):
+    _chk(x, gamma, beta, y, yc16, yc32, mean, rstd, slot)
+    n = batches * (first + keep) * D
+    if not (x.dtype == torch.float32 and y.dtype == torch.float32 and yc16.dtype == torch.bfloat16 and yc16.is_contiguous() and yc16.numel() == n
+            and (yc32 is None or (yc32.dtype == torch.float32 and yc32.is_contiguous() and yc32.numel() == n))
+            and slot.dtype == torch.int32 and slot.is_contiguous() and slot.numel() == batches * (rpb - first) and 0 <= first and 0 <= keep
+            and first + keep <= rpb and mean.numel() == batches * rpb and rstd.numel() == batches * rpb):
+        raise MirrorHipError("layernorm_fwd_keep: f32 input / output, contiguous bf16 (and f32) [batches, first + keep, D] compact rows, int32 slot "
+                             "[batches, rows - first]")
+    _lib.call("mh_layernorm_fwd_keep", _p(x), _p(gamma), _p(beta), _p(y), _p(yc16), _p(yc32), _p(mean), _p(rstd), _p(slot), batches, rpb, D, x_bs,
+              y_bs, eps, int(first), int(keep), stream=_stream())
+
+
 def layernorm_fwd_q8(x, gamma, beta, y, mean, rstd, batches, rpb, D, x_bs, y_bs, eps, q8, ring, tick, margin: float = 1.25):
     _chk(x, gamma, beta, y, mean, rstd, q8, ring, tick)
     if not (x.dtype == torch.float32 and y.dtype == torch.bfloat16 and q8.dtype == torch.uint8 and ring.numel() == 3
@@ -524,12 +537,15 @@
 
 
 def layernorm_bwd(dy, x, gamma, mean, rstd, dx, dgamma, dbeta, batches, rpb, D, x_bs, y_bs, accumulate_dx=False, gadd=None,
-                  pad: int = 0, l: int = 1, relu_out=None, relu_first: int = 0, relu_db=None, fan=None, drop=None, row_mask=None, lm_scale=None):
+                  pad: int = 0, l: int = 1, relu_out=None, relu_first: int = 0, relu_db=None, fan=None, drop=None, row_mask=None, lm_scale=None,
+                  keepsrc=None):
     _chk(dy, x, gamma, mean, rstd, dx, dgamma, dbeta, gadd, relu_out, relu_db, row_mask, lm_scale)
+    if dy is None and keepsrc is None:
+        raise MirrorHipError("layernorm_bwd: dy is None (only a compact source may stand in for it)")
     d = _lib.LnBwdDesc()
     d.dy, d.x, d.gamma, d.mean, d.rstd, d.dx, d.dgamma, d.dbeta = _p(dy), _p(x), _p(gamma), _p(mean), _p(rstd), _p(dx), _p(dgamma), _p(dbeta)
     d.batches, d.rows_per_batch, d.D, d.x_bs, d.y_bs = batches, rpb, D, x_bs, y_bs
-    d.dt_x, d.dt_dy, d.dt_dx, d.accumulate_dx = dt(x), dt(dy), dt(dx), int(accumulate_dx)
+    d.dt_x, d.dt_dy, d.dt_dx, d.accumulate_dx = dt(x), (MH_F32 if dy is None else dt(dy)), dt(dx), int(accumulate_dx)
     ws = None
     nbytes = int(_lib.load().mh_layernorm_bwd_workspace_bytes(batches * rpb, D))
     if nbytes:
@@ -569,22 +585,39 @@
             raise MirrorHipError("layernorm_bwd: drop needs f32 x / dx, a contiguous bf16 [batches, rows, D] output, D % 8 == 0, D <= 1024, offset % 8 == 0, >= 64 rows")
         d.drop_out, d.drop_p, d.drop_seed, d.drop_offset, d.drop_base, d.drop_db = _p(dout), float(p_), int(seed_), int(off_), _p(base_), _p(ddb)
         d.drop_rows_per_batch = int(dout.shape[1])
+    if keepsrc is not None:
+        dhc, slot, first, keep = keepsrc
+        _chk(dhc, slot)
+        if (fan is None or not layernorm_bwd_keep_ok(dy, dhc, slot, batches, rpb, D, first, keep)):
+            raise MirrorHipError("layernorm_bwd: keepsrc needs the fan rider, f32 dy (or None), contiguous f32 dhc [batches, first + keep, D] "
+                                 "and int32 slot [batches, rows - first]")
+        k = _lib.LnBwdKeep()
+        k.dhc, k.slot, k.first, k.keep = _p(dhc), _p(slot), int(first), int(keep)
+        _lib.call("mh_layernorm_bwd_keep", C.byref(d), C.addressof(k), stream=_stream())
+        return
     _lib.call("mh_layernorm_bwd", C.byref(d), stream=_stream())
+
+
+def layernorm_bwd_keep_ok(dy, dhc, slot, batches: int, rpb: int, D: int, first: int, keep: int) -> bool:
+    f = torch.float32
+    return ((dy is None or dy.dtype == f) and dhc.dtype == f and dhc.is_contiguous() and dhc.numel() == batches * (first + keep) * D
+            and dhc.data_ptr() % 16 == 0 and slot.dtype == torch.int32 and slot.is_contiguous() and slot.numel() == batches * (rpb - first)
+            and 0 <= first and 0 <= keep and first + keep <= rpb)
 
 
 def layernorm_bwd_drop_ok(dy, x, dx, dout, ddb, batches: int, rpb: int, D: int, offset: int) -> bool:
     f = torch.float32
-    return (x.dtype == f and dx.dtype == f and dy.dtype in (f, torch.bfloat16) and dout.dtype == torch.bfloat16 and dout.is_contiguous()
+    return (x.dtype == f and dx.dtype == f and (dy is None or dy.dtype in (f, torch.bfloat16)) and dout.dtype == torch.bfloat16 and dout.is_contiguous()
             and dout.dim() == 3 and dout.shape[0] == batches and dout.shape[1] >= rpb and dout.shape[2] == D and ddb.dtype == f and ddb.is_contiguous() and ddb.numel() == D and D % 8 == 0 and D <= 1024
-            and offset % 8 == 0 and batches * rpb >= 64 and all(t.data_ptr() % 16 == 0 for t in (dy, x, dx, dout)))
+            and offset % 8 == 0 and batches * rpb >= 64 and all(t.data_ptr() % 16 == 0 for t in (dy, x, dx, dout) if t is not None))
 
 
 def layernorm_bwd_fan_ok(dy, x, dx, src, cls, batches: int, rpb: int, D: int) -> bool:
     f = torch.float32
-    return (dy.dtype in (f, torch.bfloat16) and x.dtype == f and dx.dtype == f and src.dtype == torch.bfloat16 and src.is_contiguous()
+    return ((dy is None or dy.dtype in (f, torch.bfloat16)) and x.dtype == f and dx.dtype == f and src.dtype == torch.bfloat16 and src.is_contiguous()
             and src.numel() == batches * (rpb - 1) * D and rpb >= 2 and batches * rpb >= 64 and D % 4 == 0
             and (cls is None or (cls.dtype == f and cls.is_contiguous() and cls.numel() == batches * D and cls.data_ptr() % 16 == 0))
-            and all(t.data_ptr() % 16 == 0 for t in (dy, x, dx)) and src.data_ptr() % 8 == 0)
+            and all(t.data_ptr() % 16 == 0 for t in (dy, x, dx) if t is not None) and src.data_ptr() % 8 == 0)
 
 
 def layernorm_fwd_lm(x, gamma, beta, y, mean, rstd, xpm, batches, rows, D, x_bs, pad, l, eps, xpm_bf16=None, row_mask=None, lm_scale=None):
diff --git a/mirror_amd/models/mirror.py b/mirror_amd/models/mirror.py
--- a/mirror_amd/models/mirror.py
+++ b/mirror_amd/models/mirror.py
@@ -223,7 +223,8 @@
         self.norm = nn.LayerNorm(embed_dim)
         self.precision: Optional[str] = None
 
-    def _encode(self, h, keep_rows: Optional[int], mask: Optional[torch.Tensor] = None, capture: Optional[list] = None):
+    def _encode(self, h, keep_rows: Optional[int], mask: Optional[torch.Tensor] = None, capture: Optional[list] = None,
+                keepmap=None, before_norm=None):
         prec = resolve_precision(self.precision)
         if not h.is_cuda:
             raise MirrorHipError("mirror_amd models run on MI355X only (no CPU fallback): move the inputs to the GPU")
@@ -238,8 +239,11 @@
         seq = self.pos_layer(seq, side, side)
         seq = self.layer2(seq, prec, smask, capture)
         rows = seq.shape[1] - add if keep_rows is None else keep_rows
+        if before_norm is not None:
+            before_norm()
         return Fn.layer_norm(seq, self.norm.weight, self.norm.bias, self.norm.eps, rows=rows, out_dtype=f32,
-                             bf16_copy=(keep_rows is None and prec.act == torch.bfloat16 and torch.is_grad_enabled()))
+                             bf16_copy=(keep_rows is None and prec.act == torch.bfloat16 and torch.is_grad_enabled()),
+                             keepmap=keepmap if keep_rows is None else None, first=1)
 
     def forward(self, h):
         return self._encode(h, keep_rows=1)[:, 0]
@@ -362,8 +366,8 @@
                 nn.init.constant_(m.bias, 0)
                 nn.init.constant_(m.weight, 1.0)
 
-    def forward_encoder(self, h, mask: Optional[torch.Tensor] = None):
-        return self._encode(h, keep_rows=None, mask=mask)
+    def forward_encoder(self, h, mask: Optional[torch.Tensor] = None, keepmap=None, before_norm=None):
+        return self._encode(h, keep_rows=None, mask=mask, keepmap=keepmap, before_norm=before_norm)
 
     def forward_alignment_head(self, h):
         prec = resolve_precision(self.precision)
@@ -384,14 +388,14 @@
 
     def forward_retention_head(self, h, mask_ratio: float, noise: Optional[torch.Tensor] = None,
                                mask: Optional[torch.Tensor] = None, key_padding_mask: Optional[torch.Tensor] = None,
-                               target: Optional[torch.Tensor] = None):
+                               target: Optional[torch.Tensor] = None, h_keep: Optional[torch.Tensor] = None):
         prec = resolve_precision(self.precision)
         if h.shape[1] != self.num_tokens + 1:
             raise ValueError(f"wsi_num_tokens={self.num_tokens} but the batch has {h.shape[1] - 1} tokens")
         if mask is None:
             mask = self._draw_mask(h[:, 1:], mask_ratio, noise)
         r = Fn.embed_mask_pos(h, self.retention_embed.weight, self.retention_embed.bias, mask, self.mask_token,
-                              self.retention_gene_embed, 1, prec)
+                              self.retention_gene_embed, 1, prec, h_keep=h_keep)
         kp = None
         if key_padding_mask is not None:
             kp = Fn.KeyMask(key_padding_mask.to(h.device, torch.bool), lead=1)
@@ -511,7 +515,7 @@
                 noise["rna_eps"] = torch.randn(B, self.style_latent_dim, device=dev)
         fork = main.record_event()
 
-        def run_side():
+        def run_mask():
             side.wait_event(fork)
             with torch.cuda.stream(side):
                 if own_draws:
@@ -520,6 +524,10 @@
                 n_tok = wsi_in.shape[1]
                 mask_ = Fn.rank_mask(noise["wsi_mask"], int(n_tok * (1 - wsi_mask_ratio)))
                 ready_ = side.record_event()
+            return mask_, ready_
+
+        def run_side():
+            with torch.cuda.stream(side):
                 g = getattr(self, "_rna_graph", None)
                 if (g is not None and g[1] == rna_mask_ratio and self.training and torch.is_grad_enabled()
                         and not torch.cuda.is_current_stream_capturing() and Fn._dropout_state["offset"] == 0
@@ -527,7 +535,23 @@
                     outs_ = g[0](rna_in, noise["rna_mask"])
                 else:
                     outs_ = self.rna_branch(rna_in, noise["rna_mask"], rna_mask_ratio)
-            return mask_, ready_, outs_
+            return outs_
+
+        wsi_mask, mask_ready = run_mask()
+        keepmap = None
+        if self.training and torch.is_grad_enabled():
+            keepmap = Fn.embed_keep_plan(B, wsi_in.shape[1] + 1, self.wsi_encoder.embed_dim, self.wsi_encoder.retention_embed.weight, wsi_mask, 1,
+                                         resolve_precision(self.wsi_encoder.precision))
+        joined = []
+
+        def join_mask():
+            if joined:
+                return
+            joined.append(1)
+            main.wait_event(mask_ready)
+            wsi_mask.record_stream(main)
+            for t in getattr(wsi_mask, "_keep", ())[:2]:
+                t.record_stream(main)
 
         st = Fn._dropout_state
         key = (tuple(rna_emb.shape), self.training, torch.is_grad_enabled(), rna_mask_ratio)
@@ -536,18 +560,24 @@
             off0 = st["offset"]
             st["offset"] = off0 + n_rna
             Fn.probe("wsi_enc_start")
-            wsi_emb = Fn.probe_point(self.wsi_encoder.forward_encoder(wsi_in, wsi_key_padding_mask), "wsi_enc_out")
+            wsi_emb = Fn.probe_point(self.wsi_encoder.forward_encoder(wsi_in, wsi_key_padding_mask, keepmap=keepmap,
+                                                                      before_norm=join_mask if keepmap is not None else None), "wsi_enc_out")
             off_w, st["offset"] = st["offset"], off0
-            wsi_mask, mask_ready, (rna_emb, rna_alignment_emb, rna_retention_emb, rna_mask) = run_side()
+            rna_emb, rna_alignment_emb, rna_retention_emb, rna_mask = run_side()
             if st["offset"] != off0 + n_rna:
                 raise MirrorHipError("the RNA branch consumed a different number of dropout offsets than on its first run")
             st["offset"] = off_w
         else:
             off0 = st["offset"]
-            wsi_mask, mask_ready, (rna_emb, rna_alignment_emb, rna_retention_emb, rna_mask) = run_side()
+            rna_emb, rna_alignment_emb, rna_retention_emb, rna_mask = run_side()
             self._rna_drop_n[key] = st["offset"] - off0
-            wsi_emb = self.wsi_encoder.forward_encoder(wsi_in, wsi_key_padding_mask)
-        wsi_full, wsi_retention_target, wsi_cls = Fn.enc_fanout(wsi_emb)
+            wsi_emb = self.wsi_encoder.forward_encoder(wsi_in, wsi_key_padding_mask, keepmap=keepmap,
+                                                       before_norm=join_mask if keepmap is not None else None)
+        wsi_keep = None
+        if keepmap is not None:
+            wsi_full, wsi_retention_target, wsi_cls, wsi_keep = Fn.enc_fanout(wsi_emb, keepmap)
+        else:
+            wsi_full, wsi_retention_target, wsi_cls = Fn.enc_fanout(wsi_emb)
         heads = side
         heads.wait_event(main.record_event())
         wsi_cls.record_stream(heads)
@@ -563,14 +593,11 @@
             from ..losses.mirror_loss import prefetch_alignment_gather
             with torch.cuda.stream(heads):
                 prefetch_alignment_gather(wsi_alignment_emb, rna_alignment_emb, ag[0])
-        main.wait_event(mask_ready)
-        wsi_mask.record_stream(main)
-        for t in getattr(wsi_mask, "_keep", ())[:2]:
-            t.record_stream(main)
+        join_mask()
         Fn.probe("decoder_start")
         wsi_retention_emb, wsi_mask = self.wsi_encoder.forward_retention_head(
             wsi_full, mask_ratio=wsi_mask_ratio, mask=wsi_mask, key_padding_mask=wsi_key_padding_mask,
-            target=wsi_retention_target if self.training else None)
+            target=wsi_retention_target if self.training else None, h_keep=wsi_keep)
         Fn.probe("decoder_end")
         main.wait_stream(side)
         Fn.probe("fwd_joined")
```

Result: no change. 2192 samples/s (median of 6 runs) (+1.0%).
